# h-walk/PSA

Measured on AMD Instinct MI355X. Metric: SED throughput (k-points*timesteps*atoms/s), higher is better.
Workload: dtype f32 (2xf16 split MFMA, fp32 accumulate)

## Files before the change

include/psa_hip.h:

```cpp
#ifndef PSA_HIP_H
#define PSA_HIP_H

#include <stdint.h>

#ifdef __cplusplus
extern "C" {
#endif

#define PSA_HIP_ABI_VERSION 6

#define PSA_OK          0
#define PSA_EINVAL     -1
#define PSA_EHIP       -2
#define PSA_EFFT       -3
#define PSA_ERCCL      -4
#define PSA_ESTATE     -5
#define PSA_ENOMEM     -6

#define PSA_SLOT_VELOCITIES 0
#define PSA_SLOT_POSITIONS  1
#define PSA_NUM_SLOTS       2

#define PSA_F_DISPLACEMENTS  0x1
#define PSA_F_INTENSITY      0x2

#define PSA_K1_AUTO   0
#define PSA_K1_WAVE   1
#define PSA_K1_MFMA32 2
#define PSA_K1_SPLIT_BF16 3

typedef struct psa_ctx psa_ctx;

int         psa_abi_version(void);
const char* psa_last_error(void);
int         psa_device_count(int* count);
int         psa_host_alloc(size_t bytes, void** out);
int         psa_host_free(void* p);
int         psa_create(int device, psa_ctx** out);
int         psa_destroy(psa_ctx* ctx);
int         psa_synchronize(psa_ctx* ctx);
int         psa_set_k1(psa_ctx* ctx, int selector);
#define PSA_OPT_PLANES         0
#define PSA_OPT_PLANES_BUDGET  1
#define PSA_OPT_PLANES_EAGER   2
#define PSA_OPT_PLANES_MIN_K   3
#define PSA_OPT_FOLD_PAIRS     4
#define PSA_OPT_FFT_PRIME      5
#define PSA_OPT_K1_LOADER_WAVES 6
#define PSA_OPT_K1_WIDE         7
#define PSA_OPT_K1_LOWRANK      8
#define PSA_OPT_K1_LOWRANK_MIN_K 9
#define PSA_OPT_K1_LOWRANK_MIN_LOCAL 10
#define PSA_OPT_VDOS_WORK_BYTES 11
#define PSA_OPT_MODES_WORK_BYTES 12
#define PSA_OPT_DYNAMIC_WORK_BYTES 13
int         psa_set_option(psa_ctx* ctx, int option, int64_t value);
int         psa_device_info(psa_ctx* ctx, char* name, int name_len,
                            int* compute_units, int64_t* hbm_bytes);

int psa_data_upload(psa_ctx* ctx, int slot, const float* host, int64_t T, int64_t N);
int psa_data_alloc(psa_ctx* ctx, int slot, int64_t T, int64_t N);
int psa_data_download(psa_ctx* ctx, int slot, float* host, int64_t t0, int64_t nt);
int psa_data_release(psa_ctx* ctx, int slot);
int psa_data_shape(psa_ctx* ctx, int slot, int64_t* T, int64_t* N);

int psa_data_fill_synthetic(psa_ctx* ctx, int slot, uint64_t seed, int64_t t_offset, int n_modes,
                            const float* amp, const int32_t* mode_comp,
                            const float* ct, const float* st,
                            const float* ca, const float* sa);

int psa_mean_positions(psa_ctx* ctx, int slot, float* mean_host );

int psa_host_mean_frames(const float* x , int64_t T, int64_t cols, float* mean_out, int threads);

int psa_set_atom_weights(psa_ctx* ctx, const float* w , int64_t N);

int psa_set_segments(psa_ctx* ctx, int64_t L, int64_t hop, const float* window );

int psa_sed_project(psa_ctx* ctx, int slot,
                    const float* mean_pos_all,
                    const float* k_vectors, int64_t K_local,
                    int64_t K_total, int64_t k_offset,
                    const int32_t* group_idx, const int64_t* group_off, int32_t G,
                    int32_t flags);

int psa_sed_project_upload(psa_ctx* ctx, int slot, const float* host, int64_t T, int64_t N,
                           const float* mean_pos_all, const float* k_vectors, int64_t K,
                           const int32_t* group_idx, const int64_t* group_off, int32_t G,
                           int32_t flags);

int psa_sed_finalize(psa_ctx* ctx, void* out_host, size_t out_bytes,
                     float* out_intensity, size_t out_intensity_bytes);

int psa_sed_calculate(psa_ctx* ctx, int slot, const float* mean_pos_all,
                      const float* k_vectors, int64_t K,
                      const int32_t* group_idx, const int64_t* group_off, int32_t G,
                      int32_t flags, void* out_host, size_t out_bytes,
                      float* out_intensity, size_t out_intensity_bytes);

int psa_vdos(psa_ctx* ctx, int slot, const float* mean_pos_all ,
             const int32_t* group_idx, const int64_t* group_off, int32_t G,
             int32_t flags , float* out_host , size_t out_bytes);

int psa_sed_modes(psa_ctx* ctx, int slot, const float* mean_pos_all, const float* k_vectors, int64_t K,
                  const int32_t* group_idx, const int64_t* group_off, int32_t B,
                  const void* eig , int64_t M, int32_t flags ,
                  float* out_host , size_t out_bytes);

int psa_sed_covariance(psa_ctx* ctx, int slot, const float* mean_pos_all, const float* k_vectors, int64_t K,
                       const int32_t* group_idx, const int64_t* group_off, int32_t B,
                       const float* freq_weights , int32_t n_w, int32_t flags ,
                       double* out_host , size_t out_bytes);

typedef struct {
    float   window_hwhm;
    int32_t half_window_bins;
    int32_t max_iter;
} psa_peak_opts;
int psa_fit_peaks(psa_ctx* ctx, const float* spec_host, int64_t F, int64_t C, double df, const int32_t* bands, int32_t lo,
                  int32_t hi, const psa_peak_opts* opts, float* fit , int32_t* info );
int psa_sed_modes_fit(psa_ctx* ctx, int slot, const float* mean_pos_all, const float* k_vectors, int64_t K,
                      const int32_t* group_idx, const int64_t* group_off, int32_t B, const void* eig, int64_t M,
                      int32_t flags, double df, const int32_t* bands, int32_t lo, int32_t hi, const psa_peak_opts* opts,
                      float* fit , int32_t* info , float* out_host, size_t out_bytes);

int psa_sed_modes_welch(psa_ctx* ctx, int slot, const float* mean_pos_all, const float* k_vectors, int64_t K,
                        const int32_t* group_idx, const int64_t* group_off, int32_t B,
                        const void* eig , int64_t M, int32_t flags ,
                        float* out_host , size_t out_bytes);
int psa_sed_modes_welch_fit(psa_ctx* ctx, int slot, const float* mean_pos_all, const float* k_vectors, int64_t K,
                            const int32_t* group_idx, const int64_t* group_off, int32_t B, const void* eig, int64_t M,
                            int32_t flags, double df, const int32_t* bands, int32_t lo, int32_t hi, const psa_peak_opts* opts,
                            float* fit , int32_t* info , float* out_host, size_t out_bytes);

int psa_dynamic_spectra(psa_ctx* ctx, const float* k_vectors, int64_t K, const int32_t* idx, int64_t n_g,
                        int32_t currents , float* out_host ,
                        size_t out_bytes);

int psa_lattice_spectra(psa_ctx* ctx, const double* box_inverse , const int32_t* indices , int64_t K,
                        const int32_t* bin_of , int64_t n_bins, const int32_t* idx, int64_t n_g,
                        int32_t currents , float* out_host ,
                        size_t out_bytes);

int psa_self_spectra(psa_ctx* ctx, const double* box_inverse , const int32_t* indices , int64_t K,
                     const int32_t* bin_of , int64_t n_bins, const int32_t* idx, int64_t n_g,
                     float* out_host , size_t out_bytes);

int psa_partial_spectra(psa_ctx* ctx, const double* box_inverse , const int32_t* indices , int64_t K,
                        const int32_t* bin_of , int64_t n_bins, const int32_t* idx, const int64_t* species_start ,
                        int32_t n_species, int32_t currents ,
                        float* out_host , size_t out_bytes);

int psa_lattice_correlations(psa_ctx* ctx, const double* box_inverse , const int32_t* indices , int64_t K,
                             const int32_t* bin_of , int64_t n_bins, const int32_t* idx, int64_t n_g,
                             int32_t currents , int64_t n_lags,
                             float* out_host , size_t out_bytes);

int psa_self_correlations(psa_ctx* ctx, const double* box_inverse , const int32_t* indices , int64_t K,
                          const int32_t* bin_of , int64_t n_bins, const int32_t* idx, int64_t n_g, int64_t n_lags,
                          float* out_host , size_t out_bytes);

int psa_displacement_moments(psa_ctx* ctx, const double* box , const double* box_inverse , const int32_t* idx,
                             const int64_t* group_start , int32_t n_groups, int64_t n_lags, int64_t origin_step,
                             int32_t unwrap, double* out_host , size_t out_bytes);

int psa_van_hove_self(psa_ctx* ctx, const double* box , const double* box_inverse , const int32_t* idx,
                      const int64_t* group_start , int32_t n_groups, const int64_t* lags , int64_t n_vh,
                      int64_t origin_step, int32_t unwrap, double dr, int32_t n_r, uint64_t* out_host ,
                      size_t out_bytes);

int psa_pair_histogram(psa_ctx* ctx, const double* box , const double* box_inverse , const int32_t* idx,
                       const int64_t* group_start , int32_t n_groups, const int64_t* lags , int64_t n_lags,
                       int64_t origin_step, double dr, int32_t n_r, uint64_t* out_host ,
                       size_t out_bytes);

#define PSA_KMAP_MIRROR 0x80000000u
int psa_k_pairs(const float* k_vectors, int64_t K, int32_t* kmap ,
                int32_t* unique_idx , int64_t* n_unique);
int psa_sed_set_kmap(psa_ctx* ctx, const int32_t* kmap, int64_t K_out);

int psa_lowrank_plan(const float* k_vectors, int64_t K, const float* mean_pos_all, int64_t N, const int32_t* idx,
                     int64_t n_g, int32_t* ok, double* geo, double* kappa, float* C, float* L, float* phi);

int psa_sed_single_bin(psa_ctx* ctx, int slot, const float* mean_pos_all, const float* k_vector,
                       const int32_t* idx, int64_t n_g, int32_t flags, int64_t i_w,
                       float* out_c64x3 );

int psa_slab_read(psa_ctx* ctx, int64_t row0, int64_t nrows, void* host);
int psa_slab_write(psa_ctx* ctx, int64_t row0, int64_t nrows, const void* host);

int psa_result_intensity(psa_ctx* ctx, float* out_host , size_t out_bytes);
int psa_result_chiral_phase(psa_ctx* ctx, int c1, int c2, float* out_host, size_t out_bytes);

int psa_last_timings(psa_ctx* ctx, double* ms );
int psa_k1_stats(psa_ctx* ctx, int64_t* launches, double* total_ms);
int psa_k1_lowrank_launches(psa_ctx* ctx, int64_t* launches);
int psa_oneoff_stats(psa_ctx* ctx, double* ms );

int psa_debug_phase_table(psa_ctx* ctx, const float* mean_pos_all,
                          const float* k_vectors, int64_t K,
                          const int32_t* idx, int64_t n_g, int64_t N,
                          void* out_host);
int psa_debug_project_only(psa_ctx* ctx, int slot, const float* mean_pos_all,
                           const float* k_vectors, int64_t K,
                           const int32_t* idx, int64_t n_g, int32_t flags,
                           void* out_host);
int psa_debug_project_route(psa_ctx* ctx, int slot, const float* mean_pos_all,
                            const float* k_vectors, int64_t K,
                            const int32_t* idx, int64_t n_g, int32_t flags,
                            void* out_host);
int psa_debug_project_frames(psa_ctx* ctx, int slot, const float* mean_pos_all,
                             const float* k_vectors, int64_t K,
                             const int32_t* idx, int64_t n_g, int32_t flags,
                             int64_t t_begin, int64_t t_count, void* out_host);
int psa_debug_mode_power(psa_ctx* ctx, const void* S_host, const void* eig, int32_t B, int64_t K, int64_t M, int64_t T,
                         float* out_host);
int psa_debug_covariance(psa_ctx* ctx, const void* S_host , int32_t B, int64_t K,
                         int64_t T, const float* freq_weights, int32_t n_w, double scale, double* out_host);
int psa_debug_mode_power_welch(psa_ctx* ctx, const void* S_host, const void* eig, int32_t B, int64_t K, int64_t M, int64_t L,
                               int64_t ns, int64_t seg_block, float scale, float* out_host);
int psa_debug_dynamic_project(psa_ctx* ctx, const float* k_vectors, int64_t K, const int32_t* idx, int64_t n_g,
                              int32_t currents, void* out_host);
int psa_debug_dynamic_sincos(psa_ctx* ctx, const float* turns, int64_t n, float* out_host);
int psa_debug_lattice_project(psa_ctx* ctx, const double* box_inverse, const int32_t* indices, int64_t K, const int32_t* idx,
                              int64_t n_g, int32_t currents, void* out_host);
int psa_debug_self_series(psa_ctx* ctx, const double* box_inverse, const int32_t* indices, int64_t K, const int32_t* idx,
                          int64_t n_g, void* out_host);
int psa_debug_dynamic_power(psa_ctx* ctx, const void* seg_host, const float* k_vectors , int64_t K, int32_t currents,
                            int64_t n_seg, int64_t L, int64_t k_block, int64_t seg_block, float scale, float* out_host);
int psa_debug_lattice_shell(psa_ctx* ctx, const void* seg_host, const float* khat , const int32_t* bin_of ,
                            int64_t K, int64_t n_bins, int32_t currents, int64_t n_seg, int64_t L, int64_t k_block,
                            int64_t seg_block, double norm, float* out_host);
int psa_debug_self_power(psa_ctx* ctx, const void* work_host, int64_t na, int64_t nv, int64_t n_seg, int64_t L,
                         const int32_t* groups, int64_t n_groups, int64_t cols, const double* scale, int32_t mirror,
                         int64_t n_chunks, int64_t atom_block, int64_t vec_block, int64_t seg_block, float* out_host);
int psa_debug_partial_project(psa_ctx* ctx, const double* box_inverse, const int32_t* indices, int64_t K, const int32_t* idx,
                              const int64_t* species_start, int32_t n_species, int32_t currents, void* out_host);
int psa_debug_partial_power(psa_ctx* ctx, const void* seg_host, const float* khat , const int32_t* bin_of ,
                            int64_t K, int64_t n_bins, int32_t n_species, int32_t currents, int64_t n_seg, int64_t L,
                            int64_t k_block, int64_t seg_block, double norm, float* out_host);
int psa_debug_plane_cache(psa_ctx* ctx, int64_t* n_sets, int64_t* bytes);

#define PSA_UNIQUE_ID_BYTES 128
int psa_comm_unique_id(void* out );
int psa_comm_init(psa_ctx* ctx, const void* unique_id, int rank, int nranks);
int psa_comm_destroy(psa_ctx* ctx);
int psa_comm_selftest(psa_ctx* ctx);
int psa_sed_gather(psa_ctx* ctx, int root, const int64_t* k_offsets, const int64_t* k_counts);
int psa_comm_barrier(psa_ctx* ctx);

int psa_sed_fs_project(psa_ctx* ctx, int slot, const float* mean_pos_all,
                       const float* k_vectors, int64_t K_total,
                       const int32_t* idx, int64_t n_g, int32_t flags,
                       int64_t T_total, int64_t k_offset, int64_t k_count);
int psa_sed_fs_exchange(psa_ctx* ctx, const int64_t* t_offsets, const int64_t* t_counts,
                        const int64_t* k_offsets, const int64_t* k_counts);
int psa_sed_fs_read(psa_ctx* ctx, int64_t k0, int64_t nk, void* host);
int psa_sed_fs_write(psa_ctx* ctx, int64_t t0, int64_t nt, const void* host);
int psa_sed_fs_finish(psa_ctx* ctx, int32_t first_group);

int psa_debug_correlation_transform(psa_ctx* ctx, const double* X_host, int64_t fields, int64_t P, int64_t cols, int64_t L,
                                    int64_t n_seg, int64_t n_lags, int32_t as_float32, float* out_host);

int psa_debug_unwrap(psa_ctx* ctx, const double* box , const double* box_inverse , const int32_t* idx, int64_t n_g,
                     int32_t unwrap, double* out_u , int32_t* out_images );

int psa_debug_pair_fractions(psa_ctx* ctx, const double* box_inverse , const int32_t* idx, int64_t n_g,
                             float* out );

int psa_debug_pair_plan(const int64_t* sizes , int32_t n_groups, int32_t sym, int64_t n_origins, int64_t* out );

#ifdef __cplusplus
}
#endif
#endif
```

psa_amd/_hip.py:

```python
from __future__ import annotations

import ctypes as C
import os
import threading
import weakref
from pathlib import Path
from typing import Optional, Sequence

import numpy as np

LIB_PATH = Path(__file__).resolve().parent / "csrc" / "libpsa_hip.so"

SLOT_VELOCITIES, SLOT_POSITIONS = 0, 1
F_DISPLACEMENTS, F_INTENSITY = 0x1, 0x2
K1_AUTO, K1_WAVE, K1_MFMA32, K1_SPLIT_BF16 = 0, 1, 2, 3
OPT_PLANES, OPT_PLANES_BUDGET, OPT_PLANES_EAGER, OPT_PLANES_MIN_K, OPT_FOLD_PAIRS, OPT_FFT_PRIME = 0, 1, 2, 3, 4, 5
OPT_K1_LOADER_WAVES = 6
OPT_K1_WIDE = 7
OPT_K1_LOWRANK = 8
OPT_K1_LOWRANK_MIN_K = 9
OPT_K1_LOWRANK_MIN_LOCAL = 10
OPT_VDOS_WORK_BYTES = 11
OPT_MODES_WORK_BYTES = 12
OPT_DYNAMIC_WORK_BYTES = 13
KMAP_MIRROR = 0x80000000
ABI_VERSION = 6
COV_CHAIN = 128
COV_FOLDS = 32
COV_TILE = 64
COV_CHUNK = COV_CHAIN * COV_FOLDS
COV_MAX_ROWS = 96
DYN_THREADS = 256
DYN_ATOMS = 512
DYN_CHAIN = 128
DYN_FRAMES = 4
DYN_SINCOS_ERR = 2.6e-7
LAT_THREADS = 256
LAT_KS = 512
LAT_ATOMS = 128
LAT_TABLE = 3584
LAT_CHAIN = 128
LAT_FRAMES = 4
LAT_MAX_INDEX = 64
LAT_MAX_ENTRIES = 3 * (2 * LAT_MAX_INDEX + 1)
PARTIAL_MAX_SPECIES = 8
SELF_THREADS = 256
SELF_ATOMS = 4
SELF_FRAMES = 64
SELF_ENTRIES = 24
SELF_KS = 64
MSD_LAGS = 256
MSD_ORIGINS = 1024
MSD_WINDOW = 1280
MSD_MAX_GROUPS = 8
MSD_MAX_BINS = 1024
MSD_MAX_VH_LAGS = 64
MSD_UNWRAP_FRAMES = 64
MSD_UNWRAP_ATOMS = 16
PAIR_TILE = 256
PAIR_MAX_BINS = 1024
PAIR_MAX_LAGS = 64
PAIR_MAX_SPECIES = 8
UNIQUE_ID_BYTES = 128
TIMING_NAMES = ("h2d", "phase", "project", "fft", "epilogue", "gather", "transpose", "d2h")

_f32p = C.POINTER(C.c_float)
_i32p = C.POINTER(C.c_int32)
_i64p = C.POINTER(C.c_int64)
_ctx = C.c_void_p

SIGNATURES = {
    "psa_abi_version": (C.c_int, []),
    "psa_last_error": (C.c_char_p, []),
    "psa_device_count": (C.c_int, [C.POINTER(C.c_int)]),
    "psa_host_alloc": (C.c_int, [C.c_size_t, C.POINTER(C.c_void_p)]),
    "psa_host_free": (C.c_int, [C.c_void_p]),
    "psa_create": (C.c_int, [C.c_int, C.POINTER(_ctx)]),
    "psa_destroy": (C.c_int, [_ctx]),
    "psa_synchronize": (C.c_int, [_ctx]),
    "psa_set_k1": (C.c_int, [_ctx, C.c_int]),
    "psa_set_option": (C.c_int, [_ctx, C.c_int, C.c_int64]),
    "psa_device_info": (C.c_int, [_ctx, C.c_char_p, C.c_int, C.POINTER(C.c_int), _i64p]),
    "psa_data_upload": (C.c_int, [_ctx, C.c_int, _f32p, C.c_int64, C.c_int64]),
    "psa_data_alloc": (C.c_int, [_ctx, C.c_int, C.c_int64, C.c_int64]),
    "psa_data_download": (C.c_int, [_ctx, C.c_int, _f32p, C.c_int64, C.c_int64]),
    "psa_data_release": (C.c_int, [_ctx, C.c_int]),
    "psa_data_shape": (C.c_int, [_ctx, C.c_int, _i64p, _i64p]),
    "psa_data_fill_synthetic": (C.c_int, [_ctx, C.c_int, C.c_uint64, C.c_int64, C.c_int, _f32p, _i32p,
                                          _f32p, _f32p, _f32p, _f32p]),
    "psa_mean_positions": (C.c_int, [_ctx, C.c_int, _f32p]),
    "psa_host_mean_frames": (C.c_int, [_f32p, C.c_int64, C.c_int64, _f32p, C.c_int]),
    "psa_set_atom_weights": (C.c_int, [_ctx, _f32p, C.c_int64]),
    "psa_set_segments": (C.c_int, [_ctx, C.c_int64, C.c_int64, _f32p]),
    "psa_sed_project": (C.c_int, [_ctx, C.c_int, _f32p, _f32p, C.c_int64, C.c_int64, C.c_int64,
                                  _i32p, _i64p, C.c_int32, C.c_int32]),
    "psa_sed_project_upload": (C.c_int, [_ctx, C.c_int, _f32p, C.c_int64, C.c_int64, _f32p, _f32p, C.c_int64,
                                         _i32p, _i64p, C.c_int32, C.c_int32]),
    "psa_sed_finalize": (C.c_int, [_ctx, C.c_void_p, C.c_size_t, _f32p, C.c_size_t]),
    "psa_sed_calculate": (C.c_int, [_ctx, C.c_int, _f32p, _f32p, C.c_int64, _i32p, _i64p,
                                    C.c_int32, C.c_int32, C.c_void_p, C.c_size_t, _f32p, C.c_size_t]),
    "psa_vdos": (C.c_int, [_ctx, C.c_int, _f32p, _i32p, _i64p, C.c_int32, C.c_int32, _f32p, C.c_size_t]),
    "psa_sed_modes": (C.c_int, [_ctx, C.c_int, _f32p, _f32p, C.c_int64, _i32p, _i64p, C.c_int32, C.c_void_p, C.c_int64,
                                C.c_int32, _f32p, C.c_size_t]),
    "psa_fit_peaks": (C.c_int, [_ctx, _f32p, C.c_int64, C.c_int64, C.c_double, _i32p, C.c_int32, C.c_int32, C.c_void_p,
                                _f32p, _i32p]),
    "psa_sed_modes_fit": (C.c_int, [_ctx, C.c_int, _f32p, _f32p, C.c_int64, _i32p, _i64p, C.c_int32, C.c_void_p, C.c_int64,
                                    C.c_int32, C.c_double, _i32p, C.c_int32, C.c_int32, C.c_void_p, _f32p, _i32p, _f32p,
                                    C.c_size_t]),
    "psa_sed_modes_welch": (C.c_int, [_ctx, C.c_int, _f32p, _f32p, C.c_int64, _i32p, _i64p, C.c_int32, C.c_void_p, C.c_int64,
                                      C.c_int32, _f32p, C.c_size_t]),
    "psa_sed_modes_welch_fit": (C.c_int, [_ctx, C.c_int, _f32p, _f32p, C.c_int64, _i32p, _i64p, C.c_int32, C.c_void_p,
                                          C.c_int64, C.c_int32, C.c_double, _i32p, C.c_int32, C.c_int32, C.c_void_p, _f32p,
                                          _i32p, _f32p, C.c_size_t]),
    "psa_dynamic_spectra": (C.c_int, [_ctx, _f32p, C.c_int64, _i32p, C.c_int64, C.c_int32, _f32p, C.c_size_t]),
    "psa_debug_dynamic_project": (C.c_int, [_ctx, _f32p, C.c_int64, _i32p, C.c_int64, C.c_int32, C.c_void_p]),
    "psa_debug_dynamic_sincos": (C.c_int, [_ctx, _f32p, C.c_int64, _f32p]),
    "psa_lattice_spectra": (C.c_int, [_ctx, C.POINTER(C.c_double), _i32p, C.c_int64, _i32p, C.c_int64, _i32p, C.c_int64, C.c_int32,
                                      _f32p, C.c_size_t]),
    "psa_debug_lattice_project": (C.c_int, [_ctx, C.POINTER(C.c_double), _i32p, C.c_int64, _i32p, C.c_int64, C.c_int32, C.c_void_p]),
    "psa_self_spectra": (C.c_int, [_ctx, C.POINTER(C.c_double), _i32p, C.c_int64, _i32p, C.c_int64, _i32p, C.c_int64, _f32p,
                                   C.c_size_t]),
    "psa_debug_self_series": (C.c_int, [_ctx, C.POINTER(C.c_double), _i32p, C.c_int64, _i32p, C.c_int64, C.c_void_p]),
    "psa_debug_dynamic_power": (C.c_int, [_ctx, C.c_void_p, _f32p, C.c_int64, C.c_int32, C.c_int64, C.c_int64, C.c_int64, C.c_int64,
                                          C.c_float, _f32p]),
    "psa_debug_lattice_shell": (C.c_int, [_ctx, C.c_void_p, _f32p, _i32p, C.c_int64, C.c_int64, C.c_int32, C.c_int64, C.c_int64,
                                          C.c_int64, C.c_int64, C.c_double, _f32p]),
    "psa_debug_self_power": (C.c_int, [_ctx, C.c_void_p, C.c_int64, C.c_int64, C.c_int64, C.c_int64, _i32p, C.c_int64, C.c_int64,
                                       C.POINTER(C.c_double), C.c_int32, C.c_int64, C.c_int64, C.c_int64, C.c_int64, _f32p]),
    "psa_partial_spectra": (C.c_int, [_ctx, C.POINTER(C.c_double), _i32p, C.c_int64, _i32p, C.c_int64, _i32p, _i64p, C.c_int32,
                                      C.c_int32, _f32p, C.c_size_t]),
    "psa_debug_partial_project": (C.c_int, [_ctx, C.POINTER(C.c_double), _i32p, C.c_int64, _i32p, _i64p, C.c_int32, C.c_int32,
                                            C.c_void_p]),
    "psa_debug_partial_power": (C.c_int, [_ctx, C.c_void_p, _f32p, _i32p, C.c_int64, C.c_int64, C.c_int32, C.c_int32, C.c_int64,
                                          C.c_int64, C.c_int64, C.c_int64, C.c_double, _f32p]),
    "psa_lattice_correlations": (C.c_int, [_ctx, C.POINTER(C.c_double), _i32p, C.c_int64, _i32p, C.c_int64, _i32p, C.c_int64,
                                           C.c_int32, C.c_int64, _f32p, C.c_size_t]),
    "psa_self_correlations": (C.c_int, [_ctx, C.POINTER(C.c_double), _i32p, C.c_int64, _i32p, C.c_int64, _i32p, C.c_int64,
                                        C.c_int64, _f32p, C.c_size_t]),
    "psa_debug_correlation_transform": (C.c_int, [_ctx, C.POINTER(C.c_double), C.c_int64, C.c_int64, C.c_int64, C.c_int64,
                                                  C.c_int64, C.c_int64, C.c_int32, _f32p]),
    "psa_displacement_moments": (C.c_int, [_ctx, C.POINTER(C.c_double), C.POINTER(C.c_double), _i32p, _i64p, C.c_int32, C.c_int64,
                                           C.c_int64, C.c_int32, C.POINTER(C.c_double), C.c_size_t]),
    "psa_van_hove_self": (C.c_int, [_ctx, C.POINTER(C.c_double), C.POINTER(C.c_double), _i32p, _i64p, C.c_int32, _i64p, C.c_int64,
                                    C.c_int64, C.c_int32, C.c_double, C.c_int32, C.POINTER(C.c_uint64), C.c_size_t]),
    "psa_debug_unwrap": (C.c_int, [_ctx, C.POINTER(C.c_double), C.POINTER(C.c_double), _i32p, C.c_int64, C.c_int32,
                                   C.POINTER(C.c_double), _i32p]),
    "psa_pair_histogram": (C.c_int, [_ctx, C.POINTER(C.c_double), C.POINTER(C.c_double), _i32p, _i64p, C.c_int32, _i64p, C.c_int64,
                                     C.c_int64, C.c_double, C.c_int32, C.POINTER(C.c_uint64), C.c_size_t]),
    "psa_debug_pair_fractions": (C.c_int, [_ctx, C.POINTER(C.c_double), _i32p, C.c_int64, _f32p]),
    "psa_debug_pair_plan": (C.c_int, [_i64p, C.c_int32, C.c_int32, C.c_int64, _i64p]),
    "psa_k_pairs": (C.c_int, [_f32p, C.c_int64, _i32p, _i32p, _i64p]),
    "psa_lowrank_plan": (C.c_int, [_f32p, C.c_int64, _f32p, C.c_int64, _i32p, C.c_int64, _i32p, C.POINTER(C.c_double),
                                   C.POINTER(C.c_double), _f32p, _f32p, _f32p]),
    "psa_sed_set_kmap": (C.c_int, [_ctx, _i32p, C.c_int64]),
    "psa_sed_single_bin": (C.c_int, [_ctx, C.c_int, _f32p, _f32p, _i32p, C.c_int64, C.c_int32, C.c_int64, _f32p]),
    "psa_slab_read": (C.c_int, [_ctx, C.c_int64, C.c_int64, C.c_void_p]),
    "psa_slab_write": (C.c_int, [_ctx, C.c_int64, C.c_int64, C.c_void_p]),
    "psa_result_intensity": (C.c_int, [_ctx, _f32p, C.c_size_t]),
    "psa_result_chiral_phase": (C.c_int, [_ctx, C.c_int, C.c_int, _f32p, C.c_size_t]),
    "psa_last_timings": (C.c_int, [_ctx, C.POINTER(C.c_double)]),
    "psa_k1_stats": (C.c_int, [_ctx, _i64p, C.POINTER(C.c_double)]),
    "psa_k1_lowrank_launches": (C.c_int, [_ctx, _i64p]),
    "psa_oneoff_stats": (C.c_int, [_ctx, C.POINTER(C.c_double)]),
    "psa_debug_phase_table": (C.c_int, [_ctx, _f32p, _f32p, C.c_int64, _i32p, C.c_int64,
                                        C.c_int64, C.c_void_p]),
    "psa_debug_project_only": (C.c_int, [_ctx, C.c_int, _f32p, _f32p, C.c_int64, _i32p,
                                         C.c_int64, C.c_int32, C.c_void_p]),
    "psa_debug_project_route": (C.c_int, [_ctx, C.c_int, _f32p, _f32p, C.c_int64, _i32p,
                                          C.c_int64, C.c_int32, C.c_void_p]),
    "psa_debug_project_frames": (C.c_int, [_ctx, C.c_int, _f32p, _f32p, C.c_int64, _i32p,
                                           C.c_int64, C.c_int32, C.c_int64, C.c_int64, C.c_void_p]),
    "psa_debug_mode_power": (C.c_int, [_ctx, C.c_void_p, C.c_void_p, C.c_int32, C.c_int64, C.c_int64, C.c_int64, _f32p]),
    "psa_debug_mode_power_welch": (C.c_int, [_ctx, C.c_void_p, C.c_void_p, C.c_int32, C.c_int64, C.c_int64, C.c_int64,
                                             C.c_int64, C.c_int64, C.c_float, _f32p]),
    "psa_sed_covariance": (C.c_int, [_ctx, C.c_int, _f32p, _f32p, C.c_int64, _i32p, _i64p, C.c_int32, _f32p, C.c_int32, C.c_int32,
                                     C.c_void_p, C.c_size_t]),
    "psa_debug_covariance": (C.c_int, [_ctx, C.c_void_p, C.c_int32, C.c_int64, C.c_int64, _f32p, C.c_int32, C.c_double,
                                       C.c_void_p]),
    "psa_debug_plane_cache": (C.c_int, [_ctx, _i64p, _i64p]),
    "psa_comm_unique_id": (C.c_int, [C.c_void_p]),
    "psa_comm_init": (C.c_int, [_ctx, C.c_void_p, C.c_int, C.c_int]),
    "psa_comm_destroy": (C.c_int, [_ctx]),
    "psa_comm_selftest": (C.c_int, [_ctx]),
    "psa_sed_gather": (C.c_int, [_ctx, C.c_int, _i64p, _i64p]),
    "psa_comm_barrier": (C.c_int, [_ctx]),
    "psa_sed_fs_project": (C.c_int, [_ctx, C.c_int, _f32p, _f32p, C.c_int64, _i32p, C.c_int64, C.c_int32,
                                     C.c_int64, C.c_int64, C.c_int64]),
    "psa_sed_fs_exchange": (C.c_int, [_ctx, _i64p, _i64p, _i64p, _i64p]),
    "psa_sed_fs_read": (C.c_int, [_ctx, C.c_int64, C.c_int64, C.c_void_p]),
    "psa_sed_fs_write": (C.c_int, [_ctx, C.c_int64, C.c_int64, C.c_void_p]),
    "psa_sed_fs_finish": (C.c_int, [_ctx, C.c_int32]),
}


class PeakOpts(C.Structure):
    _fields_ = [("window_hwhm", C.c_float), ("half_window_bins", C.c_int32), ("max_iter", C.c_int32)]


class PsaHipError(RuntimeError):
    """A libpsa_hip entry point returned a non-zero code."""


_lib = None
_lib_lock = threading.Lock()


def load_library() -> C.CDLL:
    global _lib
    with _lib_lock:
        if _lib is not None:
            return _lib
        path = Path(os.environ.get("PSA_HIP_LIBRARY", LIB_PATH))
        if not path.exists():
            raise PsaHipError(
                f"{path} not found: build it with `make -C psa_amd/csrc` (needs hipcc, gfx950). "
                "psa_amd has no CPU fallback.")
        os.environ.setdefault("HSA_ENABLE_IPC_MODE_LEGACY", "0")
        lib = C.CDLL(str(path))
        for name, (res, args) in SIGNATURES.items():
            fn = getattr(lib, name)
            fn.restype, fn.argtypes = res, args
        _lib = lib
        return lib


def _check(rc: int, what: str):
    if rc != 0:
        msg = load_library().psa_last_error().decode("utf-8", "replace")
        if rc == -1 and "out of bounds" in msg:
            raise ValueError(msg)
        raise PsaHipError(f"{what} failed (rc={rc}): {msg}")


def _f32(a: np.ndarray):
    return a.ctypes.data_as(_f32p)


def _as_f32(a, shape_tail=None) -> np.ndarray:
    arr = np.ascontiguousarray(a, dtype=np.float32)
    if shape_tail is not None and arr.shape[1:] != shape_tail:
        raise ValueError(f"expected (*,{shape_tail}) array, got {arr.shape}")
    return arr


def device_count() -> int:
    n = C.c_int(0)
    _check(load_library().psa_device_count(C.byref(n)), "psa_device_count")
    return n.value


def k_pairs(k_vectors):
    kv = _as_f32(k_vectors, (3,)) if len(k_vectors) else np.zeros((0, 3), np.float32)
    K = kv.shape[0]
    kmap, uidx, n = np.zeros(K, np.int32), np.zeros(K, np.int32), C.c_int64(0)
    _check(load_library().psa_k_pairs(_f32(kv), K, kmap.ctypes.data_as(_i32p), uidx.ctypes.data_as(_i32p), C.byref(n)),
           "psa_k_pairs")
    return kmap.view(np.uint32), uidx[:n.value].copy()


def lowrank_plan(k_vectors, mean_pos_all, idx=None):
    kv = _as_f32(k_vectors, (3,))
    mean = _as_f32(mean_pos_all, (3,))
    K, N = kv.shape[0], mean.shape[0]
    ix = None if idx is None else np.ascontiguousarray(idx, np.int32)
    n_g = N if ix is None else ix.size
    ok, geo = C.c_int32(0), np.zeros(12, np.float64)
    kappa, cm = np.zeros(64, np.float64), np.zeros((K, 64), np.complex64)
    lw, phi = np.zeros((K, 64), np.float32), np.zeros(K, np.complex64)
    dp = C.POINTER(C.c_double)
    _check(load_library().psa_lowrank_plan(_f32(kv), K, _f32(mean), N, None if ix is None else ix.ctypes.data_as(_i32p), n_g,
                                           C.byref(ok), geo.ctypes.data_as(dp), kappa.ctypes.data_as(dp),
                                           cm.ctypes.data_as(_f32p), _f32(lw), phi.ctypes.data_as(_f32p)), "psa_lowrank_plan")
    if not ok.value:
        return None
    return {"u": geo[0:3].copy(), "k0": geo[3:6].copy(), "x_c": geo[6], "h_x": geo[7], "width": geo[8],
            "interval": int(geo[9]), "d_bound": geo[10], "dscale": geo[11], "kappa": kappa, "C": cm, "L": lw, "phi": phi}


def host_mean_frames(x: np.ndarray, threads: int = 0) -> np.ndarray:
    if x.dtype != np.float32 or not x.flags.c_contiguous or x.ndim < 2 or x.shape[0] < 1 or x.size == 0:
        raise ValueError("host_mean_frames needs a non-empty C-contiguous float32 array")
    out = np.empty(x.shape[1:], np.float32)
    cols = int(np.prod(x.shape[1:], dtype=np.int64))
    _check(load_library().psa_host_mean_frames(_f32(x), x.shape[0], cols, _f32(out), int(threads)), "psa_host_mean_frames")
    return out


def pack_groups(groups: Optional[Sequence[np.ndarray]]):
    if groups is None:
        return None, None, 1
    off = np.zeros(len(groups) + 1, dtype=np.int64)
    off[1:] = np.cumsum([len(g) for g in groups])
    idx = (np.concatenate([np.asarray(g).ravel() for g in groups]) if off[-1] > 0
           else np.zeros(0, dtype=np.int64))
    if idx.size and (idx.min() < 0 or idx.max() >= 2 ** 31):
        raise ValueError("Atom indices in basis out of bounds.")
    return np.ascontiguousarray(idx, dtype=np.int32), off, len(groups)


class _PinnedPool:

    granule = 2 << 20
    min_bytes = 1 << 20
    keep_bytes = 4 << 30
    max_live_bytes = 16 << 30

    def __init__(self):
        self._idle = {}
        self._idle_bytes = 0
        self._live_bytes = 0
        self._lock = threading.Lock()
        self.stats = {"recycled": 0, "allocated": 0, "pageable": 0}

    def _give_back(self, address: int, size: int):
        with self._lock:
            self._live_bytes -= size
            if self._idle_bytes + size <= self.keep_bytes:
                self._idle.setdefault(size, []).append(address)
                self._idle_bytes += size
                return
        load_library().psa_host_free(C.c_void_p(address))

    def empty(self, shape, dtype) -> np.ndarray:
        dtype = np.dtype(dtype)
        nbytes = int(np.prod(shape, dtype=np.int64)) * dtype.itemsize
        if nbytes < self.min_bytes:
            return np.empty(shape, dtype)
        size = -(-nbytes // self.granule) * self.granule
        with self._lock:
            if self._live_bytes + size > self.max_live_bytes:
                self.stats["pageable"] += 1
                return np.empty(shape, dtype)
            self._live_bytes += size
            stack = self._idle.get(size)
            address = stack.pop() if stack else None
            if address is not None:
                self._idle_bytes -= size
        if address is None:
            p = C.c_void_p()
            try:
                _check(load_library().psa_host_alloc(size, C.byref(p)), "psa_host_alloc")
            except PsaHipError:
                with self._lock:
                    self._live_bytes -= size
                    self.stats["pageable"] += 1
                return np.empty(shape, dtype)
            address = p.value
            self.stats["allocated"] += 1
        else:
            self.stats["recycled"] += 1
        block = (C.c_char * size).from_address(address)
        weakref.finalize(block, self._give_back, address, size)
        return np.frombuffer(block, dtype=dtype, count=nbytes // dtype.itemsize).reshape(shape)

    def drain(self):
        with self._lock:
            idle, self._idle, self._idle_bytes = self._idle, {}, 0
        for stack in idle.values():
            for address in stack:
                load_library().psa_host_free(C.c_void_p(address))


_pinned_pool = _PinnedPool()


def pinned_empty(shape, dtype) -> np.ndarray:
    return _pinned_pool.empty(shape, dtype)


_SAMPLE_CACHE = {}


def _sample_positions(shape):
    hit = _SAMPLE_CACHE.get(shape)
    if hit is None:
        size = int(np.prod(shape, dtype=np.int64))
        lin = np.arange(0, size, max(1, size // 1021), dtype=np.int64)[:1021]
        if size > 2048:
            lin = np.concatenate([lin, np.sort(np.random.default_rng(size).integers(0, size, 1021)), [size - 1]])
        if len(_SAMPLE_CACHE) > 64:
            _SAMPLE_CACHE.clear()
        hit = _SAMPLE_CACHE[shape] = (lin, np.unravel_index(lin, shape))
    return hit


class Engine:

    def __init__(self, device: Optional[int] = None):
        self._lib = load_library()
        if device is None:
            device = int(os.environ.get("PSA_HIP_DEVICE", os.environ.get("LOCAL_RANK", "0")))
            n = device_count()
            if n == 0:
                raise PsaHipError("no HIP device visible; psa_amd has no CPU fallback")
            device %= n
        h = _ctx()
        _check(self._lib.psa_create(int(device), C.byref(h)), "psa_create")
        self._h = h
        self.device = int(device)
        self._resident = {}
        self._converted = {}
        self.lock = threading.RLock()
        self.rank, self.nranks = 0, 1
        self.result_serial = 0
        self.segment_length = 0

    def close(self):
        if getattr(self, "_h", None):
            self._lib.psa_destroy(self._h)
            self._h = None

    def __del__(self):
        try:
            self.close()
        except Exception:
            pass

    def synchronize(self):
        _check(self._lib.psa_synchronize(self._h), "psa_synchronize")

    def set_k1(self, selector: int):
        _check(self._lib.psa_set_k1(self._h, selector), "psa_set_k1")

    def device_info(self) -> dict:
        name = C.create_string_buffer(256)
        cu, mem = C.c_int(0), C.c_int64(0)
        _check(self._lib.psa_device_info(self._h, name, 256, C.byref(cu), C.byref(mem)),
               "psa_device_info")
        return {"name": name.value.decode(), "compute_units": cu.value, "hbm_bytes": mem.value}

    @staticmethod
    def _fingerprint(a: np.ndarray) -> int:
        if a.size == 0:
            return 0
        base = a
        while base is not None and not isinstance(base, np.memmap):
            base = getattr(base, "base", None)
        if base is not None and getattr(base, "filename", None):
            try:
                st = os.stat(base.filename)
                return hash((str(base.filename), st.st_size, st.st_mtime_ns, a.shape, a.strides))
            except OSError:
                pass
        lin, idx = _sample_positions(a.shape)
        if a.flags.c_contiguous:
            return hash(a.reshape(-1)[lin].tobytes())
        return hash(a[idx].tobytes())

    def _as_device_layout(self, slot: int, array: np.ndarray) -> np.ndarray:
        if array.ndim != 3 or array.shape[2] != 3:
            raise ValueError("trajectory array must be (frames, atoms, 3)")
        if array.dtype == np.float32 and array.flags.c_contiguous:
            return array
        held = self._converted.get(slot)
        fp = self._fingerprint(array)
        if held is not None and held[0]() is array and held[1] == fp:
            return held[2]
        conv = np.ascontiguousarray(array, dtype=np.float32)
        try:
            self._converted[slot] = (weakref.ref(array), fp, conv)
        except TypeError:
            self._converted.pop(slot, None)
        return conv

    def is_resident(self, slot: int, array: np.ndarray) -> bool:
        held = self._resident.get(slot)
        if held is None or held[0] is None:
            return False
        a = array if held[0]() is array else self._as_device_layout(slot, array)
        return (held[0]() is a and held[1:3] == (a.ctypes.data, a.shape) and held[3] == self._fingerprint(a))

    def _note_resident(self, slot: int, a: np.ndarray):
        try:
            ref = weakref.ref(a)
        except TypeError:
            ref = None
        self._resident[slot] = (ref, a.ctypes.data, a.shape, self._fingerprint(a))

    def ensure_resident(self, slot: int, array: np.ndarray):
        if self.is_resident(slot, array):
            return
        a = self._as_device_layout(slot, array)
        T, N = a.shape[0], a.shape[1]
        _check(self._lib.psa_data_upload(self._h, slot, _f32(a), T, N), "psa_data_upload")
        self._note_resident(slot, a)

    def invalidate(self, slot: Optional[int] = None):
        if slot is None:
            self._resident.clear()
            self._converted.clear()
        else:
            self._resident.pop(slot, None)
            self._converted.pop(slot, None)

    def alloc(self, slot: int, T: int, N: int):
        _check(self._lib.psa_data_alloc(self._h, slot, T, N), "psa_data_alloc")
        self._resident[slot] = (None, None, (T, N, 3), None)

    def fill_synthetic(self, slot: int, seed: int, amp, comp, ct, st, ca, sa, t_offset: int = 0):
        amp = np.ascontiguousarray(amp, np.float32)
        comp = np.ascontiguousarray(comp, np.int32)
        tabs = [np.ascontiguousarray(x, np.float32) for x in (ct, st, ca, sa)]
        _check(self._lib.psa_data_fill_synthetic(
            self._h, slot, C.c_uint64(seed), int(t_offset), len(amp), _f32(amp), comp.ctypes.data_as(_i32p),
            *[_f32(t) for t in tabs]), "psa_data_fill_synthetic")

    def set_option(self, option: int, value: int):
        _check(self._lib.psa_set_option(self._h, option, int(value)), "psa_set_option")

    def plane_cache(self):
        n, b = C.c_int64(0), C.c_int64(0)
        _check(self._lib.psa_debug_plane_cache(self._h, C.byref(n), C.byref(b)), "psa_debug_plane_cache")
        return n.value, b.value

    def download(self, slot: int, t0: int, nt: int) -> np.ndarray:
        T, N = self.shape(slot)
        out = np.empty((nt, N, 3), np.float32)
        _check(self._lib.psa_data_download(self._h, slot, _f32(out), t0, nt), "psa_data_download")
        return out

    def release(self, slot: int):
        _check(self._lib.psa_data_release(self._h, slot), "psa_data_release")
        self._resident.pop(slot, None)

    def shape(self, slot: int):
        T, N = C.c_int64(0), C.c_int64(0)
        _check(self._lib.psa_data_shape(self._h, slot, C.byref(T), C.byref(N)), "psa_data_shape")
        return T.value, N.value

    def mean_positions(self, slot: int) -> np.ndarray:
        _, N = self.shape(slot)
        out = np.empty((N, 3), np.float32)
        _check(self._lib.psa_mean_positions(self._h, slot, _f32(out)), "psa_mean_positions")
        return out

    def set_atom_weights(self, weights: Optional[np.ndarray]):
        if weights is None:
            _check(self._lib.psa_set_atom_weights(self._h, None, 0), "psa_set_atom_weights")
            return
        w = np.ascontiguousarray(weights, np.float32)
        if w.ndim != 1 or w.size == 0:
            raise ValueError(f"atom weights must be a non-empty (N,) array, got shape {w.shape}")
        if not np.all(np.isfinite(w)):
            raise ValueError("atom weights must be finite")
        _check(self._lib.psa_set_atom_weights(self._h, _f32(w), w.shape[0]), "psa_set_atom_weights")

    def set_segments(self, segments):
        if segments is None:
            _check(self._lib.psa_set_segments(self._h, 0, 0, None), "psa_set_segments")
            self.segment_length = 0
            return
        w = np.ascontiguousarray(segments.window_array(), np.float32)
        _check(self._lib.psa_set_segments(self._h, segments.length, segments.hop, _f32(w)), "psa_set_segments")
        self.segment_length = segments.length

    def project(self, slot, mean_pos_all, k_vectors, groups=None, flags=0,
                K_total=None, k_offset=0):
        mean = _as_f32(mean_pos_all, (3,))
        kv = _as_f32(k_vectors, (3,)) if len(k_vectors) else np.zeros((0, 3), np.float32)
        idx, off, G = pack_groups(groups)
        K_local = kv.shape[0]
        self.result_serial += 1
        _check(self._lib.psa_sed_project(
            self._h, slot, _f32(mean), _f32(kv), K_local,
            K_local if K_total is None else K_total, k_offset,
            idx.ctypes.data_as(_i32p) if idx is not None else None,
            off.ctypes.data_as(_i64p) if off is not None else None, G, flags),
            "psa_sed_project")

    def project_upload(self, slot, array, mean_pos_all, k_vectors, groups=None, flags=0):
        a = self._as_device_layout(slot, array)
        mean = _as_f32(mean_pos_all, (3,))
        kv = _as_f32(k_vectors, (3,))
        idx, off, G = pack_groups(groups)
        self._resident.pop(slot, None)
        self.result_serial += 1
        _check(self._lib.psa_sed_project_upload(
            self._h, slot, _f32(a), a.shape[0], a.shape[1], _f32(mean), _f32(kv), kv.shape[0],
            idx.ctypes.data_as(_i32p) if idx is not None else None,
# ... 245 lines not shown
        _check(self._lib.psa_lattice_correlations(self._h, inv.ctypes.data_as(C.POINTER(C.c_double)), n.ctypes.data_as(_i32p), K,
                                                  None if bins is None else bins.ctypes.data_as(_i32p), int(n_bins), ip, n_g,
                                                  1 if currents else 0, int(n_lags), _f32(out), out.nbytes),
               "psa_lattice_correlations")
        return out

    def self_correlations(self, box_inverse, indices, n_lags: int, bin_of=None, n_bins=0, idx=None) -> np.ndarray:
        inv, n, keep, ip, n_g = self._lattice_args(box_inverse, indices, idx)
        K = n.shape[0]
        bins = None if bin_of is None else np.ascontiguousarray(bin_of, np.int32).ravel()
        if bins is not None and bins.size != K:
            raise ValueError(f"bin_of has {bins.size} entries for {K} vectors")
        out = np.empty((max(int(n_lags), 0), K if bins is None else int(n_bins)), np.float32)
        _check(self._lib.psa_self_correlations(self._h, inv.ctypes.data_as(C.POINTER(C.c_double)), n.ctypes.data_as(_i32p), K,
                                               None if bins is None else bins.ctypes.data_as(_i32p), int(n_bins), ip, n_g,
                                               int(n_lags), _f32(out), out.nbytes), "psa_self_correlations")
        return out

    @staticmethod
    def _displacement_args(box, box_inverse, groups):
        H = np.ascontiguousarray(box, np.float64)
        if H.shape != (3, 3):
            raise ValueError(f"box must be (3, 3), got {H.shape}")
        if box_inverse is None:
            try:
                box_inverse = np.linalg.inv(H)
            except np.linalg.LinAlgError as e:
                raise ValueError(f"the box is singular: {e}") from None
        inv = np.ascontiguousarray(box_inverse, np.float64)
        if inv.shape != (3, 3):
            raise ValueError(f"box_inverse must be (3, 3), got {inv.shape}")
        if groups is None:
            return H, inv, None, None, None, None, 1
        lists = [np.asarray(g, np.int32).ravel() for g in groups]
        start = np.zeros(len(lists) + 1, np.int64)
        start[1:] = np.cumsum([g.size for g in lists])
        flat = np.ascontiguousarray(np.concatenate(lists) if lists else np.zeros(0, np.int32), np.int32)
        keep = flat if flat.size else np.zeros(1, np.int32)
        return H, inv, keep, keep.ctypes.data_as(_i32p), start, start.ctypes.data_as(_i64p), len(lists)

    def displacement_moments(self, box, n_lags: int, groups=None, origin_step: int = 1, unwrap: bool = True,
                             box_inverse=None) -> np.ndarray:
        H, inv, keep, ip, start, sp, G = self._displacement_args(box, box_inverse, groups)
        out = np.empty((max(int(n_lags), 0), G, 4), np.float64)
        dp = C.POINTER(C.c_double)
        _check(self._lib.psa_displacement_moments(self._h, H.ctypes.data_as(dp), inv.ctypes.data_as(dp), ip, sp, G, int(n_lags),
                                                  int(origin_step), 1 if unwrap else 0, out.ctypes.data_as(dp), out.nbytes),
               "psa_displacement_moments")
        return out

    def van_hove_self(self, box, lags, dr: float, n_r: int, groups=None, origin_step: int = 1, unwrap: bool = True,
                      box_inverse=None) -> np.ndarray:
        H, inv, keep, ip, start, sp, G = self._displacement_args(box, box_inverse, groups)
        tau = np.ascontiguousarray(lags, np.int64).ravel()
        held = tau if tau.size else np.zeros(1, np.int64)
        out = np.empty((tau.size, G, max(int(n_r), 0) + 1), np.uint64)
        dp = C.POINTER(C.c_double)
        _check(self._lib.psa_van_hove_self(self._h, H.ctypes.data_as(dp), inv.ctypes.data_as(dp), ip, sp, G,
                                           held.ctypes.data_as(_i64p), tau.size, int(origin_step), 1 if unwrap else 0, float(dr),
                                           int(n_r), out.ctypes.data_as(C.POINTER(C.c_uint64)), out.nbytes), "psa_van_hove_self")
        return out

    def debug_unwrap(self, box, idx=None, unwrap: bool = True, images: bool = True, box_inverse=None):
        T, N = self.shape(SLOT_POSITIONS)
        H, inv, keep, ip, _, _, _ = self._displacement_args(box, box_inverse, None if idx is None else [idx])
        n_g = N if idx is None else int(np.asarray(idx).size)
        u = np.empty((T, n_g, 3), np.float64)
        img = np.empty((T, n_g, 3), np.int32) if images else None
        dp = C.POINTER(C.c_double)
        _check(self._lib.psa_debug_unwrap(self._h, H.ctypes.data_as(dp), inv.ctypes.data_as(dp), ip, n_g, 1 if unwrap else 0,
                                          u.ctypes.data_as(dp), None if img is None else img.ctypes.data_as(_i32p)),
               "psa_debug_unwrap")
        return u, img

    def pair_histogram(self, box, lags, dr: float, n_r: int, groups=None, origin_step: int = 1, box_inverse=None) -> np.ndarray:
        H, inv, keep, ip, start, sp, G = self._displacement_args(box, box_inverse, groups)
        tau = np.ascontiguousarray(lags, np.int64).ravel()
        held = tau if tau.size else np.zeros(1, np.int64)
        out = np.empty((tau.size, G, G, max(int(n_r), 0) + 1), np.uint64)
        dp = C.POINTER(C.c_double)
        _check(self._lib.psa_pair_histogram(self._h, H.ctypes.data_as(dp), inv.ctypes.data_as(dp), ip, sp, G,
                                            held.ctypes.data_as(_i64p), tau.size, int(origin_step), float(dr), int(n_r),
                                            out.ctypes.data_as(C.POINTER(C.c_uint64)), out.nbytes), "psa_pair_histogram")
        return out

    def debug_pair_fractions(self, box, idx=None, box_inverse=None) -> np.ndarray:
        T, N = self.shape(SLOT_POSITIONS)
        H, inv, keep, ip, _, _, _ = self._displacement_args(box, box_inverse, None if idx is None else [idx])
        n_g = N if idx is None else int(np.asarray(idx).size)
        out = np.empty((T, n_g, 3), np.float32)
        _check(self._lib.psa_debug_pair_fractions(self._h, inv.ctypes.data_as(C.POINTER(C.c_double)), ip, n_g, _f32(out)),
               "psa_debug_pair_fractions")
        return out

    @staticmethod
    def debug_pair_plan(sizes, sym: bool, n_origins: int) -> dict:
        n = np.ascontiguousarray(sizes, np.int64).ravel()
        out = np.zeros(4, np.int64)
        _check(load_library().psa_debug_pair_plan(n.ctypes.data_as(_i64p), n.size, 1 if sym else 0, int(n_origins),
                                                  out.ctypes.data_as(_i64p)), "psa_debug_pair_plan")
        return dict(run=int(out[0]), slabs=int(out[1]), items=int(out[2]), most_samples=int(out[3]))

    def debug_correlation_transform(self, power, L: int, n_seg: int, n_lags: int, as_float32: bool = False) -> np.ndarray:
        X = np.ascontiguousarray(power, np.float64)
        if X.ndim != 3:
            raise ValueError(f"power {X.shape} does not fit (fields, P, cols)")
        fields, P, cols = X.shape
        out = np.empty((fields, max(int(n_lags), 0), cols), np.float32)
        _check(self._lib.psa_debug_correlation_transform(self._h, X.ctypes.data_as(C.POINTER(C.c_double)), fields, P, cols, int(L),
                                                         int(n_seg), int(n_lags), 1 if as_float32 else 0, _f32(out)),
               "psa_debug_correlation_transform")
        return out

    def _modes_args(self, slot, mean_pos_all, k_vectors, groups, eigenvectors, flags):
        mean = _as_f32(mean_pos_all, (3,))
        kv = _as_f32(k_vectors, (3,))
        idx, off, B = pack_groups(groups)
        eig = np.ascontiguousarray(eigenvectors, np.complex64)
        K = kv.shape[0]
        if eig.ndim != 4 or eig.shape[0] != K or eig.shape[2:] != (B, 3) or eig.shape[1] < 1:
            raise ValueError(f"eigenvectors have shape {eig.shape}, expected (K, M, B, 3) = ({K}, M, {B}, 3)")
        M = eig.shape[1]
        head = (self._h, slot, _f32(mean), _f32(kv), K,
                idx.ctypes.data_as(_i32p) if idx is not None else None,
                off.ctypes.data_as(_i64p) if off is not None else None, B,
                eig.ctypes.data_as(C.c_void_p), M, flags)
        return head, K, M, (mean, kv, idx, off, eig)

    def _sed_modes(self, entry, rows, slot, mean_pos_all, k_vectors, groups, eigenvectors, flags):
        head, K, M, _held = self._modes_args(slot, mean_pos_all, k_vectors, groups, eigenvectors, flags)
        out = pinned_empty((rows, K, M), np.float32)
        _check(getattr(self._lib, entry)(*head, _f32(out), out.nbytes), entry)
        return out

    def sed_modes(self, slot, mean_pos_all, k_vectors, groups, eigenvectors, flags=0) -> np.ndarray:
        return self._sed_modes("psa_sed_modes", self.shape(slot)[0], slot, mean_pos_all, k_vectors, groups, eigenvectors, flags)

    def sed_modes_welch(self, slot, mean_pos_all, k_vectors, groups, eigenvectors, flags=0) -> np.ndarray:
        return self._sed_modes("psa_sed_modes_welch", self.segment_length or self.shape(slot)[0], slot, mean_pos_all, k_vectors,
                               groups, eigenvectors, flags)

    def fit_peaks(self, spectrum, df, *, band=None, centers=None, search=None, window_hwhm=8.0, half_window=None,
                  max_iter=50):
        from . import peaks
        spec, shape = peaks.spectrum_columns(spectrum)
        F, ncol = spec.shape
        peaks.check_fit_options(window_hwhm, max_iter)
        bands = peaks.peak_bands(F, df, ncol, band, centers, search)
        opts = PeakOpts(float(window_hwhm), peaks.half_window_bins(half_window, df), int(max_iter))
        fit, info = np.empty((ncol, 6), np.float32), np.empty((ncol, 4), np.int32)
        _check(self._lib.psa_fit_peaks(self._h, _f32(spec), F, ncol, float(df), bands.ctypes.data_as(_i32p), 0, 0,
                                       C.byref(opts), _f32(fit), info.ctypes.data_as(_i32p)), "psa_fit_peaks")
        return peaks.PeakFit.from_arrays(fit, info, shape)

    def _sed_modes_fit(self, entry, rows, slot, mean_pos_all, k_vectors, groups, eigenvectors, df, flags, return_sed, band,
                       centers, search, window_hwhm, half_window, max_iter):
        from . import peaks
        head, K, M, _held = self._modes_args(slot, mean_pos_all, k_vectors, groups, eigenvectors, flags)
        peaks.check_fit_options(window_hwhm, max_iter)
        bands = peaks.peak_bands(rows, df, K * M, band, centers, search)
        opts = PeakOpts(float(window_hwhm), peaks.half_window_bins(half_window, df), int(max_iter))
        fit, info = np.empty((K * M, 6), np.float32), np.empty((K * M, 4), np.int32)
        out = pinned_empty((rows, K, M), np.float32) if return_sed else None
        _check(getattr(self._lib, entry)(
            *head, float(df), bands.ctypes.data_as(_i32p), 0, 0, C.byref(opts), _f32(fit), info.ctypes.data_as(_i32p),
            _f32(out) if out is not None else None, out.nbytes if out is not None else 0), entry)
        return peaks.PeakFit.from_arrays(fit, info, (K, M)), out

    def sed_modes_fit(self, slot, mean_pos_all, k_vectors, groups, eigenvectors, df, flags=0, *, return_sed=False, band=None,
                      centers=None, search=None, window_hwhm=8.0, half_window=None, max_iter=50):
        return self._sed_modes_fit("psa_sed_modes_fit", self.shape(slot)[0], slot, mean_pos_all, k_vectors, groups, eigenvectors,
                                   df, flags, return_sed, band, centers, search, window_hwhm, half_window, max_iter)

    def sed_modes_welch_fit(self, slot, mean_pos_all, k_vectors, groups, eigenvectors, df, flags=0, *, return_sed=False,
                            band=None, centers=None, search=None, window_hwhm=8.0, half_window=None, max_iter=50):
        return self._sed_modes_fit("psa_sed_modes_welch_fit", self.segment_length or self.shape(slot)[0], slot, mean_pos_all,
                                   k_vectors, groups, eigenvectors, df, flags, return_sed, band, centers, search, window_hwhm,
                                   half_window, max_iter)

    def debug_mode_power(self, spectra: np.ndarray, eigenvectors: np.ndarray) -> np.ndarray:
        S = np.ascontiguousarray(spectra, np.complex64)
        eig = np.ascontiguousarray(eigenvectors, np.complex64)
        B, K, _, T = S.shape
        if S.shape[2] != 3 or eig.ndim != 4 or eig.shape[0] != K or eig.shape[2:] != (B, 3):
            raise ValueError(f"spectra {S.shape} and eigenvectors {eig.shape} do not fit (B,K,3,T) and (K,M,B,3)")
        M = eig.shape[1]
        out = np.empty((T, K, M), np.float32)
        _check(self._lib.psa_debug_mode_power(self._h, S.ctypes.data_as(C.c_void_p), eig.ctypes.data_as(C.c_void_p), B, K, M, T,
                                              _f32(out)), "psa_debug_mode_power")
        return out

    def debug_mode_power_welch(self, segments: np.ndarray, eigenvectors: np.ndarray, scale: float = 1.0, seg_block: int = 0
                               ) -> np.ndarray:
        S = np.ascontiguousarray(segments, np.complex64)
        eig = np.ascontiguousarray(eigenvectors, np.complex64)
        if S.ndim != 5 or S.shape[2] != 3 or eig.ndim != 4 or eig.shape[0] != S.shape[1] or eig.shape[2:] != (S.shape[0], 3):
            raise ValueError(f"segments {S.shape} and eigenvectors {eig.shape} do not fit (B,K,3,ns,L) and (K,M,B,3)")
        if int(seg_block) < 0:
            raise ValueError(f"seg_block = {seg_block} must not be negative")
        B, K, _, ns, L = S.shape
        M = eig.shape[1]
        out = np.empty((L, K, M), np.float32)
        _check(self._lib.psa_debug_mode_power_welch(self._h, S.ctypes.data_as(C.c_void_p), eig.ctypes.data_as(C.c_void_p), B, K, M,
                                                    L, ns, int(seg_block), float(scale), _f32(out)),
               "psa_debug_mode_power_welch")
        return out

    def sed_covariance(self, slot, mean_pos_all, k_vectors, groups, freq_weights, flags=0) -> np.ndarray:
        mean = _as_f32(mean_pos_all, (3,))
        kv = _as_f32(k_vectors, (3,))
        idx, off, B = pack_groups(groups)
        g = np.ascontiguousarray(freq_weights, np.float32)
        T = self.shape(slot)[0]
        if g.ndim != 2 or g.shape[1] != T:
            raise ValueError(f"freq_weights have shape {g.shape}, expected (n_w, T) = (n_w, {T})")
        K, n = kv.shape[0], 3 * B
        out = np.empty((g.shape[0], K, n, n), np.complex128)
        _check(self._lib.psa_sed_covariance(
            self._h, slot, _f32(mean), _f32(kv), K,
            idx.ctypes.data_as(_i32p) if idx is not None else None,
            off.ctypes.data_as(_i64p) if off is not None else None, B, _f32(g), g.shape[0], flags,
            out.ctypes.data_as(C.c_void_p), out.nbytes), "psa_sed_covariance")
        return out

    def debug_covariance(self, spectra: np.ndarray, freq_weights: np.ndarray, scale: float = 1.0) -> np.ndarray:
        S = np.ascontiguousarray(spectra, np.complex64)
        g = np.ascontiguousarray(freq_weights, np.float32)
        if S.ndim != 4 or S.shape[2] != 3 or g.ndim != 2 or g.shape[1] != S.shape[3]:
            raise ValueError(f"spectra {S.shape} and freq_weights {g.shape} do not fit (B,K,3,T) and (n_w,T)")
        B, K, _, T = S.shape
        out = np.empty((g.shape[0], K, 3 * B, 3 * B), np.complex128)
        _check(self._lib.psa_debug_covariance(self._h, S.ctypes.data_as(C.c_void_p), B, K, T, _f32(g), g.shape[0], float(scale),
                                              out.ctypes.data_as(C.c_void_p)), "psa_debug_covariance")
        return out

    def set_kmap(self, kmap: np.ndarray):
        m = np.ascontiguousarray(kmap, np.uint32).view(np.int32)
        _check(self._lib.psa_sed_set_kmap(self._h, m.ctypes.data_as(_i32p), len(m)), "psa_sed_set_kmap")

    def slab_read(self, row0: int, nrows: int, T: int, intensity: bool) -> np.ndarray:
        out = np.empty((nrows, T), np.float32) if intensity else np.empty((nrows, 3, T), np.complex64)
        _check(self._lib.psa_slab_read(self._h, row0, nrows, out.ctypes.data_as(C.c_void_p)), "psa_slab_read")
        return out

    def slab_write(self, row0: int, rows: np.ndarray):
        rows = np.ascontiguousarray(rows)
        self.result_serial += 1
        _check(self._lib.psa_slab_write(self._h, row0, rows.shape[0], rows.ctypes.data_as(C.c_void_p)),
               "psa_slab_write")

    def intensity_source(self, array: np.ndarray):
        serial, ref, stamp = self.result_serial, weakref.ref(array), self._fingerprint(array)
        T, K = array.shape[0], array.shape[1]

        def source(current):
            if current is not ref() or self._h is None:
                return None
            with self.lock:
                if self.result_serial != serial or self._fingerprint(current) != stamp:
                    return None
                try:
                    return self.result_intensity(T, K)
                except PsaHipError:
                    return None
        return source

    def result_intensity(self, T: int, K: int) -> np.ndarray:
        out = pinned_empty((T, K), np.float32)
        _check(self._lib.psa_result_intensity(self._h, _f32(out), out.nbytes), "psa_result_intensity")
        return out

    def result_chiral_phase(self, T: int, K: int, c1: int, c2: int) -> np.ndarray:
        out = pinned_empty((T, K), np.float32)
        _check(self._lib.psa_result_chiral_phase(self._h, c1, c2, _f32(out), out.nbytes),
               "psa_result_chiral_phase")
        return out

    def timings(self) -> dict:
        ms = (C.c_double * 8)()
        _check(self._lib.psa_last_timings(self._h, ms), "psa_last_timings")
        return dict(zip(TIMING_NAMES, list(ms)))

    def oneoff_stats(self) -> dict:
        ms = (C.c_double * 4)()
        _check(self._lib.psa_oneoff_stats(self._h, ms), "psa_oneoff_stats")
        return dict(zip(("rocfft_plan", "absmax", "split_planes", "upload"), list(ms)))

    def adopt(self, slot: int, array: np.ndarray):
        T, N = self.shape(slot)
        if tuple(array.shape) != (T, N, 3) or array.dtype != np.float32 or not array.flags.c_contiguous and array.strides != (0, 0, 0):
            raise ValueError("stand-in must be a float32 (T, N, 3) array of the slot's shape")
        self._note_resident(slot, array)

    def k1_stats(self):
        n, ms = C.c_int64(0), C.c_double(0.0)
        _check(self._lib.psa_k1_stats(self._h, C.byref(n), C.byref(ms)), "psa_k1_stats")
        return n.value, ms.value

    def lowrank_launches(self) -> int:
        n = C.c_int64(0)
        _check(self._lib.psa_k1_lowrank_launches(self._h, C.byref(n)), "psa_k1_lowrank_launches")
        return n.value

    def debug_phase_table(self, mean_pos_all, k_vectors, idx=None) -> np.ndarray:
        mean = _as_f32(mean_pos_all, (3,))
        kv = _as_f32(k_vectors, (3,))
        N = mean.shape[0]
        ii = None if idx is None else np.ascontiguousarray(idx, np.int32)
        n_g = N if ii is None else len(ii)
        out = np.empty((kv.shape[0], n_g), np.complex64)
        _check(self._lib.psa_debug_phase_table(
            self._h, _f32(mean), _f32(kv), kv.shape[0],
            ii.ctypes.data_as(_i32p) if ii is not None else None, n_g, N,
            out.ctypes.data_as(C.c_void_p)), "psa_debug_phase_table")
        return out

    def debug_project_only(self, slot, mean_pos_all, k_vectors, idx=None, flags=0, frames=None, route=False) -> np.ndarray:
        if route and frames is not None:
            raise ValueError("route=True projects all frames")
        T, N = self.shape(slot)
        mean = _as_f32(mean_pos_all, (3,))
        kv = _as_f32(k_vectors, (3,))
        ii = None if idx is None else np.ascontiguousarray(idx, np.int32)
        n_g = N if ii is None else len(ii)
        out = np.empty((kv.shape[0], 3, T), np.complex64)
        ip = ii.ctypes.data_as(_i32p) if ii is not None else None
        if route:
            _check(self._lib.psa_debug_project_route(
                self._h, slot, _f32(mean), _f32(kv), kv.shape[0], ip, n_g, flags,
                out.ctypes.data_as(C.c_void_p)), "psa_debug_project_route")
        elif frames is None:
            _check(self._lib.psa_debug_project_only(
                self._h, slot, _f32(mean), _f32(kv), kv.shape[0], ip, n_g, flags,
                out.ctypes.data_as(C.c_void_p)), "psa_debug_project_only")
        else:
            _check(self._lib.psa_debug_project_frames(
                self._h, slot, _f32(mean), _f32(kv), kv.shape[0], ip, n_g, flags, int(frames[0]), int(frames[1]),
                out.ctypes.data_as(C.c_void_p)), "psa_debug_project_frames")
        return out

    @staticmethod
    def new_unique_id() -> bytes:
        buf = C.create_string_buffer(UNIQUE_ID_BYTES)
        _check(load_library().psa_comm_unique_id(buf), "psa_comm_unique_id")
        return buf.raw

    def comm_init(self, unique_id: bytes, rank: int, nranks: int):
        buf = C.create_string_buffer(bytes(unique_id), UNIQUE_ID_BYTES)
        _check(self._lib.psa_comm_init(self._h, buf, rank, nranks), "psa_comm_init")
        self.rank, self.nranks = rank, nranks

    def comm_selftest(self):
        _check(self._lib.psa_comm_selftest(self._h), "psa_comm_selftest")

    def comm_destroy(self):
        _check(self._lib.psa_comm_destroy(self._h), "psa_comm_destroy")
        self.rank, self.nranks = 0, 1

    def gather(self, root: int, k_offsets, k_counts):
        o = np.ascontiguousarray(k_offsets, np.int64)
        n = np.ascontiguousarray(k_counts, np.int64)
        _check(self._lib.psa_sed_gather(self._h, root, o.ctypes.data_as(_i64p),
                                        n.ctypes.data_as(_i64p)), "psa_sed_gather")

    def barrier(self):
        _check(self._lib.psa_comm_barrier(self._h), "psa_comm_barrier")

    def fs_project(self, slot, mean_pos_all, k_vectors, idx, flags, T_total: int, k_offset: int, k_count: int):
        mean = _as_f32(mean_pos_all, (3,))
        kv = _as_f32(k_vectors, (3,))
        ii = None if idx is None else np.ascontiguousarray(idx, np.int32)
        self.result_serial += 1
        _check(self._lib.psa_sed_fs_project(
            self._h, slot, _f32(mean), _f32(kv), kv.shape[0], ii.ctypes.data_as(_i32p) if ii is not None else None,
            0 if ii is None else len(ii), flags, int(T_total), int(k_offset), int(k_count)), "psa_sed_fs_project")

    def fs_exchange(self, t_offsets, t_counts, k_offsets, k_counts):
        arrs = [np.ascontiguousarray(x, np.int64) for x in (t_offsets, t_counts, k_offsets, k_counts)]
        _check(self._lib.psa_sed_fs_exchange(self._h, *[a.ctypes.data_as(_i64p) for a in arrs]), "psa_sed_fs_exchange")

    def fs_read(self, k0: int, nk: int, T_local: int) -> np.ndarray:
        out = np.empty((nk, 3, T_local), np.complex64)
        _check(self._lib.psa_sed_fs_read(self._h, k0, nk, out.ctypes.data_as(C.c_void_p)), "psa_sed_fs_read")
        return out

    def fs_write(self, t0: int, block: np.ndarray):
        block = np.ascontiguousarray(block, np.complex64)
        _check(self._lib.psa_sed_fs_write(self._h, t0, block.shape[2], block.ctypes.data_as(C.c_void_p)),
               "psa_sed_fs_write")

    def fs_finish(self, first_group: bool):
        _check(self._lib.psa_sed_fs_finish(self._h, 1 if first_group else 0), "psa_sed_fs_finish")
```

psa_amd/csrc/api_core.hip:

```cpp
#include "api_internal.h"

#include <unistd.h>

#include <filesystem>

namespace psa {

thread_local std::string g_error;


void set_error(const char* fmt, ...) {
    char    buf[1024];
    va_list ap;
    va_start(ap, fmt);
    vsnprintf(buf, sizeof(buf), fmt, ap);
    va_end(ap);
    g_error = buf;
}

int DevBuf::reserve(size_t bytes) {
    if (bytes <= cap) return PSA_OK;
    if (ptr) {
        PSA_HIP_CHECK(hipFree(ptr));
        ptr = nullptr;
// ... 8 lines not shown
    cap = bytes;
    return PSA_OK;
}

void DevBuf::release() {
    if (ptr) (void)hipFree(ptr);
    ptr = nullptr;
    cap = 0;
}

int enter(psa_ctx* c) {
    PSA_REQUIRE(c != nullptr, "null context");
    PSA_HIP_CHECK(hipSetDevice(c->device));
    return PSA_OK;
}

TimingState& timing(psa_ctx* c) { return c->timing; }

int get_event(TimingState& ts, hipEvent_t* ev) {
    if (!ts.pool.empty()) {
        *ev = ts.pool.back();
        ts.pool.pop_back();
        return PSA_OK;
    }
    PSA_HIP_CHECK(hipEventCreate(ev));
    return PSA_OK;
}

int collect(psa_ctx* c, TimingState& ts) {
    if (ts.pending.empty()) return PSA_OK;
    PSA_HIP_CHECK(hipStreamSynchronize(c->stream));
    for (auto& p : ts.pending) {
        float ms = 0.f;
        PSA_HIP_CHECK(hipEventElapsedTime(&ms, p.e0, p.e1));
        ts.acc[p.stage] += ms;
        if (p.stage == PSA_T_PROJECT) {
            ts.k1_launches += 1;
            ts.k1_ms += ms;
        }
        ts.pool.push_back(p.e0);
        ts.pool.push_back(p.e1);
    }
    ts.pending.clear();
    return PSA_OK;
}

int upload(psa_ctx* c, DevBuf& b, const void* host, size_t bytes) {
    PSA_TRY(b.reserve(bytes ? bytes : 16));
    if (bytes) PSA_HIP_CHECK(hipMemcpyAsync(b.ptr, host, bytes, hipMemcpyHostToDevice, c->stream));
    return PSA_OK;
}

static int create_plan(psa_ctx* c, int64_t T, int64_t batch, FftPlan* p) {
    size_t len = (size_t)T;
    PSA_FFT_CHECK(rocfft_plan_create(&p->plan, rocfft_placement_inplace, rocfft_transform_type_complex_forward,
                                     rocfft_precision_single, 1, &len, (size_t)batch, nullptr));
    PSA_FFT_CHECK(rocfft_plan_get_work_buffer_size(p->plan, &p->work_bytes));
    PSA_FFT_CHECK(rocfft_execution_info_create(&p->info));
    PSA_FFT_CHECK(rocfft_execution_info_set_stream(p->info, c->stream));
    return PSA_OK;
}

static void join_primer(psa_ctx* c) {
    if (!c->fft_primer.joinable()) return;
    HostTimer ht(&c->oneoff_ms[0]);
    c->fft_primer.join();
    if (c->primed.plan) {
        auto key = std::make_pair(c->primed_T, (int64_t)3);
        if (c->plans.find(key) == c->plans.end()) {
            c->plans.emplace(key, c->primed);
        } else {
            (void)rocfft_execution_info_destroy(c->primed.info);
            (void)rocfft_plan_destroy(c->primed.plan);
        }
        c->primed = FftPlan{};
    }
}

void prime_fft(psa_ctx* c, int64_t T) {
    if (!c->opt_fft_prime || c->fft_primer.joinable() || T < 2 || c->primed_T == T) return;
    for (auto& kv : c->plans)
        if (kv.first.first == T) return;
    c->primed_T = T;
    c->fft_primer = std::thread([c, T] {
        (void)hipSetDevice(c->device);
        FftPlan p;
        if (create_plan(c, T, 3, &p) == PSA_OK) c->primed = p;
    });
}

int get_plan(psa_ctx* c, int64_t T, int64_t batch, FftPlan** out) {
    join_primer(c);
    auto key = std::make_pair(T, batch);
    auto it = c->plans.find(key);
    if (it == c->plans.end()) {
        HostTimer ht(&c->oneoff_ms[0]);
        FftPlan   p;
        PSA_TRY(create_plan(c, T, batch, &p));
        it = c->plans.emplace(key, p).first;
    }
    *out = &it->second;
    return PSA_OK;
}

int run_fft(psa_ctx* c, float2* data, int64_t T, int64_t batch) {
    FftPlan* p = nullptr;
    PSA_TRY(get_plan(c, T, batch, &p));
    if (p->work_bytes) {
        PSA_TRY(c->d_fft_work.reserve(p->work_bytes));
        PSA_FFT_CHECK(rocfft_execution_info_set_work_buffer(p->info, c->d_fft_work.ptr, p->work_bytes));
    }
    void* bufs[1] = {data};
    PSA_FFT_CHECK(rocfft_execute(p->plan, bufs, nullptr, p->info));
    return PSA_OK;
}

int check_slot(psa_ctx* c, int slot) {
    PSA_REQUIRE(slot >= 0 && slot < PSA_NUM_SLOTS, "bad data slot %d", slot);
    PSA_REQUIRE(c->slot[slot].valid, "data slot %d holds no array", slot);
    return PSA_OK;
}

int validate_groups(int64_t N, const int32_t* group_idx, const int64_t* group_off, int32_t G) {
    PSA_REQUIRE(G >= 1, "need at least one atom group");
    if (!group_idx) {
        PSA_REQUIRE(G == 1, "group_idx NULL means one group of all atoms (G must be 1)");
        return PSA_OK;
    }
    PSA_REQUIRE(group_off != nullptr, "group_off is NULL");
    PSA_REQUIRE(group_off[0] == 0, "group_off[0] must be 0");
    for (int g = 0; g < G; ++g)
        PSA_REQUIRE(group_off[g + 1] >= group_off[g], "group_off must be non-decreasing");
    for (int64_t i = 0; i < group_off[G]; ++i)
        PSA_REQUIRE(group_idx[i] >= 0 && group_idx[i] < N, "Atom indices in basis out of bounds.");
    return PSA_OK;
}

}

using namespace psa;

extern "C" {

int psa_abi_version(void) { return PSA_HIP_ABI_VERSION; }

const char* psa_last_error(void) { return g_error.c_str(); }

int psa_device_count(int* count) {
    PSA_REQUIRE(count != nullptr, "null count");
    PSA_HIP_CHECK(hipGetDeviceCount(count));
    return PSA_OK;
}

int psa_host_alloc(size_t bytes, void** out) {
    PSA_REQUIRE(out != nullptr && bytes > 0, "bad argument");
    PSA_HIP_CHECK(hipHostMalloc(out, bytes, hipHostMallocDefault));
    return PSA_OK;
}

int psa_host_free(void* p) {
    if (p) PSA_HIP_CHECK(hipHostFree(p));
    return PSA_OK;
}

int psa_create(int device, psa_ctx** out) {
    PSA_REQUIRE(out != nullptr, "null out");
    int n = 0;
    PSA_HIP_CHECK(hipGetDeviceCount(&n));
    PSA_REQUIRE(device >= 0 && device < n, "device %d out of range (%d visible)", device, n);
    PSA_HIP_CHECK(hipSetDevice(device));
    hipDeviceProp_t prop;
    PSA_HIP_CHECK(hipGetDeviceProperties(&prop, device));
    PSA_REQUIRE(std::strncmp(prop.gcnArchName, "gfx950", 6) == 0,
                "libpsa_hip is built for gfx950 (MI355X) only; device %d is %s", device,
                prop.gcnArchName);
    static std::once_flag fft_once;
    std::call_once(fft_once, [] {
        if (!std::getenv("ROCFFT_RTC_CACHE_PATH")) {
            std::string dir;
            if (const char* e = std::getenv("PSA_CACHE_DIR")) dir = e;
            else if (const char* x = std::getenv("XDG_CACHE_HOME")) dir = std::string(x) + "/psa_amd";
            else if (const char* h = std::getenv("HOME")) dir = std::string(h) + "/.cache/psa_amd";
            if (!dir.empty()) {
                std::error_code ec;
                std::filesystem::create_directories(dir, ec);
                if (!ec && ::access(dir.c_str(), W_OK) == 0)
                    ::setenv("ROCFFT_RTC_CACHE_PATH", (dir + "/rocfft_rtc_cache.db").c_str(), 0);
            }
        }
        (void)rocfft_setup();
    });
    psa_ctx* c = new psa_ctx();
    c->device = device;
    c->compute_units = prop.multiProcessorCount;
    if (const char* v = std::getenv("PSA_K1_LOWRANK")) c->opt_k1_lowrank = std::atoi(v) != 0;
    if (const char* v = std::getenv("PSA_K1_LOWRANK_MIN_K")) c->opt_k1_lowrank_min_k = std::max(1, std::atoi(v));
    hipError_t e = hipStreamCreateWithFlags(&c->stream, hipStreamNonBlocking);
    if (e != hipSuccess) {
        delete c;
        set_error("hipStreamCreate failed: %s", hipGetErrorString(e));
        return PSA_EHIP;
    }
    *out = c;
    return PSA_OK;
}

int psa_destroy(psa_ctx* c) {
    if (!c) return PSA_OK;
    {
        Guard g(c);
        (void)hipSetDevice(c->device);
        (void)hipStreamSynchronize(c->stream);
        if (c->fft_primer.joinable()) c->fft_primer.join();
        if (c->primed.plan) {
            (void)rocfft_execution_info_destroy(c->primed.info);
            (void)rocfft_plan_destroy(c->primed.plan);
        }
        if (c->comm) (void)ncclCommDestroy(c->comm);
        for (auto& kv : c->plans) {
            (void)rocfft_execution_info_destroy(kv.second.info);
            (void)rocfft_plan_destroy(kv.second.plan);
        }
        for (auto& p : c->timing.pending) {
            (void)hipEventDestroy(p.e0);
            (void)hipEventDestroy(p.e1);
        }
        for (auto ev : c->timing.pool) (void)hipEventDestroy(ev);
        for (auto& s : c->slot) s.buf.release();
        for (auto& ps : c->planes) ps->buf.release();
        c->planes.clear();
        stager_release(c);
        if (c->d2h_stream) (void)hipStreamDestroy(c->d2h_stream);
        if (c->d2h_ready) (void)hipEventDestroy(c->d2h_ready);
        for (DevBuf* b : {&c->d_kvec, &c->d_mean_all, &c->d_idx, &c->d_mean_g, &c->d_phase, &c->d_qwork,
                          &c->d_fft_work, &c->d_tables, &c->d_absmax, &c->d_slab, &c->d_out, &c->d_aux, &c->d_sync,
                          &c->d_qrows, &c->d_stage, &c->d_bin, &c->d_upload_max, &c->d_zeros, &c->d_kmap, &c->d_cols, &c->d_inten,
                          &c->d_vdos_work, &c->d_vdos_pairs, &c->d_vdos_off, &c->d_vdos_mean, &c->d_vdos_part, &c->d_vdos_acc,
                          &c->d_vdos_out, &c->d_modes_work, &c->d_modes_coef, &c->d_modes_out, &c->d_cov_slab, &c->d_cov_g, &c->d_cov_out, &c->d_peaks_spec, &c->d_peaks_bands,
                          &c->d_peaks_part, &c->d_peaks_fit, &c->d_peaks_info, &c->d_dyn_q, &c->d_dyn_kappa, &c->d_dyn_khat, &c->d_dyn_idx,
                          &c->d_dyn_out, &c->d_lat_q, &c->d_lat_tiles, &c->d_lat_ent, &c->d_lat_slot, &c->d_lat_dest, &c->d_lat_khat,
                          &c->d_lat_idx, &c->d_lat_bins, &c->d_lat_scale, &c->d_lat_acc, &c->d_lat_out, &c->d_self_work, &c->d_self_tiles,
                          &c->d_self_ent, &c->d_self_slot, &c->d_self_idx, &c->d_self_groups, &c->d_self_scale, &c->d_self_part, &c->d_self_acc,
                          &c->d_self_out, &c->d_par_q, &c->d_par_tiles, &c->d_par_ent, &c->d_par_slot, &c->d_par_dest, &c->d_par_khat,
                          &c->d_par_idx, &c->d_par_bins, &c->d_par_scale, &c->d_par_acc, &c->d_par_out, &c->d_corr_tab, &c->d_corr_factor,
                          &c->d_corr_scale, &c->d_corr_in, &c->d_corr_out, &c->d_msd_u, &c->d_msd_img, &c->d_msd_sums, &c->d_msd_offs,
                          &c->d_msd_idx, &c->d_msd_chunks, &c->d_msd_sizes, &c->d_msd_lags, &c->d_msd_part, &c->d_msd_acc, &c->d_msd_out,
                          &c->d_pair_c, &c->d_pair_idx, &c->d_pair_items, &c->d_pair_part, &c->d_pair_acc})
            b->release();
        (void)hipStreamDestroy(c->stream);
    }
    delete c;
    return PSA_OK;
}

int psa_synchronize(psa_ctx* c) {
    PSA_TRY(enter(c));
    Guard g(c);
    PSA_HIP_CHECK(hipStreamSynchronize(c->stream));
    return PSA_OK;
}

int psa_set_k1(psa_ctx* c, int selector) {
    PSA_TRY(enter(c));
    PSA_REQUIRE(selector == PSA_K1_AUTO || selector == PSA_K1_WAVE || selector == PSA_K1_MFMA32 ||
                    selector == PSA_K1_SPLIT_BF16,
                "unknown K1 selector %d", selector);
    Guard g(c);
    c->k1_selector = selector;
    return PSA_OK;
}

int psa_set_option(psa_ctx* c, int option, int64_t value) {
    PSA_TRY(enter(c));
    Guard g(c);
    switch (option) {
        case PSA_OPT_PLANES:
            c->opt_planes = value != 0;
            if (!c->opt_planes) {
                PSA_HIP_CHECK(hipStreamSynchronize(c->stream));
                for (auto& ps : c->planes) ps->buf.release();
                c->planes.clear();
            }
            return PSA_OK;
        case PSA_OPT_PLANES_BUDGET:
            PSA_REQUIRE(value >= 0, "negative plane budget");
            c->opt_planes_budget = value;
            return PSA_OK;
        case PSA_OPT_PLANES_EAGER: c->opt_planes_eager = value != 0; return PSA_OK;
        case PSA_OPT_PLANES_MIN_K:
            PSA_REQUIRE(value >= 1, "PSA_OPT_PLANES_MIN_K must be >= 1");
            c->opt_planes_min_k = value;
            return PSA_OK;
        case PSA_OPT_FOLD_PAIRS: c->opt_fold_pairs = value != 0; return PSA_OK;
        case PSA_OPT_FFT_PRIME: c->opt_fft_prime = value != 0; return PSA_OK;
        case PSA_OPT_K1_LOADER_WAVES: c->opt_k1_loader_waves = value != 0; return PSA_OK;
        case PSA_OPT_K1_WIDE: c->opt_k1_wide = value != 0; return PSA_OK;
        case PSA_OPT_K1_LOWRANK:
            c->opt_k1_lowrank = value != 0;
            if (!c->opt_k1_lowrank) {
                PSA_HIP_CHECK(hipStreamSynchronize(c->stream));
                for (psa::DevBuf* b : {&c->d_lr_diff, &c->d_lr_qn, &c->d_lr_L, &c->d_lr_phi, &c->d_lr_f64}) b->release();
            }
            return PSA_OK;
        case PSA_OPT_K1_LOWRANK_MIN_LOCAL:
            PSA_REQUIRE(value >= 1, "PSA_OPT_K1_LOWRANK_MIN_LOCAL must be >= 1");
            c->opt_k1_lowrank_min_local = value;
            return PSA_OK;
        case PSA_OPT_K1_LOWRANK_MIN_K:
            PSA_REQUIRE(value >= 1, "PSA_OPT_K1_LOWRANK_MIN_K must be >= 1");
            c->opt_k1_lowrank_min_k = value;
            return PSA_OK;
        case PSA_OPT_VDOS_WORK_BYTES:
            PSA_REQUIRE(value >= 1, "PSA_OPT_VDOS_WORK_BYTES must be >= 1");
            c->opt_vdos_work_bytes = value;
            return PSA_OK;
        case PSA_OPT_MODES_WORK_BYTES:
            PSA_REQUIRE(value >= 1, "PSA_OPT_MODES_WORK_BYTES must be >= 1");
            c->opt_modes_work_bytes = value;
            return PSA_OK;
        case PSA_OPT_DYNAMIC_WORK_BYTES:
            PSA_REQUIRE(value >= 1, "PSA_OPT_DYNAMIC_WORK_BYTES must be >= 1");
            c->opt_dynamic_work_bytes = value;
            return PSA_OK;
    }
    set_error("unknown option %d", option);
    return PSA_EINVAL;
}

int psa_device_info(psa_ctx* c, char* name, int name_len, int* compute_units, int64_t* hbm_bytes) {
    PSA_TRY(enter(c));
    hipDeviceProp_t prop;
    PSA_HIP_CHECK(hipGetDeviceProperties(&prop, c->device));
    if (name && name_len > 0) {
        std::snprintf(name, (size_t)name_len, "%s (%s)", prop.name[0] ? prop.name : "AMD GPU",
                      prop.gcnArchName);
    }
    if (compute_units) *compute_units = prop.multiProcessorCount;
    if (hbm_bytes) *hbm_bytes = (int64_t)prop.totalGlobalMem;
    return PSA_OK;
}

int psa_last_timings(psa_ctx* c, double* ms) {
    PSA_TRY(enter(c));
    PSA_REQUIRE(ms != nullptr, "null output");
    Guard guard(c);
    TimingState& ts = timing(c);
    PSA_TRY(collect(c, ts));
    for (int i = 0; i < PSA_T_COUNT; ++i) {
        ms[i] = ts.acc[i];
        ts.acc[i] = 0.0;
    }
    return PSA_OK;
}

int psa_oneoff_stats(psa_ctx* c, double* ms) {
    PSA_TRY(enter(c));
    PSA_REQUIRE(ms != nullptr, "null output");
    Guard guard(c);
    for (int i = 0; i < 4; ++i) {
        ms[i] = c->oneoff_ms[i];
        c->oneoff_ms[i] = 0.0;
    }
    return PSA_OK;
}

int psa_k1_lowrank_launches(psa_ctx* c, int64_t* launches) {
    PSA_TRY(enter(c));
    PSA_REQUIRE(launches != nullptr, "null argument");
    *launches = c->lowrank_launches;
    return PSA_OK;
}

int psa_k1_stats(psa_ctx* c, int64_t* launches, double* total_ms) {
    PSA_TRY(enter(c));
    Guard guard(c);
    TimingState& ts = timing(c);
    PSA_TRY(collect(c, ts));
    if (launches) *launches = ts.k1_launches;
    if (total_ms) *total_ms = ts.k1_ms;
    ts.k1_launches = 0;
    ts.k1_ms = 0.0;
    return PSA_OK;
}

}
```

psa_amd/csrc/api_lowrank.hip:

```cpp
#include "api_internal.h"

namespace psa {

namespace {
constexpr double LR_OMEGA = 30.0;
constexpr double LR_D_MAX = 1.0 / 8192.0;
}

int plan_lowrank(const float* k, int64_t K, const float* mean_all, int64_t N, const int32_t* h_idx, int64_t n_g, LowRankPlan* p,
                 float* C) {
    *p = LowRankPlan{};
    auto fail = [&](const char* why) {
        p->why = why;
        return PSA_OK;
    };
    if (K < 2) return fail("fewer than two k-vectors");
    if (n_g < 1) return fail("empty group");
    for (int64_t i = 0; i < 3 * K; ++i)
        if (!std::isfinite(k[i])) return fail("k-vector not finite");
    double  p0[3] = {k[0], k[1], k[2]}, far = 0.0;
    int64_t jf = 0;
    for (int64_t j = 1; j < K; ++j) {
        double d2 = 0.0;
        for (int i = 0; i < 3; ++i) d2 += ((double)k[3 * j + i] - p0[i]) * ((double)k[3 * j + i] - p0[i]);
        if (d2 > far) {
            far = d2;
            jf = j;
        }
    }
    if (!(far > 0.0)) return fail("all k-vectors equal");
    double u[3], nu = std::sqrt(far);
    for (int i = 0; i < 3; ++i) u[i] = ((double)k[3 * jf + i] - p0[i]) / nu;
    {
        int im = 0;
        for (int i = 1; i < 3; ++i)
            if (std::fabs(u[i]) > std::fabs(u[im])) im = i;
        if (u[im] < 0)
            for (double& v : u) v = -v;
    }
    bool snapped = false;
    for (int n = 1; n <= 12 && !snapped; ++n) {
        double m[3], mn = 0.0, dev = 0.0;
        const double s = n / std::max({std::fabs(u[0]), std::fabs(u[1]), std::fabs(u[2])});
        for (int i = 0; i < 3; ++i) {
            m[i] = std::nearbyint(u[i] * s);
            mn += m[i] * m[i];
        }
        mn = std::sqrt(mn);
        for (int i = 0; i < 3; ++i) dev = std::max(dev, std::fabs(m[i] / mn - u[i]));
        if (dev < 1e-6) {
            for (int i = 0; i < 3; ++i) u[i] = m[i] / mn + 0.0;
            snapped = true;
        }
    }
    if (!snapped) return fail("direction not a lattice direction");
    {
        double kmax2 = 0.0, off2 = 0.0;
        for (int64_t j = 0; j < K; ++j) {
            double kj[3], d = 0.0, n2 = 0.0;
            for (int i = 0; i < 3; ++i) {
                kj[i] = k[3 * j + i];
                d += kj[i] * u[i];
                n2 += kj[i] * kj[i];
            }
            double o2 = 0.0;
            for (int i = 0; i < 3; ++i) o2 += (kj[i] - d * u[i]) * (kj[i] - d * u[i]);
            kmax2 = std::max(kmax2, n2);
            off2 = std::max(off2, o2);
        }
        if (!(std::sqrt(off2) <= 1e-5 * std::sqrt(kmax2))) return fail("line does not pass through Gamma");
    }
    for (int i = 0; i < 3; ++i) p->u[i] = u[i];
    double xmin = INFINITY, xmax = -INFINITY, rmax = 0.0, rabs[3] = {0, 0, 0};
    for (int64_t a = 0; a < n_g; ++a) {
        const int64_t src = h_idx ? h_idx[a] : a;
        if (src < 0 || src >= N) return fail("index outside the trajectory");
        const float* r = mean_all + 3 * src;
        if (!std::isfinite(r[0]) || !std::isfinite(r[1]) || !std::isfinite(r[2])) return fail("mean position not finite");
        const double x = u[0] * r[0] + u[1] * r[1] + u[2] * r[2];
        xmin = std::min(xmin, x);
        xmax = std::max(xmax, x);
        rmax = std::max(rmax, std::sqrt((double)r[0] * r[0] + (double)r[1] * r[1] + (double)r[2] * r[2]));
        for (int i = 0; i < 3; ++i) rabs[i] = std::max(rabs[i], (double)std::fabs(r[i]));
    }
    p->x_c = 0.5 * (xmin + xmax);
    p->h_x = std::max(0.5 * (xmax - xmin), 1e-12);
    p->width = 2.0 * LR_OMEGA / p->h_x;
    p->kline.resize((size_t)3 * K);
    std::vector<double> kap((size_t)K);
    double              off = 0.0, kabs[3] = {0, 0, 0};
    for (int64_t j = 0; j < K; ++j) {
        double kj[3], kk = 0.0;
        for (int i = 0; i < 3; ++i) {
            kj[i] = k[3 * j + i];
            kk += (kj[i] - p->k0[i]) * u[i];
            kabs[i] = std::max(kabs[i], std::fabs(kj[i]));
        }
        kap[(size_t)j] = kk;
        double e2 = 0.0;
        for (int i = 0; i < 3; ++i) {
            p->kline[3 * j + i] = p->k0[i] + kk * u[i];
            e2 += (kj[i] - p->kline[3 * j + i]) * (kj[i] - p->kline[3 * j + i]);
        }
        off = std::max(off, std::sqrt(e2));
    }
    p->d_bound = 0x1p-22 * (kabs[0] * rabs[0] + kabs[1] * rabs[1] + kabs[2] * rabs[2]) + off * rmax + 0x1p-20;
    if (!(p->d_bound <= LR_D_MAX)) return fail("k-vectors not on one line (or phases too large)");
    bool pos = true, neg = true;
    for (int64_t j = 0; j < K; ++j) {
        pos = pos && kap[(size_t)j] >= 0.0;
        neg = neg && kap[(size_t)j] <= 0.0;
    }
    if (!pos && !neg) return fail("k-list crosses Gamma");
    const bool   side = pos;
    const double n0 = std::floor(std::fabs(kap[0]) / p->width);
    for (int64_t j = 0; j < K; ++j)
        if (std::floor(std::fabs(kap[(size_t)j]) / p->width) != n0) return fail("k-path longer than one node interval");
    p->interval = side ? (int64_t)n0 : -(int64_t)n0 - 1;
    const double mid = (p->interval + 0.5) * p->width, half = 0.5 * p->width;
    double       bw[LOWRANK_NODES];
    for (int l = 0; l < LOWRANK_NODES; ++l) {
        const double th = M_PI * (2 * l + 1) / (2.0 * LOWRANK_NODES);
        p->kappa[l] = mid + half * std::cos(th);
        bw[l] = ((l & 1) ? -1.0 : 1.0) * std::sin(th);
    }
    p->L.assign((size_t)K * LOWRANK_NODES, 0.f);
    p->phi.assign((size_t)K * 2, 0.f);
    for (int64_t j = 0; j < K; ++j) {
        const double kj = kap[(size_t)j];
        double       L[LOWRANK_NODES], den = 0.0;
        int          hit = -1;
        for (int l = 0; l < LOWRANK_NODES; ++l)
            if (kj == p->kappa[l]) hit = l;
        if (hit >= 0) {
            for (int l = 0; l < LOWRANK_NODES; ++l) L[l] = l == hit;
        } else {
            for (int l = 0; l < LOWRANK_NODES; ++l) {
                L[l] = bw[l] / (kj - p->kappa[l]);
                den += L[l];
            }
            for (double& v : L) v /= den;
        }
        const double cr = std::cos(kj * p->x_c), ci = std::sin(kj * p->x_c);
        p->phi[(size_t)j * 2 + 0] = (float)cr;
        p->phi[(size_t)j * 2 + 1] = (float)ci;
        for (int l = 0; l < LOWRANK_NODES; ++l) {
            p->L[(size_t)j * LOWRANK_NODES + l] = (float)L[l];
            if (C) {
                C[((size_t)j * LOWRANK_NODES + l) * 2 + 0] = (float)(cr * L[l]);
                C[((size_t)j * LOWRANK_NODES + l) * 2 + 1] = (float)(ci * L[l]);
            }
        }
    }
    p->dscale = std::ldexp(1.0f, 14 - (int)std::ceil(std::log2(p->d_bound)));
    p->ok = true;
    return PSA_OK;
}

int prepare_lowrank(psa_ctx* c, const GroupView& v, const ProjectArgs& list, int64_t k_first, int64_t nk, ProjGeom* g) {
    g->lowrank = false;
    if (!c->opt_k1_lowrank || g->split != K1Family::f16_planes || !v.ps || list.K_total < c->opt_k1_lowrank_min_k ||
        nk < c->opt_k1_lowrank_min_local)
        return PSA_OK;
    LowRankPlan p;
    PSA_TRY(plan_lowrank(list.k_vectors + 3 * k_first, nk, list.mean_pos_all, c->slot[v.slot].N, v.h_idx, g->n_g, &p));
    if (!p.ok) return PSA_OK;
    std::vector<double> f64((size_t)7 + LOWRANK_NODES + 3 * (size_t)nk);
    std::memcpy(f64.data(), p.k0, 3 * sizeof(double));
    std::memcpy(f64.data() + 3, p.u, 3 * sizeof(double));
    f64[6] = p.x_c;
    std::memcpy(f64.data() + 7, p.kappa, sizeof(p.kappa));
    std::memcpy(f64.data() + 7 + LOWRANK_NODES, p.kline.data(), p.kline.size() * sizeof(double));
    PSA_TRY(upload(c, c->d_lr_f64, f64.data(), f64.size() * sizeof(double)));
    PSA_TRY(upload(c, c->d_lr_L, p.L.data(), p.L.size() * sizeof(float)));
    PSA_TRY(upload(c, c->d_lr_phi, p.phi.data(), p.phi.size() * sizeof(float)));
    PSA_TRY(c->d_lr_qn.reserve((size_t)LOWRANK_NODES * 3 * (size_t)c->slot[v.slot].T * sizeof(float2)));
    g->lowrank = true;
    g->dscale = p.dscale;
    g->M_pad_d = (int)((2 * nk + 511) / 512 * 512);
    return PSA_OK;
}

}

using namespace psa;

extern "C" {

int psa_lowrank_plan(const float* k_vectors, int64_t K, const float* mean_pos_all, int64_t N, const int32_t* idx, int64_t n_g,
                     int32_t* ok, double* geo, double* kappa, float* C, float* L, float* phi) {
    PSA_REQUIRE(K >= 0 && K < (1ll << 29) && N >= 1 && n_g >= 0 && n_g <= (idx ? (int64_t)1 << 30 : N) && ok && geo &&
                    (K == 0 || k_vectors) && mean_pos_all,
                "bad argument");
    LowRankPlan p;
    PSA_TRY(plan_lowrank(k_vectors, K, mean_pos_all, N, idx, n_g, &p, C));
    *ok = p.ok;
    const double g[12] = {p.u[0], p.u[1], p.u[2], p.k0[0], p.k0[1], p.k0[2], p.x_c, p.h_x, p.width, (double)p.interval, p.d_bound, p.dscale};
    std::memcpy(geo, g, sizeof(g));
    if (p.ok && kappa) std::memcpy(kappa, p.kappa, sizeof(p.kappa));
    if (p.ok && L) std::memcpy(L, p.L.data(), p.L.size() * sizeof(float));
    if (p.ok && phi) std::memcpy(phi, p.phi.data(), p.phi.size() * sizeof(float));
    return PSA_OK;
}

}
```

psa_amd/csrc/api_project.hip:

```cpp
#include "api_internal.h"

namespace psa {

uint64_t hash_idx(const int32_t* p, int64_t n) {
    uint64_t h = 1469598103934665603ull ^ (uint64_t)n;
    for (int64_t i = 0; i < n; ++i) h = (h ^ (uint32_t)p[i]) * 1099511628211ull;
    return h;
}

void fold_pairs(const float* k, int64_t K, std::vector<int32_t>* kmap, std::vector<int32_t>* unique_idx) {
    struct Key {
        uint32_t x, y, z;
        bool operator==(const Key& o) const { return x == o.x && y == o.y && z == o.z; }
    };
    struct KeyHash {
        size_t operator()(const Key& a) const {
            uint64_t h = 1469598103934665603ull;
            for (uint32_t v : {a.x, a.y, a.z}) h = (h ^ v) * 1099511628211ull;
            return (size_t)h;
        }
    };
    auto bits = [](float v, bool negate) {
        if (negate) v = -v;
        if (v == 0.f) v = 0.f;
        uint32_t u;
        std::memcpy(&u, &v, sizeof(u));
        return u;
    };
    std::unordered_map<Key, int32_t, KeyHash> seen;
    seen.reserve((size_t)K * 2);
    kmap->assign((size_t)K, 0);
    unique_idx->clear();
    for (int64_t i = 0; i < K; ++i) {
        const float* v = k + 3 * i;
        const bool   has_nan = v[0] != v[0] || v[1] != v[1] || v[2] != v[2];
        const Key    same{bits(v[0], false), bits(v[1], false), bits(v[2], false)};
        const Key    neg{bits(v[0], true), bits(v[1], true), bits(v[2], true)};
        if (!has_nan) {
            auto it = seen.find(same);
            if (it != seen.end()) {
                (*kmap)[i] = it->second;
                continue;
            }
            it = seen.find(neg);
            if (it != seen.end()) {
                (*kmap)[i] = it->second | KMAP_MIRROR;
                continue;
            }
        }
        const int32_t row = (int32_t)unique_idx->size();
        unique_idx->push_back((int32_t)i);
        (*kmap)[i] = row;
        if (!has_nan) seen.emplace(same, row);
    }
}

static bool fold_k_list(psa_ctx* c, const float* k, int64_t K, std::vector<float>* uniq_k, std::vector<int32_t>* kmap) {
    if (!c->opt_fold_pairs || K < 2 || K >= (1ll << 30)) return false;
    std::vector<int32_t> uidx;
    fold_pairs(k, K, kmap, &uidx);
    if ((int64_t)uidx.size() == K) return false;
    uniq_k->resize(uidx.size() * 3);
    for (size_t u = 0; u < uidx.size(); ++u) std::memcpy(uniq_k->data() + 3 * u, k + 3 * (size_t)uidx[u], 3 * sizeof(float));
    return true;
}

int install_kmap(psa_ctx* c, const std::vector<int32_t>& kmap) {
    c->kmap = kmap;
    c->out_K = (int64_t)kmap.size();
    c->out_valid = false;
    return upload(c, c->d_kmap, c->kmap.data(), c->kmap.size() * sizeof(int32_t));
}

size_t planes_bytes_held(psa_ctx* c) {
    size_t b = 0;
    for (auto& ps : c->planes) b += ps->buf.cap;
    return b;
}

void drop_stale_planes(psa_ctx* c) {
    auto& v = c->planes;
    v.erase(std::remove_if(v.begin(), v.end(),
                           [&](const std::unique_ptr<PlaneSet>& ps) {
                               const DataSlot& s = c->slot[ps->slot];
                               if (s.valid && s.generation == ps->generation) return false;
                               ps->buf.release();
                               return true;
                           }),
            v.end());
}

bool evict_one_plane_set(psa_ctx* c) {
    int victim = -1;
    for (size_t i = 0; i < c->planes.size(); ++i)
        if (c->planes[i]->last_use < c->plane_call_mark &&
            (victim < 0 || c->planes[i]->last_use < c->planes[victim]->last_use))
            victim = (int)i;
    if (victim < 0) return false;
    c->planes[victim]->buf.release();
    c->planes.erase(c->planes.begin() + victim);
    return true;
}

int get_planes(psa_ctx* c, const GroupView& v, int64_t K_local, const float* mean_host, PlaneSet** out) {
    *out = nullptr;
    if (c->k1_selector != PSA_K1_AUTO || !c->opt_planes) return PSA_OK;
    const int      slot = v.slot;
    const int32_t* h_idx = v.h_idx;
    const int64_t  n_g = v.n_g;
    DataSlot&      s = c->slot[slot];
    drop_stale_planes(c);
    const bool     all = h_idx == nullptr, displaced = mean_host != nullptr;
    const uint64_t h = (all ? 0 : hash_idx(h_idx, n_g)) ^ (displaced ? 0x9E3779B97F4A7C15ull : 0);
    const size_t   n_mean = (size_t)s.N * 3;
    for (auto& ps : c->planes)
        if (ps->slot == slot && ps->all_atoms == all && ps->n_g == n_g && ps->displaced == displaced &&
            (all || (ps->idx_hash == h && std::memcmp(ps->idx.data(), h_idx, (size_t)n_g * sizeof(int32_t)) == 0)) &&
            (!displaced || (ps->mean.size() == n_mean && std::memcmp(ps->mean.data(), mean_host, n_mean * sizeof(float)) == 0))) {
            ps->last_use = ++c->plane_tick;
            *out = ps.get();
            return PSA_OK;
        }
    if (K_local < c->opt_planes_min_k) return PSA_OK;
    if (!all && !c->opt_planes_eager) {
        auto& seen = c->seen_groups;
        if (std::find(seen.begin(), seen.end(), h) == seen.end()) {
            seen.push_back(h);
            if (seen.size() > 256) seen.erase(seen.begin());
            return PSA_OK;
        }
    }
    unsigned bits = 0;
    if (displaced) {
        PSA_TRY(displaced_absmax(c, slot, mean_host, h_idx, n_g, &bits));
    } else if (all) {
        PSA_TRY(slot_absmax(c, slot));
        bits = s.absmax_bits;
    } else {
        PSA_TRY(group_absmax(c, slot, h_idx, n_g, &bits));
    }
    const float vscale = k1_f16_vscale(bits);
    if (!(vscale > 0.f)) return PSA_OK;
    const int     A_pad = k1_pair_atom_pad(n_g);
    const int64_t n_fg = (s.T + 15) / 16;
    const size_t  bytes = plane_bytes(n_fg, A_pad / K1_BA);
    size_t        free_b = 0, total_b = 0;
    PSA_HIP_CHECK(hipMemGetInfo(&free_b, &total_b));
    const size_t budget = c->opt_planes_budget > 0 ? (size_t)c->opt_planes_budget : (size_t)(0.45 * (double)total_b);
    if (bytes > budget) return PSA_OK;
    while (planes_bytes_held(c) + bytes > budget)
        if (!evict_one_plane_set(c)) return PSA_OK;
    const size_t reserve = (size_t)2 << 30;
    while (free_b < bytes + reserve) {
        if (!evict_one_plane_set(c)) return PSA_OK;
        PSA_HIP_CHECK(hipMemGetInfo(&free_b, &total_b));
    }
    auto ps = std::make_unique<PlaneSet>();
    if (ps->buf.reserve(bytes) != PSA_OK) {
        (void)hipGetLastError();
        return PSA_OK;
    }
    {
        HostTimer ht(&c->oneoff_ms[2]);
        PSA_HIP_CHECK(hipStreamSynchronize(c->stream));
        PSA_TRY(launch_split_planes(c, s.buf.as<float>(), displaced ? c->d_mean_all.as<float>() : nullptr, v.d_idx, ps->buf.ptr,
                                    s.T, s.N, (int)n_g, A_pad, vscale));
        PSA_HIP_CHECK(hipStreamSynchronize(c->stream));
    }
    ps->slot = slot;
    ps->generation = s.generation;
    ps->all_atoms = all;
    if (!all) ps->idx.assign(h_idx, h_idx + n_g);
    ps->idx_hash = h;
    ps->displaced = displaced;
    if (displaced) ps->mean.assign(mean_host, mean_host + n_mean);
    ps->T = s.T;
    ps->n_fg = n_fg;
    ps->n_g = (int)n_g;
    ps->A_pad = A_pad;
    ps->vscale = vscale;
    ps->last_use = ++c->plane_tick;
    *out = ps.get();
    c->planes.push_back(std::move(ps));
    return PSA_OK;
}

int check_weights(psa_ctx* c, int64_t N) {
    PSA_REQUIRE(c->weights_N == 0 || c->weights_N == N, "atom weights were set for %lld atoms, the trajectory has %lld",
                (long long)c->weights_N, (long long)N);
    return PSA_OK;
}

void set_geom_weights(const psa_ctx* c, ProjGeom* g) {
    g->weights = c->weights_N ? c->d_weights.as<float>() : nullptr;
    g->wscale = c->weights_N ? c->weights_scale : 1.f;
}

int make_geom(psa_ctx* c, const GroupView& v, int64_t K_local, GeomRule rule, ProjGeom* g) {
    const int     slot = v.slot;
    const int64_t n_g = v.n_g;
    set_geom_weights(c, g);
    g->T = c->slot[slot].T;
    g->q_stride = g->T;
    g->N_tot = c->slot[slot].N;
    PSA_REQUIRE(n_g < (1ll << 30) && K_local < (1ll << 29), "group or k-list too large");
    g->n_g = (int)n_g;
    g->A_pad = (int)((n_g + 31) / 32 * 32);
    g->K = (int)K_local;
    g->split = K1Family::f32;
    const bool autosel = c->k1_selector == PSA_K1_AUTO;
    if (v.ps && rule == GeomRule::product) {
        g->split = K1Family::f16_planes;
        g->vscale = v.ps->vscale;
        g->m_blk = k1_planes_block_rows((int)K_local, c->opt_k1_wide != 0);
        g->A_pad = v.ps->A_pad;
        g->M_pad = (int)((2 * K_local + g->m_blk - 1) / g->m_blk * g->m_blk);
        return PSA_OK;
    }
    if (rule == GeomRule::product && autosel && k1_pair_eligible(v.d_idx, g->N_tot, n_g, K_local, v.disp)) {
        unsigned bits = 0;
        if (v.h_idx) {
            PSA_TRY(group_absmax(c, slot, v.h_idx, n_g, &bits));
        } else {
            PSA_TRY(slot_absmax(c, slot));
            bits = c->slot[slot].absmax_bits;
        }
        g->vscale = k1_f16_vscale(bits);
        if (g->vscale > 0.f) g->split = K1Family::f16_fly;
    }
    if (g->split == K1Family::f32 && rule != GeomRule::f32_only && (autosel || c->k1_selector == PSA_K1_SPLIT_BF16) &&
        k1_split_eligible(v.d_idx, g->N_tot, n_g, v.disp))
        g->split = K1Family::bf16;
    if (g->split == K1Family::f16_fly) {
        g->m_blk = k1_pair_block_rows((int)K_local);
        g->A_pad = k1_pair_atom_pad(n_g);
    } else {
        g->m_blk = g->split == K1Family::bf16 ? k1_split_block_rows((int)K_local) : k1_mfma_block_rows((int)K_local);
    }
    g->M_pad = (int)((2 * K_local + g->m_blk - 1) / g->m_blk * g->m_blk);
    return PSA_OK;
}

int prepare_phase(psa_ctx* c, const GroupView& v, const ProjGeom& g, int64_t k_first) {
    const int*   d_idx = v.d_idx;
    const float* d_kvec = c->d_kvec.as<float>() + 3 * k_first;
    const bool   f16 = g.split == K1Family::f16_fly || g.split == K1Family::f16_planes, bf16 = g.split == K1Family::bf16;
    if (g.lowrank) {
        PSA_TRY(c->d_lr_diff.reserve(pd16_table_bytes(g.M_pad_d, g.A_pad)));
        PSA_TRY(c->d_phase.reserve(pf16_table_bytes(128, g.A_pad)));
        StageTimer    st(c, PSA_T_PHASE);
        const double* f64 = c->d_lr_f64.as<double>();
        return launch_lowrank_tables(c, d_kvec, f64 + 7 + LOWRANK_NODES, f64, f64 + 7, c->d_mean_all.as<float>(), d_idx,
                                     c->d_lr_diff.ptr, c->d_phase.ptr, g, g.M_pad_d, g.dscale);
    }
    PSA_TRY(c->d_phase.reserve(f16    ? pf16_table_bytes(g.M_pad, g.A_pad)
                               : bf16 ? pb_table_bytes(g.M_pad, g.A_pad)
                                      : p_table_floats(g.M_pad, g.A_pad) * sizeof(float)));
    StageTimer st(c, PSA_T_PHASE);
    if (f16)
        PSA_TRY(launch_phase_table_f16(c, d_kvec, c->d_mean_all.as<float>(), d_idx, c->d_phase.ptr, g));
    else if (bf16)
        PSA_TRY(launch_phase_table_split(c, d_kvec, c->d_mean_all.as<float>(), d_idx, c->d_phase.ptr, g));
    else
        PSA_TRY(launch_phase_table(c, d_kvec, c->d_mean_all.as<float>(), d_idx, c->d_phase.as<float>(), g));
    if (v.disp) {
        PSA_TRY(c->d_mean_g.reserve((size_t)g.A_pad * 3 * sizeof(float)));
        PSA_TRY(launch_gather_mean(c, c->d_mean_all.as<float>(), d_idx, c->d_mean_g.as<float>(), g));
    }
    return PSA_OK;
}

static int launch_projection_once(psa_ctx* c, const GroupView& v, ProjGeom g, float2* d_q, int64_t q_stride, int64_t t_begin,
                                  int64_t t_count);

int launch_projection(psa_ctx* c, const GroupView& v, ProjGeom g, float2* d_q, int64_t q_stride, int64_t t_begin,
                      int64_t t_count) {
    static const int reps = [] {
        const char* e = std::getenv("PSA_DEBUG_REPEAT_K1");
        return e ? std::max(1, std::atoi(e)) : 1;
    }();
    for (int r = 0; r < reps; ++r) PSA_TRY(launch_projection_once(c, v, g, d_q, q_stride, t_begin, t_count));
    return PSA_OK;
}

static int launch_projection_once(psa_ctx* c, const GroupView& v, ProjGeom g, float2* d_q, int64_t q_stride, int64_t t_begin,
                                  int64_t t_count) {
    const DataSlot& s = c->slot[v.slot];
    const PlaneSet* ps = v.ps;
    PSA_REQUIRE(t_begin >= 0 && t_count > 0 && t_begin + t_count <= s.T && q_stride >= t_begin + t_count,
                "frame range [%lld,%lld) outside the slot", (long long)t_begin, (long long)(t_begin + t_count));
    g.T = t_count;
    g.q_stride = q_stride;
    StageTimer   st(c, PSA_T_PROJECT);
    const float* d_v = s.buf.as<float>() + (size_t)t_begin * 3 * (size_t)s.N;
    d_q += t_begin;
    if (g.split == K1Family::f16_planes) {
        PSA_REQUIRE(ps != nullptr && t_begin % 16 == 0, "planes are cut in groups of 16 frames");
        const int64_t fg0 = t_begin / 16, n_fg = ps->n_fg - fg0;
        const _Float16* pl = ps->buf.as<_Float16>() + (size_t)fg0 * (size_t)(ps->A_pad / K1_BA) * PL_STAGE_ELEMS;
        if (g.lowrank) {
            ProjGeom gn = g;
            gn.K = LOWRANK_NODES;
            gn.m_blk = gn.M_pad = 2 * LOWRANK_NODES;
            gn.q_stride = t_count;
            PSA_REQUIRE(c->d_lr_qn.cap >= (size_t)LOWRANK_NODES * 3 * t_count * sizeof(float2), "node projections not reserved");
            PSA_TRY(launch_k1_planes_lw(c, pl, c->d_phase.ptr, c->d_lr_qn.as<float2>(), gn, n_fg));
            ProjGeom gd = g;
            gd.M_pad = g.M_pad_d;
            PSA_TRY(launch_k1_planes_diff(c, pl, c->d_lr_diff.ptr, d_q, gd, n_fg, g.dscale));
            PSA_TRY(launch_lowrank_combine_r(c, c->d_lr_qn.as<float2>(), c->d_lr_L.as<float>(), c->d_lr_phi.as<float2>(), d_q, g,
                                             t_count));
            ++c->lowrank_launches;
            return PSA_OK;
        }
        if (g.m_blk == 256) return launch_k1_planes_wide(c, pl, c->d_phase.ptr, d_q, g, n_fg);
        if (g.m_blk == 128 && c->opt_k1_loader_waves) return launch_k1_planes_lw(c, pl, c->d_phase.ptr, d_q, g, n_fg);
        return launch_k1_planes(c, pl, c->d_phase.ptr, d_q, g, n_fg);
    }
    if (g.split == K1Family::f16_fly) return launch_k1_pair(c, d_v, c->d_phase.ptr, v.d_idx, d_q, g);
    if (g.split == K1Family::bf16) return launch_k1_split(c, d_v, c->d_phase.ptr, v.d_idx, d_q, g);
    if (c->k1_selector == PSA_K1_WAVE)
        return launch_k1_wave(c, d_v, c->d_phase.as<float>(), v.d_idx, c->d_mean_g.as<float>(), d_q, g, v.disp);
    return launch_k1_mfma(c, d_v, c->d_phase.as<float>(), v.d_idx, c->d_mean_g.as<float>(), d_q, g, v.disp);
}

int prepare_block(psa_ctx* c, const GroupView& v, GeomRule rule, const ProjectArgs* lowrank, int64_t k_first, int64_t nk,
                  ProjGeom* g) {
    PSA_TRY(make_geom(c, v, nk, rule, g));
    if (lowrank) PSA_TRY(prepare_lowrank(c, v, *lowrank, k_first, nk, g));
    return prepare_phase(c, v, *g, k_first);
}

int project_block(psa_ctx* c, const GroupView& v, const ProjectArgs* lowrank, int64_t k_first, int64_t nk, float2* d_q) {
    const int64_t T = c->slot[v.slot].T;
    ProjGeom      g;
    PSA_TRY(prepare_block(c, v, GeomRule::product, lowrank, k_first, nk, &g));
    return launch_projection(c, v, g, d_q, T, 0, T);
}

int group_source(psa_ctx* c, GroupView* v, const float* mean_host, int64_t K) {
    PSA_TRY(get_planes(c, *v, K, v->disp ? mean_host : nullptr, &v->ps));
    if (v->ps) {
        v->disp = false;
        return PSA_OK;
    }
    return materialise_displacements(c, v, mean_host);
}

int check_group_indices(const GroupView& v, int64_t N) {
    for (int64_t i = 0; v.h_idx && i < v.n_g; ++i)
        PSA_REQUIRE(v.h_idx[i] >= 0 && v.h_idx[i] < N, "Atom indices in basis out of bounds.");
    return PSA_OK;
}

int upload_single_group(psa_ctx* c, GroupView* v, int64_t N, const float* k_vectors, int64_t K, const float* mean_pos_all) {
    if (v->n_g == 0) return PSA_OK;
    PSA_TRY(upload(c, c->d_kvec, k_vectors, (size_t)K * 3 * sizeof(float)));
    PSA_TRY(upload(c, c->d_mean_all, mean_pos_all, (size_t)N * 3 * sizeof(float)));
    if (v->h_idx) PSA_TRY(upload(c, c->d_idx, v->h_idx, (size_t)v->n_g * sizeof(int32_t)));
    v->d_idx = v->h_idx ? c->d_idx.as<int>() : nullptr;
    return PSA_OK;
}

int check_project_args(psa_ctx* c, const ProjectArgs& a, int64_t N) {
    PSA_REQUIRE(a.mean_pos_all != nullptr, "null mean_pos_all");
    PSA_REQUIRE(a.K_local >= 0 && a.K_total >= 1 && a.k_offset >= 0 && a.k_offset + a.K_local <= a.K_total,
                "k range [%lld,%lld) outside [0,%lld)", (long long)a.k_offset, (long long)(a.k_offset + a.K_local),
                (long long)a.K_total);
    PSA_REQUIRE(a.K_local == 0 || a.k_vectors != nullptr, "null k_vectors");
    PSA_TRY(validate_groups(N, a.group_idx, a.group_off, a.G));
    PSA_REQUIRE((a.flags & PSA_F_INTENSITY) || a.G == 1, "complex output needs exactly one atom group (got %d)", a.G);
    (void)c;
    return PSA_OK;
}

int begin_result(psa_ctx* c, int64_t T, int64_t K_total, int64_t k_offset, bool intensity, char** rows) {
    PSA_TRY(c->d_slab.reserve(row_bytes(T, intensity) * (size_t)K_total));
    c->res_T = T;
    c->res_K = K_total;
    c->res_intensity = intensity;
    c->slab_valid = true;
    c->out_valid = false;
    c->inten_valid = false;
    c->kmap.clear();
    c->out_K = K_total;
    c->plane_call_mark = c->plane_tick + 1;
    *rows = (char*)c->d_slab.ptr + row_bytes(T, intensity) * (size_t)k_offset;
    return PSA_OK;
}

int upload_project_inputs(psa_ctx* c, const ProjectArgs& a, int64_t N) {
    StageTimer st(c, PSA_T_H2D);
    PSA_TRY(upload(c, c->d_kvec, a.k_vectors, (size_t)a.K_local * 3 * sizeof(float)));
    PSA_TRY(upload(c, c->d_mean_all, a.mean_pos_all, (size_t)N * 3 * sizeof(float)));
    if (a.group_idx) PSA_TRY(upload(c, c->d_idx, a.group_idx, (size_t)a.group_off[a.G] * sizeof(int32_t)));
    return PSA_OK;
}

int check_segments(psa_ctx* c, int64_t T, int32_t flags) {
    if (c->seg_L == 0) return PSA_OK;
    PSA_REQUIRE(flags & PSA_F_INTENSITY, "segment-averaged spectra are intensities: PSA_F_INTENSITY is required while segments are set");
    PSA_REQUIRE(c->seg_L <= T, "segment length %lld exceeds the trajectory's %lld frames", (long long)c->seg_L, (long long)T);
    return PSA_OK;
}

static int64_t result_frames(const psa_ctx* c, int64_t T) { return c->seg_L ? c->seg_L : T; }

static void segment_blocks(const psa_ctx* c, int64_t T, int64_t K_local, int64_t* nk, int64_t* ns) {
    const int64_t n_seg = 1 + (T - c->seg_L) / c->seg_hop;
    const int64_t units = std::max<int64_t>(1, K_local * T / c->seg_L);
    if (units >= n_seg) {
        *ns = n_seg;
        *nk = std::max<int64_t>(1, std::min(K_local, units / n_seg));
    } else {
        *ns = units;
        *nk = 1;
    }
}

static int segment_stage(psa_ctx* c, const float2* d_q, int64_t T, int64_t K_local, float* rows, bool first) {
    const int64_t L = c->seg_L, H = c->seg_hop, n_seg = 1 + (T - L) / H;
    int64_t       nk = 0, ns = 0;
    segment_blocks(c, T, K_local, &nk, &ns);
    const float inv_norm = (float)(1.0 / ((double)n_seg * c->seg_U));
    PSA_TRY(c->d_seg.reserve((size_t)nk * 3 * (size_t)ns * (size_t)L * sizeof(float2)));
    float2* d_seg = c->d_seg.as<float2>();
    for (int64_t k0 = 0; k0 < K_local; k0 += nk) {
        const int64_t bk = std::min(nk, K_local - k0);
        for (int64_t s0 = 0; s0 < n_seg; s0 += ns) {
            const int64_t bs = std::min(ns, n_seg - s0);
            {
                StageTimer st(c, PSA_T_EPILOGUE);
                PSA_TRY(launch_segment_window(c, d_q + (size_t)k0 * 3 * (size_t)T, c->d_seg_window.as<float>(), d_seg, T, L, H, s0,
                                              bs, bk));
            }
            {
                StageTimer st(c, PSA_T_FFT);
                PSA_TRY(run_fft(c, d_seg, L, 3 * bk * bs));
            }
            StageTimer st(c, PSA_T_EPILOGUE);
            PSA_TRY(launch_segment_power(c, d_seg, rows + (size_t)k0 * (size_t)L, L, bs, bk, inv_norm, first && s0 == 0));
        }
    }
    return PSA_OK;
}

static int spectrum_stage(psa_ctx* c, float2* d_q, int64_t T, int64_t K_local, bool intensity, float* rows, bool first) {
    if (c->seg_L) return segment_stage(c, d_q, T, K_local, rows, first);
    {
        StageTimer st(c, PSA_T_FFT);
        PSA_TRY(run_fft(c, d_q, T, 3 * K_local));
    }
    if (intensity) {
        StageTimer st(c, PSA_T_EPILOGUE);
        PSA_TRY(launch_intensity_accumulate(c, d_q, rows, T, K_local, first));
    }
    return PSA_OK;
}

static int project_groups(psa_ctx* c, const ProjectArgs& a, int g_first, bool* first, char* rows, float2* d_q) {
    const int64_t T = c->slot[a.slot].T, N = c->slot[a.slot].N;
    for (int gi = g_first; gi < a.G; ++gi) {
        GroupView v{a.slot, (a.flags & PSA_F_DISPLACEMENTS) != 0};
        set_group(c, a.group_idx, a.group_off, gi, N, &v);
        if (v.n_g == 0) continue;
        PSA_TRY(group_source(c, &v, a.mean_pos_all, a.K_local));
        const int64_t per_k = 8 * ((v.n_g + 63) / 64 * 64);
        int64_t       table = (int64_t)2 << 30;
        if (const char* e = std::getenv("PSA_PHASE_TABLE_MIB")) table = (int64_t)std::max(1, std::atoi(e)) << 20;
        int64_t kb = std::max<int64_t>(64, (table / per_k) / 64 * 64);
        if (a.K_local <= kb + 64) kb = a.K_local;
        for (int64_t k0 = 0; k0 < a.K_local; k0 += kb)
            PSA_TRY(project_block(c, v, &a, k0, std::min(kb, a.K_local - k0), d_q + (size_t)k0 * 3 * (size_t)T));
        PSA_TRY(spectrum_stage(c, d_q, T, a.K_local, (a.flags & PSA_F_INTENSITY) != 0, (float*)rows, *first));
        *first = false;
    }
    return PSA_OK;
}

static int begin_list(psa_ctx* c, ProjectArgs* a, std::vector<float>* uniq_k, std::vector<int32_t>* kmap, char** rows,
                      float2** d_q) {
    const int64_t T = c->slot[a->slot].T, N = c->slot[a->slot].N;
    const bool    intensity = (a->flags & PSA_F_INTENSITY) != 0;
    const bool folded = a->K_local == a->K_total && a->k_offset == 0 && fold_k_list(c, a->k_vectors, a->K_local, uniq_k, kmap);
    if (folded) {
        a->k_vectors = uniq_k->data();
        a->K_local = a->K_total = (int64_t)uniq_k->size() / 3;
    }
    PSA_TRY(begin_result(c, result_frames(c, T), a->K_total, a->k_offset, intensity, rows));
    if (folded) PSA_TRY(install_kmap(c, *kmap));
    if (a->K_local == 0) return PSA_OK;
    PSA_TRY(upload_project_inputs(c, *a, N));
    *d_q = (float2*)*rows;
    if (intensity) {
        PSA_TRY(c->d_qwork.reserve((size_t)a->K_local * 3 * T * sizeof(float2)));
        *d_q = c->d_qwork.as<float2>();
    }
    return PSA_OK;
}

}

using namespace psa;

extern "C" {

int psa_set_atom_weights(psa_ctx* c, const float* w, int64_t N) {
    PSA_TRY(enter(c));
    Guard guard(c);
    if (w == nullptr) {
        c->weights_N = 0;
        c->weights_scale = 1.f;
        return PSA_OK;
    }
    PSA_REQUIRE(N >= 1 && N < (1ll << 31), "bad atom count %lld", (long long)N);
    float wmax = 0.f;
    for (int64_t a = 0; a < N; ++a) {
        PSA_REQUIRE(std::isfinite(w[a]), "atom weight %lld is not finite", (long long)a);
        wmax = std::max(wmax, std::fabs(w[a]));
    }
    int e = 0;
    if (wmax > 0.f) {
        const float m = std::frexp(wmax, &e);
        if (m == 0.5f) --e;
        e = std::min(127, std::max(-126, e));
    }
    c->weights_N = 0;
    PSA_TRY(upload(c, c->d_weights, w, (size_t)N * sizeof(float)));
    PSA_HIP_CHECK(hipStreamSynchronize(c->stream));
    c->weights_N = N;
    c->weights_scale = std::ldexp(1.f, e);
    return PSA_OK;
}

int psa_set_segments(psa_ctx* c, int64_t L, int64_t hop, const float* window) {
    PSA_TRY(enter(c));
    Guard guard(c);
    if (L == 0) {
        c->seg_L = c->seg_hop = 0;
        c->seg_U = 0.0;
        return PSA_OK;
    }
    PSA_REQUIRE(L >= 2 && L < (1ll << 31), "bad segment length %lld", (long long)L);
    PSA_REQUIRE(hop >= 1, "segment hop %lld < 1", (long long)hop);
    PSA_REQUIRE(window != nullptr, "null window");
    double u = 0.0;
    bool   boxcar = true;
    for (int64_t t = 0; t < L; ++t) {
        PSA_REQUIRE(std::isfinite(window[t]), "window value %lld is not finite", (long long)t);
        u += (double)window[t] * (double)window[t];
        boxcar = boxcar && window[t] == 1.0f;
    }
    u /= (double)L;
    PSA_REQUIRE(u > 0.0, "the window is zero everywhere (U = 0)");
    c->seg_L = 0;
    PSA_TRY(upload(c, c->d_seg_window, window, (size_t)L * sizeof(float)));
    PSA_HIP_CHECK(hipStreamSynchronize(c->stream));
    c->seg_L = L;
    c->seg_hop = hop;
    c->seg_U = u;
    c->seg_boxcar = boxcar;
    return PSA_OK;
}

int psa_sed_project(psa_ctx* c, int slot, const float* mean_pos_all, const float* k_vectors,
                    int64_t K_local, int64_t K_total, int64_t k_offset, const int32_t* group_idx,
                    const int64_t* group_off, int32_t G, int32_t flags) {
    PSA_TRY(enter(c));
    Guard guard(c);
    PSA_TRY(check_slot(c, slot));
    ProjectArgs   a{slot, mean_pos_all, k_vectors, K_local, K_total, k_offset, group_idx, group_off, G, flags};
    const int64_t T = c->slot[slot].T, N = c->slot[slot].N;
    PSA_TRY(check_project_args(c, a, N));
    PSA_TRY(check_weights(c, N));
    PSA_TRY(check_segments(c, T, flags));
    std::vector<float>   uniq_k;
    std::vector<int32_t> kmap;
    char*                rows = nullptr;
    float2*              d_q = nullptr;
    PSA_TRY(begin_list(c, &a, &uniq_k, &kmap, &rows, &d_q));
    if (a.K_local == 0) return PSA_OK;
    bool first = true;
    PSA_TRY(project_groups(c, a, 0, &first, rows, d_q));
    if (first)
        PSA_HIP_CHECK(hipMemsetAsync(rows, 0, row_bytes(c->res_T, c->res_intensity) * (size_t)a.K_local, c->stream));
    return PSA_OK;
}

int psa_sed_project_upload(psa_ctx* c, int slot, const float* host, int64_t T, int64_t N, const float* mean_pos_all,
                           const float* k_vectors, int64_t K, const int32_t* group_idx, const int64_t* group_off,
                           int32_t G, int32_t flags) {
    PSA_TRY(enter(c));
    PSA_REQUIRE(host != nullptr, "null host array");
    PSA_REQUIRE(K >= 1, "need at least one k-vector");
    Guard       guard(c);
    ProjectArgs a{slot, mean_pos_all, k_vectors, K, K, 0, group_idx, group_off, G, flags};
    PSA_REQUIRE(slot >= 0 && slot < PSA_NUM_SLOTS, "bad data slot %d", slot);
    PSA_REQUIRE(T > 0 && N > 0, "empty trajectory (T=%lld, N=%lld)", (long long)T, (long long)N);
    PSA_TRY(check_project_args(c, a, N));
    PSA_TRY(check_weights(c, N));
    PSA_TRY(check_segments(c, T, flags));
    PSA_TRY(data_alloc_locked(c, slot, T, N));
    c->slot[slot].valid = false;
    const bool         intensity = (flags & PSA_F_INTENSITY) != 0;
    const bool         disp = (flags & PSA_F_DISPLACEMENTS) != 0;
    std::vector<float>   uniq_k;
    std::vector<int32_t> kmap;
    char*                rows = nullptr;
    float2*              d_q = nullptr;
    PSA_TRY(begin_list(c, &a, &uniq_k, &kmap, &rows, &d_q));
    K = a.K_local;
    int64_t fft_len = T, fft_batch = 3 * K;
// ... 335 lines not shown
```

psa_amd/csrc/k1_planes_diff.hip:

```cpp
#include <utility>

#include "k1_f16.h"

namespace psa {

namespace {
constexpr int D_M_BLK = 512, D_T_BLK = 64, D_MT = 16, D_PERIOD = 40;
constexpr int D_STAGE_UNITS = 44, D_RING_UNITS = 160, D_EARLY = D_RING_UNITS - 3 * D_STAGE_UNITS;
constexpr int D_STAGE_BYTES = D_M_BLK * K1_BA * 2;
static_assert(D_EARLY == 28 && D_RING_UNITS % 4 == 0 && D_STAGE_UNITS % 4 == 0, "ring arithmetic");
constexpr auto d_unit_off = unit_off<D_STAGE_UNITS, D_RING_UNITS, D_PERIOD>;
}

__host__ __device__ inline size_t pd16_index(int m, int a, int n_stage) {
    const int row = m % D_M_BLK, rt = row >> 4, v = 2 * (rt & 15) + (rt >> 4), r = row & 15, al = a % K1_BA;
    return (((size_t)(m / D_M_BLK) * n_stage + a / K1_BA) * 32 + v) * (16 * K1_BA) + (size_t)r * K1_BA +
           (size_t)((((al >> 3) ^ pl_swizzle(r)) << 3) + (al & 7));
}
size_t pd16_table_bytes(int M_pad, int A_pad) { return ((size_t)M_pad * A_pad + 4 * (size_t)D_M_BLK * K1_BA) * 2; }

template <bool NT_V>
__global__ void __launch_bounds__(512, 2)
k1_planes_diff_kernel(const _Float16* __restrict__ planes, const _Float16* __restrict__ Db, float2* __restrict__ Q, int64_t T,
                      int64_t q_stride, int n_fg, int n_stage, int K, int n_mblk, int n_tblk, float qscale) {
    using PR = F16x2;
    using E8 = PR::v8;
    __shared__ __attribute__((aligned(16))) unsigned char smem[D_RING_UNITS * 1024];
    const unsigned lds0 = (unsigned)(size_t)(lds_u8*)smem;

    int mb, tb;
    if (!k1_block_map(n_mblk, n_tblk, mb, tb)) return;

    const int tid = threadIdx.x, lane = tid & 63;
    const int w = __builtin_amdgcn_readfirstlane(tid >> 6);
    const int wh = w >> 2, wf = w & 3;
    const int r16 = lane & 15, q = lane >> 4;

    const unsigned char* src[11];
    {
        int fg = tb * 4 + (w & 3);
        if (fg >= n_fg) fg = n_fg - 1;
        const unsigned char* pl0 = reinterpret_cast<const unsigned char*>(planes) + (size_t)fg * n_stage * PL_STAGE_BYTES;
#pragma unroll
        for (int i = 0; i < 3; ++i) src[i] = pl0 + 1024 * (2 * i);
        const unsigned char* d0 = reinterpret_cast<const unsigned char*>(Db) + (size_t)mb * n_stage * D_STAGE_BYTES;
#pragma unroll
        for (int i = 3; i < 11; ++i) src[i] = d0 + 1024 * ((w & 3) + 4 * (i - 3));
    }
    const unsigned dma_voff = 16 * lane;
    const unsigned wbase = lds0 + 1024 * (w & 3);
    using std::integral_constant;
    auto dma = [&](auto s40_c, auto i_c) __attribute__((always_inline)) {
        constexpr int      S40 = decltype(s40_c)::value, I = decltype(i_c)::value;
        constexpr unsigned OFF = d_unit_off(S40, 4 * I);
        if constexpr (I < 3) {
            lds_dma16_at<OFF, NT_V>(src[I], dma_voff, wbase);
            src[I] += PL_STAGE_BYTES;
        } else {
            lds_dma16_at<OFF, false>(src[I], dma_voff, wbase);
            src[I] += D_STAGE_BYTES;
        }
    };
    auto dma_range = [&]<int S40, int... Is>(integral_constant<int, S40>, std::integer_sequence<int, Is...>) __attribute__((always_inline)) {
        (dma(integral_constant<int, S40>{}, integral_constant<int, Is>{}), ...);
    };
    auto dma_late = [&](auto s40_c) __attribute__((always_inline)) {
        dma_range(s40_c, std::integer_sequence<int, 7, 8, 9, 10>{});
    };
    auto dma_early = [&](auto s40_c) __attribute__((always_inline)) {
        dma_range(s40_c, std::make_integer_sequence<int, 7>{});
    };

    const unsigned lane_off = lds0 + r16 * (K1_BA * 2) + ((q ^ pl_swizzle(r16)) << 4);
    unsigned       lane_a[3], lane_b[3];
    unit_ring_windows(lane_off + 1024 * wh, lane_off + 1024 * wf, lane_a, lane_b);
    E8    a[4];
    E8    bf[3];
    f32x4 acc[D_MT][3];
    auto  read_a = [&](auto s40_c, auto mt_c) __attribute__((always_inline)) {
        constexpr int S40 = decltype(s40_c)::value, MTI = decltype(mt_c)::value;
        a[MTI & 3] = lds_frag(lane_a, d_unit_off(S40, 12 + 2 * MTI));
    };
    auto read_b = [&](auto s40_c, auto c_c) __attribute__((always_inline)) {
        constexpr int S40 = decltype(s40_c)::value, CC = decltype(c_c)::value;
        bf[CC] = lds_frag(lane_b, d_unit_off(S40, 4 * CC));
    };
#pragma unroll
    for (int mt = 0; mt < D_MT; ++mt)
#pragma unroll
        for (int c = 0; c < 3; ++c) acc[mt][c] = f32x4{0.f, 0.f, 0.f, 0.f};

    using I0 = integral_constant<int, 0>;
    using I1 = integral_constant<int, 1>;
    using I2 = integral_constant<int, 2>;
    if (wh == 0) {
        dma_early(I0{});
        dma_late(I0{});
        dma_early(I1{});
        dma_late(I1{});
        dma_early(I2{});
    }
    asm volatile("s_waitcnt vmcnt(7)\n\ts_barrier" ::: "memory");
    read_b(I0{}, I0{});
    read_b(I0{}, I1{});
    read_b(I0{}, I2{});
    read_a(I0{}, I0{});
    read_a(I0{}, I1{});

    int  left = n_stage;
    auto stage = [&](auto s40_c) __attribute__((always_inline)) {
        constexpr int S40 = decltype(s40_c)::value;
        if (left <= S40) return;
        using SN = integral_constant<int, (S40 + 1) % D_PERIOD>;
        using SNN = integral_constant<int, (S40 + 2) % D_PERIOD>;
        using S3 = integral_constant<int, (S40 + 3) % D_PERIOD>;
        if (wh == 0) {
            dma_late(SNN{});
            dma_early(S3{});
        }
        auto tile = [&](auto mt_c) __attribute__((always_inline)) {
            constexpr int MTI = decltype(mt_c)::value;
            if constexpr (MTI + 2 < D_MT)
                read_a(s40_c, integral_constant<int, MTI + 2>{});
            else
                read_a(SN{}, integral_constant<int, MTI + 2 - D_MT>{});
            auto comp = [&](auto c_c) __attribute__((always_inline)) {
                constexpr int CC = decltype(c_c)::value;
                acc[MTI][CC] = PR::mma(a[MTI & 3], bf[CC], acc[MTI][CC]);
                if constexpr (MTI == D_MT - 1) read_b(SN{}, c_c);
            };
            comp(I0{});
            comp(I1{});
            comp(I2{});
            __builtin_amdgcn_sched_barrier(0);
        };
        [&]<int... Ms>(std::integer_sequence<int, Ms...>) __attribute__((always_inline)) { (tile(integral_constant<int, Ms>{}), ...); }(
            std::make_integer_sequence<int, D_MT>{});
        asm volatile("s_waitcnt vmcnt(7)\n\ts_barrier" ::: "memory");
    };
    for (; left > 0; left -= D_PERIOD)
        [&]<int... Ss>(std::integer_sequence<int, Ss...>) __attribute__((always_inline)) { (stage(integral_constant<int, Ss>{}), ...); }(
            std::make_integer_sequence<int, D_PERIOD>{});
    asm volatile("s_waitcnt vmcnt(0)" ::: "memory");

    const int lane_e = __builtin_amdgcn_mbcnt_hi(~0u, __builtin_amdgcn_mbcnt_lo(~0u, 0u));
    const int r16_e = lane_e & 15, q_e = lane_e >> 4;
    k1_store_q(Q, acc, wh * (D_M_BLK / 2) + mb * D_M_BLK, q_e, (int64_t)tb * D_T_BLK + wf * 16 + r16_e, T, K, q_stride, qscale);
}

int launch_k1_planes_diff(psa_ctx* c, const void* d_planes, const void* d_diff, float2* d_q, const ProjGeom& g, int64_t n_fg, float dscale) {
    PSA_REQUIRE(g.M_pad % D_M_BLK == 0 && g.M_pad >= 2 * g.K && g.M_pad > 0, "D pass: 512-row M blocks only");
    PSA_REQUIRE(dscale > 0.f, "planes do not cover the launch");
    return launch_planes_family(c, k1_planes_diff_kernel<true>, k1_planes_diff_kernel<false>, D_M_BLK, 512, "D pass", K1_BA, dscale,
                                d_planes, d_diff, d_q, g, n_fg);
}

__global__ void __launch_bounds__(256)
diff_table_kernel(const float* __restrict__ kvec, const double* __restrict__ kline, const float* __restrict__ mean_all,
                  const int* __restrict__ idx, const float* __restrict__ w, float wnorm, _Float16* __restrict__ Db, int K,
                  int n_g, int A_pad, float dscale) {
    const int a = blockIdx.y * 256 + threadIdx.x;
    const int k = blockIdx.x;
    if (a >= A_pad) return;
    float d[2] = {0.f, 0.f};
    if (k < K && a < n_g) {
        const int   src = idx ? idx[a] : a;
        const float rx = mean_all[3 * (size_t)src + 0], ry = mean_all[3 * (size_t)src + 1], rz = mean_all[3 * (size_t)src + 2];
        const float kx = kvec[3 * k + 0], ky = kvec[3 * k + 1], kz = kvec[3 * k + 2];
        const float arg = __fmaf_rn(kz, rz, __fmaf_rn(ky, ry, __fmul_rn(kx, rx)));
        float       cs[2];
        sincosf(arg, &cs[1], &cs[0]);
        const double th = kline[3 * k + 0] * (double)rx + kline[3 * k + 1] * (double)ry + kline[3 * k + 2] * (double)rz;
        double       se, ce;
        sincos(th, &se, &ce);
        const double wa = w ? (double)(w[src] * wnorm) : 1.0;
        d[0] = (float)(((double)cs[0] - ce) * (double)dscale * wa);
        d[1] = (float)(((double)cs[1] - se) * (double)dscale * wa);
    }
    const int n_stage = A_pad / K1_BA;
    Db[pd16_index(2 * k, a, n_stage)] = (_Float16)d[0];
    Db[pd16_index(2 * k + 1, a, n_stage)] = (_Float16)d[1];
}

__global__ void __launch_bounds__(256)
node_table_kernel(const double* __restrict__ geo, const double* __restrict__ kappa, const float* __restrict__ mean_all,
                  const int* __restrict__ idx, const float* __restrict__ w, float wnorm, _Float16* __restrict__ Pb, int n_g,
                  int A_pad) {
    const int a = blockIdx.y * 256 + threadIdx.x;
    const int l = blockIdx.x;
    if (a >= A_pad) return;
    double cs[2] = {0.0, 0.0};
    if (a < n_g) {
        const int    src = idx ? idx[a] : a;
        const double rx = mean_all[3 * (size_t)src + 0], ry = mean_all[3 * (size_t)src + 1], rz = mean_all[3 * (size_t)src + 2];
        const double th = (geo[0] * rx + geo[1] * ry + geo[2] * rz) + kappa[l] * ((geo[3] * rx + geo[4] * ry + geo[5] * rz) - geo[6]);
        sincos(th, &cs[1], &cs[0]);
        if (w) {
            const double wa = (double)(w[src] * wnorm);
            cs[0] *= wa;
            cs[1] *= wa;
        }
    }
    const int n_stage = A_pad / K1_BA;
#pragma unroll
    for (int ri = 0; ri < 2; ++ri) {
        const double   x = cs[ri] * (double)F16x2::P_SCALE;
        const _Float16 lead = (_Float16)(float)x;
        Pb[pf16_tile_index(0, 2 * l + ri, a, 128, n_stage)] = lead;
        Pb[pf16_tile_index(1, 2 * l + ri, a, 128, n_stage)] = (_Float16)(float)(x - (double)lead);
    }
}

int launch_lowrank_tables(psa_ctx* c, const float* d_kvec, const double* d_kline, const double* d_geo, const double* d_kappa,
                          const float* d_mean_all, const int* d_idx, void* d_diff, void* d_nodes, const ProjGeom& g, int M_pad_d,
                          float dscale) {
    PSA_REQUIRE(M_pad_d % D_M_BLK == 0 && M_pad_d >= 2 * g.K && g.A_pad % K1_BA == 0, "bad low-rank table geometry");
    hipLaunchKernelGGL(diff_table_kernel, dim3(M_pad_d / 2, (g.A_pad + 255) / 256), dim3(256), 0, c->stream, d_kvec, d_kline, d_mean_all,
                       d_idx, g.weights, 1.f / g.wscale, (_Float16*)d_diff, g.K, g.n_g, g.A_pad, dscale);
    PSA_HIP_CHECK(hipGetLastError());
    PSA_HIP_CHECK(hipMemsetAsync((char*)d_diff + (size_t)M_pad_d * g.A_pad * 2, 0, pd16_table_bytes(M_pad_d, g.A_pad) - (size_t)M_pad_d * g.A_pad * 2,
                                 c->stream));
    hipLaunchKernelGGL(node_table_kernel, dim3(LOWRANK_NODES, (g.A_pad + 255) / 256), dim3(256), 0, c->stream, d_geo, d_kappa, d_mean_all,
                       d_idx, g.weights, 1.f / g.wscale, (_Float16*)d_nodes, g.n_g, g.A_pad);
    PSA_HIP_CHECK(hipGetLastError());
    return PSA_OK;
}

}
```

psa_amd/csrc/psa_ctx.h:

```cpp
#pragma once
#include <hip/hip_runtime.h>
#include <rocfft/rocfft.h>
#include <rccl/rccl.h>

#include <cstdarg>
#include <cstdint>
#include <cstdio>
#include <map>
#include <memory>
#include <mutex>
#include <string>
#include <thread>
#include <utility>
#include <vector>

#include "psa_hip.h"

namespace psa {

void set_error(const char* fmt, ...);

#define PSA_HIP_CHECK(expr)                                                              \
    do {                                                                                 \
        hipError_t e_ = (expr);                                                          \
        if (e_ != hipSuccess) {                                                          \
            psa::set_error("%s:%d: %s -> %s", __FILE__, __LINE__, #expr,                 \
                           hipGetErrorString(e_));                                       \
            return PSA_EHIP;                                                             \
        }                                                                                \
    } while (0)

#define PSA_FFT_CHECK(expr)                                                              \
    do {                                                                                 \
        rocfft_status s_ = (expr);                                                       \
        if (s_ != rocfft_status_success) {                                               \
            psa::set_error("%s:%d: %s -> rocfft_status %d", __FILE__, __LINE__, #expr,   \
                           (int)s_);                                                     \
            return PSA_EFFT;                                                             \
        }                                                                                \
    } while (0)

#define PSA_NCCL_CHECK(expr)                                                             \
    do {                                                                                 \
        ncclResult_t r_ = (expr);                                                        \
        if (r_ != ncclSuccess) {                                                         \
            psa::set_error("%s:%d: %s -> %s", __FILE__, __LINE__, #expr,                 \
                           ncclGetErrorString(r_));                                      \
            return PSA_ERCCL;                                                            \
        }                                                                                \
    } while (0)

#define PSA_REQUIRE(cond, ...)                                                           \
    do {                                                                                 \
        if (!(cond)) {                                                                   \
            psa::set_error(__VA_ARGS__);                                                 \
            return PSA_EINVAL;                                                           \
        }                                                                                \
    } while (0)

#define PSA_TRY(expr)                                                                    \
    do {                                                                                 \
        int rc_ = (expr);                                                                \
        if (rc_ != PSA_OK) return rc_;                                                   \
    } while (0)

struct DevBuf {
    void*  ptr = nullptr;
    size_t cap = 0;
    int reserve(size_t bytes);
    void release();
    template <class T> T* as() const { return static_cast<T*>(ptr); }
};

struct FftPlan {
    rocfft_plan           plan = nullptr;
    rocfft_execution_info info = nullptr;
    size_t                work_bytes = 0;
};

struct DataSlot {
    DevBuf  buf;
    int64_t T = 0, N = 0;
    bool    valid = false;
    uint64_t generation = 0;
    bool     absmax_known = false;
    unsigned absmax_bits = 0;
    bool                  blocks_known = false;
    std::vector<unsigned> block_absmax;
};

struct Timed {
    int        stage;
    hipEvent_t e0, e1;
};
struct TimingState {
    std::vector<hipEvent_t> pool;
    std::vector<Timed>      pending;
    double                  acc[8] = {};
    int64_t                 k1_launches = 0;
    double                  k1_ms = 0.0;
};

constexpr int K1_BA   = 32;
constexpr int LOWRANK_NODES = 64;
constexpr int K1_VROW = 96;
constexpr int K1_PROW = 36;

__host__ __device__ inline size_t p_tile_index(int m, int a, int m_blk, int n_stage) {
    return ((size_t)(m / m_blk) * n_stage + (a / K1_BA)) * ((size_t)m_blk * K1_PROW) +
           (size_t)(m % m_blk) * K1_PROW + (a % K1_BA);
}
inline size_t p_table_floats(int M_pad, int A_pad) { return (size_t)M_pad * (A_pad / K1_BA) * K1_PROW; }

enum class K1Family : int {
    f32 = 0,
    f16_fly = 2,
    bf16 = 3,
    f16_planes = 4,
};

struct ProjGeom {
    int64_t T = 0;
    int64_t q_stride = 0;
    int64_t N_tot = 0;
    int     n_g = 0;
    int     A_pad = 0;
    int     K = 0;
    int     M_pad = 0;
    int     m_blk = 0;
    K1Family split = K1Family::f32;
    float   vscale = 0.f;
    bool    lowrank = false;
    int     M_pad_d = 0;
    float   dscale = 0.f;
    const float* weights = nullptr;
    float        wscale = 1.f;
};

struct PlaneSet {
    DevBuf               buf;
    int                  slot = 0;
    uint64_t             generation = 0;
    bool                 all_atoms = true;
    std::vector<int32_t> idx;
    uint64_t             idx_hash = 0;
    bool                 displaced = false;
    std::vector<float>   mean;
    int64_t              T = 0, n_fg = 0;
    int                  n_g = 0, A_pad = 0;
    float                vscale = 0.f;
    uint64_t             last_use = 0;
};

constexpr int KMAP_MIRROR = (int)0x80000000u;

struct Stager {
    void*       pin[2] = {nullptr, nullptr};
    size_t      cap = 0;
    hipEvent_t  freed[2] = {nullptr, nullptr};
    hipStream_t copy_stream = nullptr;
};

}

enum { PSA_T_H2D = 0, PSA_T_PHASE, PSA_T_PROJECT, PSA_T_FFT, PSA_T_EPILOGUE, PSA_T_GATHER,
       PSA_T_TRANSPOSE, PSA_T_D2H, PSA_T_COUNT };

struct psa_ctx {
    int         device = 0;
    hipStream_t stream = nullptr;
    std::mutex  mu;
    int         k1_selector = PSA_K1_AUTO;
    int         compute_units = 0;

    psa::DataSlot slot[PSA_NUM_SLOTS + 1];
    std::vector<float> disp_mean;
    uint64_t           disp_source = 0;
    std::vector<unsigned> disp_block_absmax;
    std::vector<float>    disp_abs_mean;
    uint64_t              disp_abs_source = ~0ull;

    psa::DevBuf d_kvec, d_mean_all, d_idx, d_mean_g, d_phase, d_qwork, d_fft_work, d_tables, d_absmax;
    psa::DevBuf d_upload_max;
    psa::DevBuf d_zeros;
    psa::DevBuf d_qrows, d_stage, d_bin;

    std::vector<std::unique_ptr<psa::PlaneSet>> planes;
    std::vector<uint64_t> seen_groups;
    uint64_t plane_tick = 0, plane_call_mark = 0;
    int64_t  opt_planes = 1, opt_planes_budget = 0, opt_planes_eager = 0, opt_planes_min_k = 17;
    psa::Stager stager;
    hipStream_t d2h_stream = nullptr;
    hipEvent_t  d2h_ready = nullptr;

    int64_t fs_T_total = 0, fs_T_local = 0, fs_K_total = 0, fs_rows_k0 = 0, fs_rows_nk = 0;
    bool    fs_intensity = false;
    psa::DevBuf d_slab;
    psa::DevBuf d_out;
    psa::DevBuf d_aux;
    int64_t res_T = 0, res_K = 0;
    bool    res_intensity = false;
    int64_t              out_K = 0;
    std::vector<int32_t> kmap;
    psa::DevBuf          d_kmap, d_cols;
    int64_t              opt_fold_pairs = 1;
    psa::DevBuf          d_inten;
    bool                 inten_valid = false;
    bool    slab_valid = false, out_valid = false;

    std::map<std::pair<int64_t, int64_t>, psa::FftPlan> plans;
    std::thread  fft_primer;
    psa::FftPlan primed;
    int64_t      primed_T = 0;
    int64_t      opt_fft_prime = 1;
    int64_t      opt_k1_wide = 1;
    int64_t      opt_k1_loader_waves = 1;
    int64_t      opt_k1_lowrank = 1;
    int64_t      opt_k1_lowrank_min_k = 256;
    int64_t      opt_k1_lowrank_min_local = 128;
    int64_t      lowrank_launches = 0;
    psa::DevBuf  d_lr_diff, d_lr_qn, d_lr_L, d_lr_phi, d_lr_f64;

    psa::DevBuf  d_weights;
    int64_t      weights_N = 0;
    float        weights_scale = 1.f;

    psa::DevBuf  d_seg_window, d_seg;
    int64_t      seg_L = 0, seg_hop = 0;
    double       seg_U = 0.0;
    bool         seg_boxcar = false;

    psa::DevBuf  d_vdos_work, d_vdos_pairs, d_vdos_off, d_vdos_mean, d_vdos_part, d_vdos_acc, d_vdos_out;
    int64_t      opt_vdos_work_bytes = (int64_t)1 << 30;

    psa::DevBuf  d_modes_work, d_modes_coef, d_modes_out;
    int64_t      opt_modes_work_bytes = (int64_t)4 << 30;

    psa::DevBuf  d_cov_slab, d_cov_g, d_cov_out;

    psa::DevBuf  d_peaks_spec, d_peaks_bands, d_peaks_part, d_peaks_fit, d_peaks_info;

    psa::DevBuf  d_dyn_q, d_dyn_kappa, d_dyn_khat, d_dyn_idx, d_dyn_out;
    int64_t      opt_dynamic_work_bytes = (int64_t)4 << 30;

    psa::DevBuf  d_lat_q, d_lat_tiles, d_lat_ent, d_lat_slot, d_lat_dest, d_lat_khat, d_lat_idx, d_lat_bins, d_lat_scale,
                 d_lat_acc, d_lat_out;

    psa::DevBuf  d_self_work, d_self_tiles, d_self_ent, d_self_slot, d_self_idx, d_self_groups, d_self_scale, d_self_part,
                 d_self_acc, d_self_out;

    psa::DevBuf  d_par_q, d_par_tiles, d_par_ent, d_par_slot, d_par_dest, d_par_khat, d_par_idx, d_par_bins, d_par_scale,
                 d_par_acc, d_par_out;

    psa::DevBuf  d_corr_tab, d_corr_factor, d_corr_scale, d_corr_in, d_corr_out;

    psa::DevBuf  d_msd_u, d_msd_img, d_msd_sums, d_msd_offs, d_msd_idx, d_msd_chunks, d_msd_sizes, d_msd_lags, d_msd_part,
                 d_msd_acc, d_msd_out;

    psa::DevBuf  d_pair_c, d_pair_idx, d_pair_items, d_pair_part, d_pair_acc;

    psa::TimingState timing;
    double oneoff_ms[4] = {0, 0, 0, 0};
    psa::DevBuf      d_sync;

    ncclComm_t comm = nullptr;
    int        rank = 0, nranks = 1;
};

namespace psa {

int launch_phase_table(psa_ctx* c, const float* d_kvec, const float* d_mean_all, const int* d_idx,
                       float* d_phase, const ProjGeom& g);
int launch_gather_mean(psa_ctx* c, const float* d_mean_all, const int* d_idx, float* d_mean_g,
                       const ProjGeom& g);
int launch_fill_synthetic(psa_ctx* c, float* d_v, int64_t T, int64_t N, uint64_t seed, int64_t t_offset, int n_modes,
                          const float* d_amp, const int* d_comp, const float* d_ct,
                          const float* d_st, const float* d_ca, const float* d_sa);
int launch_mean_over_frames(psa_ctx* c, const float* d_x, int64_t T, int64_t N, float* d_mean);
int launch_subtract_mean(psa_ctx* c, const float* d_x, const float* d_mean, float* d_out, int64_t T, int64_t N);
int launch_absmax_bits(psa_ctx* c, const float* d_x, int64_t n, unsigned* d_out, bool reset = true);
int launch_absmax_blocks(psa_ctx* c, const float* d_x, const float* d_mean, int64_t T, int64_t N, unsigned* d_out);

int  k1_mfma_block_rows(int K);
int  launch_k1_mfma(psa_ctx* c, const float* d_v, const float* d_phase, const int* d_idx,
                    const float* d_mean_g, float2* d_q, const ProjGeom& g, bool displacements);
int  launch_k1_wave(psa_ctx* c, const float* d_v, const float* d_phase, const int* d_idx,
                    const float* d_mean_g, float2* d_q, const ProjGeom& g, bool displacements);

bool   k1_split_eligible(const int* d_idx, int64_t N_tot, int64_t n_g, bool displacements);
int    k1_split_block_rows(int K);
size_t pb_table_bytes(int M_pad, int A_pad);
int    launch_phase_table_split(psa_ctx* c, const float* d_kvec, const float* d_mean_all, const int* d_idx,
                                void* d_phase, const ProjGeom& g);
int    launch_k1_split(psa_ctx* c, const float* d_v, const void* d_phase, const int* d_idx, float2* d_q,
                       const ProjGeom& g);

bool   k1_pair_eligible(const int* d_idx, int64_t N_tot, int64_t n_g, int64_t K, bool displacements);
int    k1_pair_atom_pad(int64_t n_g);
int    k1_pair_block_rows(int K);
float  k1_f16_vscale(unsigned absmax_bits);
size_t pf16_table_bytes(int M_pad, int A_pad);
int    launch_phase_table_f16(psa_ctx* c, const float* d_kvec, const float* d_mean_all, const int* d_idx,
                              void* d_phase, const ProjGeom& g);
int    launch_k1_pair(psa_ctx* c, const float* d_v, const void* d_phase, const int* d_idx, float2* d_q,
                      const ProjGeom& g);

int    k1_planes_block_rows(int K, bool wide);
int    launch_split_planes(psa_ctx* c, const float* d_x, const float* d_mean, const int* d_idx, void* d_planes, int64_t T,
                           int64_t N_tot, int n_g, int A_pad, float vscale);
int    launch_k1_planes(psa_ctx* c, const void* d_planes, const void* d_phase, float2* d_q, const ProjGeom& g,
                        int64_t n_fg);
int    launch_k1_planes_lw(psa_ctx* c, const void* d_planes, const void* d_phase, float2* d_q, const ProjGeom& g,
                           int64_t n_fg);

int    launch_k1_planes_wide(psa_ctx* c, const void* d_planes, const void* d_phase, float2* d_q, const ProjGeom& g,
                             int64_t n_fg);

size_t pd16_table_bytes(int M_pad, int A_pad);
int    launch_lowrank_tables(psa_ctx* c, const float* d_kvec, const double* d_kline, const double* d_geo, const double* d_kappa,
                             const float* d_mean_all, const int* d_idx, void* d_diff, void* d_nodes, const ProjGeom& g, int M_pad_d,
                             float dscale);
int    launch_k1_planes_diff(psa_ctx* c, const void* d_planes, const void* d_diff, float2* d_q, const ProjGeom& g, int64_t n_fg,
                             float dscale);

int    launch_lowrank_combine_r(psa_ctx* c, const float2* d_qn, const float* d_L, const float2* d_phi, float2* d_q, const ProjGeom& g,
                                int64_t qn_stride);

int launch_dft_bin(psa_ctx* c, const float2* d_q, int64_t T, int64_t bin, float2* d_out3);
int launch_scale_transpose_c64(psa_ctx* c, const float2* d_slab, float2* d_out, float* d_inten, int64_t T, int64_t n,
                               int64_t K_pitch, int64_t col_first, int64_t src_first, const int32_t* d_cols,
                               const int32_t* d_srcs);
int launch_intensity_accumulate(psa_ctx* c, const float2* d_q, float* d_slab_rows, int64_t T,
                                int64_t K_local, bool first_group);
int launch_transpose_f32(psa_ctx* c, const float* d_slab, float* d_out, int64_t T, int64_t K, const int32_t* d_srcs);
int launch_segment_window(psa_ctx* c, const float2* d_q, const float* d_w, float2* d_seg, int64_t T, int64_t L, int64_t H,
                          int64_t s0, int64_t ns, int64_t nk);
int launch_segment_window_rows(psa_ctx* c, const float2* d_q, const float* d_w, float2* d_seg, int64_t T, int64_t L, int64_t H,
                               int64_t s0, int64_t ns, int64_t n_series);
int launch_segment_power(psa_ctx* c, const float2* d_seg, float* d_rows, int64_t L, int64_t ns, int64_t nk, float inv_norm,
                         bool first);
constexpr int VDOS_TILE_PAIRS = 32;
int launch_vdos_gather(psa_ctx* c, const float* d_data, const float* d_mean, const float* d_weights, const float* d_win,
                       const int* d_pair_atoms, float2* d_work, int64_t T, int64_t N, int64_t L, int64_t H, int64_t s0,
                       int64_t ns, int64_t n_pairs);
int launch_vdos_power(psa_ctx* c, const float2* d_work, const int64_t* d_pair_off, double* d_part, double* d_acc, int64_t L,
                      int64_t ns, int64_t n_pairs, int64_t p0, int64_t g_first, int64_t n_groups, int64_t n_chunks);
int launch_vdos_finish(psa_ctx* c, const double* d_acc, float* d_out, int64_t L, int64_t rows, double scale);
int modes_tile(int64_t M);
int launch_mode_power(psa_ctx* c, const float2* d_S, const float2* d_coef, float* d_out, int64_t L, int64_t ns, int64_t nk,
                      int64_t B, int64_t M, int MT, int64_t K_pitch, int64_t k_col0, float scale, bool first);
int64_t covariance_chunks(int64_t T);
int64_t covariance_slab_floats(int64_t T, int64_t n, int n_w);
int launch_covariance(psa_ctx* c, const float2* d_S, const float* d_g, float* d_slab, double2* d_out, int64_t T, int64_t nk, int64_t B,
                      int n_w, int64_t K_pitch, int64_t k_col0, double scale);
int peaks_slices(int64_t C, int64_t rows);
int launch_peak_find(psa_ctx* c, const float* d_spec, int64_t C, const int32_t* d_bands, int lo, int hi, int row0, int row_end,
                     int n_slices, float* d_pmax, int* d_pidx, int* d_pflag);
int launch_peak_fit(psa_ctx* c, const float* d_spec, int64_t C, const int32_t* d_bands, int lo, int hi, const float* d_pmax,
                    const int* d_pidx, const int* d_pflag, int n_slices, double df, float window_hwhm, int half_window_bins,
                    int max_iter, float* d_fit, int32_t* d_info);
constexpr int DYN_THREADS = 256;
constexpr int DYN_ATOMS = 512;
constexpr int DYN_CHAIN = 128;
constexpr int DYN_FRAMES = 4;
int dynamic_slices(int64_t K);
int launch_dynamic_project(psa_ctx* c, const float* d_pos, const float* d_vel, const float* d_weights, const int* d_idx,
                           const float* d_kappa, float2* d_q, int64_t T, int64_t N, int64_t n_g, int64_t nk, bool currents,
                           int slices);
int launch_dynamic_power(psa_ctx* c, const float2* d_seg, const float* d_khat, float* d_out, int64_t L, int64_t ns, int64_t nk,
                         bool currents, int64_t K_pitch, int64_t k_col0, float scale, bool first);
int launch_dynamic_sincos(psa_ctx* c, const float* d_turns, float2* d_out, int64_t n);
constexpr int LAT_THREADS = 256;
constexpr int LAT_KS = 512;
constexpr int LAT_ATOMS = 128;
constexpr int LAT_TABLE = 3584;
constexpr int LAT_CHAIN = 128;
constexpr int LAT_FRAMES = 4;
constexpr int LAT_MAX_INDEX = 64;
constexpr int LAT_MAX_ENTRIES = 3 * (2 * LAT_MAX_INDEX + 1);
int launch_lattice_project(psa_ctx* c, const float* d_pos, const float* d_vel, const float* d_weights, const int* d_idx,
                           const float* box_hi, const float* box_lo, const int* d_tile_off, const unsigned short* d_ent,
                           const unsigned* d_slot, const int* d_dest, float2* d_q, int64_t T, int64_t N, int64_t n_g, int64_t tile0,
                           int64_t n_tiles, bool currents);
int launch_lattice_shell(psa_ctx* c, const float2* d_seg, const float* d_khat, const int* d_bin_start, double* d_acc, int64_t L,
                         int64_t ns, int64_t g0, int64_t nb, int64_t n_bins, bool currents);
int launch_lattice_finish(psa_ctx* c, const double* d_acc, const double* d_scale, float* d_out, int64_t n, int64_t n_bins);
constexpr int PARTIAL_MAX_SPECIES = 8;
constexpr int PARTIAL_MAX_PAIRS = PARTIAL_MAX_SPECIES * (PARTIAL_MAX_SPECIES + 1) / 2;
int launch_partial_power(psa_ctx* c, const float2* d_seg, const float* d_khat, float* d_out, int64_t L, int64_t ns, int64_t nk,
                         int n_species, bool currents, int64_t K_pitch, int64_t k_col0, float scale, bool first);
int launch_partial_shell(psa_ctx* c, const float2* d_seg, const float* d_khat, const int* d_bin_start, double* d_acc, int64_t L,
                         int64_t ns, int64_t g0, int64_t nb, int64_t n_bins, int n_species, bool currents);
constexpr int SELF_THREADS = 256;
constexpr int SELF_ATOMS = 4;
constexpr int SELF_FRAMES = 64;
constexpr int SELF_ENTRIES = 24;
constexpr int SELF_KS = 64;
int launch_self_series(psa_ctx* c, const float* d_pos, const float* d_weights, const int* d_idx, int64_t a0, const float* box_hi,
                       const float* box_lo, const int* d_tile, const unsigned short* d_ent, const unsigned* d_slot, const float* d_win,
                       float2* d_work, int64_t T, int64_t N, int64_t na, int64_t tile0, int64_t n_tiles, int64_t v0, int64_t nv,
                       int64_t L, int64_t H, int64_t s0, int64_t ns, int64_t pitch);
int launch_self_power(psa_ctx* c, const float2* d_work, const int* d_groups, double* d_part, double* d_acc, int64_t L, int64_t ns,
                      int64_t na, int64_t v0, int64_t nv, int64_t g_first, int64_t ng, int64_t cols, int64_t n_chunks, bool mirror);
constexpr int CORR_LAGS = 8;
constexpr int CORR_COLS_MIN = 64;
int launch_correlation_pad(psa_ctx* c, const float2* d_q, float2* d_seg, int64_t T, int64_t L, int64_t P, int64_t H, int64_t s0,
                           int64_t ns, int64_t n_rows);
int launch_correlation_transform(psa_ctx* c, const double* d_X, const double* d_tab, const double* d_factor, const double* d_scale,
                                 float* d_out, int64_t fields, int64_t P, int64_t cols, int64_t n_lags);
int launch_correlation_transform(psa_ctx* c, const float* d_X, const double* d_tab, const double* d_factor, const double* d_scale,
                                 float* d_out, int64_t fields, int64_t P, int64_t cols, int64_t n_lags);
constexpr int MSD_LAGS = 256;
constexpr int MSD_ORIGINS = 1024;
constexpr int MSD_WINDOW = 1280;
constexpr int MSD_MAX_GROUPS = 8;
constexpr int MSD_MAX_BINS = 1024;
constexpr int MSD_MAX_VH_LAGS = 64;
constexpr int MSD_UNWRAP_FRAMES = 64;
constexpr int MSD_UNWRAP_ATOMS = 16;
int msd_origins(int64_t step);
int launch_msd_unwrap(psa_ctx* c, const float* d_pos, const int* d_idx, int64_t a0, int64_t na, const double* box,
                      const double* box_inverse, bool unwrap, int* d_sums, int* d_offs, double* d_u, int* d_img, int64_t T, int64_t N);
int launch_msd_moments(psa_ctx* c, const double* d_u, const void* d_chunks, int64_t n_chunks, double* d_part, int64_t T, int64_t n_lags,
                       int64_t step, int64_t n_os);
int launch_msd_moments_reduce(psa_ctx* c, const double* d_part, const int32_t* group_first, double* d_acc, int64_t n_lags, int64_t n_os,
                              int32_t G);
int launch_msd_moments_finish(psa_ctx* c, const double* d_acc, const int64_t* d_group_size, double* d_out, int64_t T, int64_t n_lags,
                              int32_t G, int64_t step);
int launch_msd_hist(psa_ctx* c, const double* d_u, const void* d_chunks, int64_t n_chunks, const int64_t* d_lags, int64_t n_vh,
                    unsigned* d_part, int64_t T, int64_t step, int64_t n_os, float inv_dr, int32_t n_r);
int launch_msd_hist_reduce(psa_ctx* c, const unsigned* d_part, const int32_t* group_first, unsigned long long* d_acc, int64_t n_vh,
                           int64_t n_os, int32_t n_r, int32_t G);
constexpr int PAIR_TILE = 256;
constexpr int PAIR_MAX_BINS = 1024;
constexpr int PAIR_MAX_LAGS = 64;
constexpr int PAIR_MAX_SPECIES = 8;
struct PairItem {
    int a_lo, a_n, b_lo, b_hi, slab, n_os, diag, pair;
};
int launch_pair_frac(psa_ctx* c, const float* d_pos, const int* d_idx, int64_t n_a, const double* box_inverse, float* d_out, int64_t f0,
                     int64_t df, int64_t n_frames, int64_t T, int64_t N);
int launch_pair_hist(psa_ctx* c, const float* d_cA, const float* d_cB, const void* d_items, int64_t n_items, unsigned* d_part,
                     const double* box, int64_t n_a, int64_t n_ob, float inv_dr, int32_t n_r);
int launch_pair_hist_reduce(psa_ctx* c, const unsigned* d_part, const int32_t* pair_first, unsigned long long* d_acc, int32_t S,
                            int32_t n_r, bool sym);
int launch_result_intensity(psa_ctx* c, const float2* d_out, float* d_int, int64_t n_tk);
int launch_result_chiral_c(psa_ctx* c, const float2* d_out, float* d_phase, int64_t n_tk, int c1, int c2);

}
```

Baseline: 53930 billion.

## Fuse low-rank node and diff projections into one paired-role MFMA kernel

Adds a kernel in which one 512-row block computes the low-rank node projections (two-f16 split, hi/lo) together with the first 64 diff rows, while a second block computes the remaining 448 diff rows. Both roles are balanced to issue the same number of MFMAs per stage and stream from a shared LDS ring. A new pair-specific diff-table layout matches the two roles. The aim is to replace two separate launches with one and overlap the small node GEMM with the diff GEMM, avoiding the underutilised node-only launch and a second pass over the planes. The path is used only when the diff table is exactly one 512-row block, it adds complex hand-scheduled code, and the new layout risks indexing errors.

```diff
diff --git a/include/psa_hip.h b/include/psa_hip.h
--- a/include/psa_hip.h
+++ b/include/psa_hip.h
@@ -54,6 +54,7 @@
 #define PSA_OPT_VDOS_WORK_BYTES 11
 #define PSA_OPT_MODES_WORK_BYTES 12
 #define PSA_OPT_DYNAMIC_WORK_BYTES 13
+#define PSA_OPT_K1_LOWRANK_PAIR 15
 int         psa_set_option(psa_ctx* ctx, int option, int64_t value);
 int         psa_device_info(psa_ctx* ctx, char* name, int name_len,
                             int* compute_units, int64_t* hbm_bytes);
@@ -195,6 +196,8 @@
 int psa_last_timings(psa_ctx* ctx, double* ms );
 int psa_k1_stats(psa_ctx* ctx, int64_t* launches, double* total_ms);
 int psa_k1_lowrank_launches(psa_ctx* ctx, int64_t* launches);
+int psa_k1_lowrank_pair_launches(psa_ctx* ctx, int64_t* launches);
+int psa_lowrank_pair_image(int32_t n_stage, int64_t* index, int64_t* bytes);
 int psa_oneoff_stats(psa_ctx* ctx, double* ms );
 
 int psa_debug_phase_table(psa_ctx* ctx, const float* mean_pos_all,
diff --git a/psa_amd/_hip.py b/psa_amd/_hip.py
--- a/psa_amd/_hip.py
+++ b/psa_amd/_hip.py
@@ -23,6 +23,7 @@
 OPT_VDOS_WORK_BYTES = 11
 OPT_MODES_WORK_BYTES = 12
 OPT_DYNAMIC_WORK_BYTES = 13
+OPT_K1_LOWRANK_PAIR = 15
 KMAP_MIRROR = 0x80000000
 ABI_VERSION = 6
 COV_CHAIN = 128
@@ -161,6 +162,8 @@
     "psa_last_timings": (C.c_int, [_ctx, C.POINTER(C.c_double)]),
     "psa_k1_stats": (C.c_int, [_ctx, _i64p, C.POINTER(C.c_double)]),
     "psa_k1_lowrank_launches": (C.c_int, [_ctx, _i64p]),
+    "psa_k1_lowrank_pair_launches": (C.c_int, [_ctx, _i64p]),
+    "psa_lowrank_pair_image": (C.c_int, [C.c_int32, _i64p, _i64p]),
     "psa_oneoff_stats": (C.c_int, [_ctx, C.POINTER(C.c_double)]),
     "psa_debug_phase_table": (C.c_int, [_ctx, _f32p, _f32p, C.c_int64, _i32p, C.c_int64,
                                         C.c_int64, C.c_void_p]),
@@ -275,6 +278,12 @@
         return None
     return {"u": geo[0:3].copy(), "k0": geo[3:6].copy(), "x_c": geo[6], "h_x": geo[7], "width": geo[8],
             "interval": int(geo[9]), "d_bound": geo[10], "dscale": geo[11], "kappa": kappa, "C": cm, "L": lw, "phi": phi}
+
+
+def lowrank_pair_image(n_stage: int):
+    index, nbytes = np.zeros((512, 32 * int(n_stage)), np.int64), C.c_int64(0)
+    _check(load_library().psa_lowrank_pair_image(int(n_stage), index.ctypes.data_as(_i64p), C.byref(nbytes)), "psa_lowrank_pair_image")
+    return index, nbytes.value
 
 
 def host_mean_frames(x: np.ndarray, threads: int = 0) -> np.ndarray:
@@ -1126,6 +1135,11 @@
         _check(self._lib.psa_k1_lowrank_launches(self._h, C.byref(n)), "psa_k1_lowrank_launches")
         return n.value
 
+    def lowrank_pair_launches(self) -> int:
+        n = C.c_int64(0)
+        _check(self._lib.psa_k1_lowrank_pair_launches(self._h, C.byref(n)), "psa_k1_lowrank_pair_launches")
+        return n.value
+
     def debug_phase_table(self, mean_pos_all, k_vectors, idx=None) -> np.ndarray:
         mean = _as_f32(mean_pos_all, (3,))
         kv = _as_f32(k_vectors, (3,))
diff --git a/psa_amd/csrc/api_core.hip b/psa_amd/csrc/api_core.hip
--- a/psa_amd/csrc/api_core.hip
+++ b/psa_amd/csrc/api_core.hip
@@ -334,6 +334,7 @@
                 for (psa::DevBuf* b : {&c->d_lr_diff, &c->d_lr_qn, &c->d_lr_L, &c->d_lr_phi, &c->d_lr_f64}) b->release();
             }
             return PSA_OK;
+        case PSA_OPT_K1_LOWRANK_PAIR: c->opt_k1_lowrank_pair = value != 0; return PSA_OK;
         case PSA_OPT_K1_LOWRANK_MIN_LOCAL:
             PSA_REQUIRE(value >= 1, "PSA_OPT_K1_LOWRANK_MIN_LOCAL must be >= 1");
             c->opt_k1_lowrank_min_local = value;
@@ -403,6 +404,13 @@
     return PSA_OK;
 }
 
+int psa_k1_lowrank_pair_launches(psa_ctx* c, int64_t* launches) {
+    PSA_TRY(enter(c));
+    PSA_REQUIRE(launches != nullptr, "null argument");
+    *launches = c->lowrank_pair_launches;
+    return PSA_OK;
+}
+
 int psa_k1_stats(psa_ctx* c, int64_t* launches, double* total_ms) {
     PSA_TRY(enter(c));
     Guard guard(c);
diff --git a/psa_amd/csrc/api_lowrank.hip b/psa_amd/csrc/api_lowrank.hip
--- a/psa_amd/csrc/api_lowrank.hip
+++ b/psa_amd/csrc/api_lowrank.hip
@@ -1,4 +1,5 @@
 #include "api_internal.h"
+#include "k1_lowrank_pair.h"
 
 namespace psa {
 
@@ -178,6 +179,7 @@
     g->lowrank = true;
     g->dscale = p.dscale;
     g->M_pad_d = (int)((2 * nk + 511) / 512 * 512);
+    g->lr_pair = c->opt_k1_lowrank_pair && g->M_pad_d == LRP_ROWS;
     return PSA_OK;
 }
 
@@ -203,4 +205,13 @@
     return PSA_OK;
 }
 
-}
+int psa_lowrank_pair_image(int32_t n_stage, int64_t* index, int64_t* bytes) {
+    PSA_REQUIRE(n_stage >= 1 && n_stage < (1 << 20) && bytes, "bad argument");
+    *bytes = (int64_t)pd16_pair_table_bytes(n_stage);
+    if (index)
+        for (int m = 0; m < LRP_ROWS; ++m)
+            for (int a = 0; a < n_stage * K1_BA; ++a) index[(size_t)m * n_stage * K1_BA + a] = (int64_t)pd16_pair_index(m, a, n_stage);
+    return PSA_OK;
+}
+
+}
diff --git a/psa_amd/csrc/api_project.hip b/psa_amd/csrc/api_project.hip
--- a/psa_amd/csrc/api_project.hip
+++ b/psa_amd/csrc/api_project.hip
@@ -251,7 +251,7 @@
         StageTimer    st(c, PSA_T_PHASE);
         const double* f64 = c->d_lr_f64.as<double>();
         return launch_lowrank_tables(c, d_kvec, f64 + 7 + LOWRANK_NODES, f64, f64 + 7, c->d_mean_all.as<float>(), d_idx,
-                                     c->d_lr_diff.ptr, c->d_phase.ptr, g, g.M_pad_d, g.dscale);
+                                     c->d_lr_diff.ptr, c->d_phase.ptr, g, g.M_pad_d, g.dscale, g.lr_pair);
     }
     PSA_TRY(c->d_phase.reserve(f16    ? pf16_table_bytes(g.M_pad, g.A_pad)
                                : bf16 ? pb_table_bytes(g.M_pad, g.A_pad)
@@ -304,10 +304,15 @@
             gn.m_blk = gn.M_pad = 2 * LOWRANK_NODES;
             gn.q_stride = t_count;
             PSA_REQUIRE(c->d_lr_qn.cap >= (size_t)LOWRANK_NODES * 3 * t_count * sizeof(float2), "node projections not reserved");
-            PSA_TRY(launch_k1_planes_lw(c, pl, c->d_phase.ptr, c->d_lr_qn.as<float2>(), gn, n_fg));
-            ProjGeom gd = g;
-            gd.M_pad = g.M_pad_d;
-            PSA_TRY(launch_k1_planes_diff(c, pl, c->d_lr_diff.ptr, d_q, gd, n_fg, g.dscale));
+            if (g.lr_pair) {
+                PSA_TRY(launch_k1_lowrank_pair(c, pl, c->d_phase.ptr, c->d_lr_diff.ptr, c->d_lr_qn.as<float2>(), d_q, g, n_fg, g.dscale));
+                ++c->lowrank_pair_launches;
+            } else {
+                PSA_TRY(launch_k1_planes_lw(c, pl, c->d_phase.ptr, c->d_lr_qn.as<float2>(), gn, n_fg));
+                ProjGeom gd = g;
+                gd.M_pad = g.M_pad_d;
+                PSA_TRY(launch_k1_planes_diff(c, pl, c->d_lr_diff.ptr, d_q, gd, n_fg, g.dscale));
+            }
             PSA_TRY(launch_lowrank_combine_r(c, c->d_lr_qn.as<float2>(), c->d_lr_L.as<float>(), c->d_lr_phi.as<float2>(), d_q, g,
                                              t_count));
             ++c->lowrank_launches;
diff --git a/psa_amd/csrc/k1_lowrank_pair.h b/psa_amd/csrc/k1_lowrank_pair.h
--- /dev/null
+++ b/psa_amd/csrc/k1_lowrank_pair.h
@@ -0,0 +1,28 @@
+#pragma once
+#include "k1_tile.h"
+
+namespace psa {
+
+constexpr int LRP_ROWS = 512;
+constexpr int LRP_A_ROWS = 64, LRP_A_UNITS = 4;
+constexpr int LRP_B_MT = 14, LRP_B_UNITS = 2 * LRP_B_MT;
+constexpr int LRP_PAD_STAGES = 4;
+static_assert(LRP_A_ROWS + 16 * LRP_B_UNITS == LRP_ROWS, "the two roles share the block's rows");
+
+__host__ __device__ inline size_t lrp_b_first_unit(int n_stage) { return (size_t)(n_stage + LRP_PAD_STAGES) * LRP_A_UNITS; }
+__host__ __device__ inline size_t pd16_pair_index(int m, int a, int n_stage) {
+    const int rt = m >> 4, r = m & 15, al = a % K1_BA, st = a / K1_BA;
+    size_t    unit;
+    if (rt < LRP_A_UNITS) {
+        unit = (size_t)st * LRP_A_UNITS + (size_t)(2 * (rt & 1) + (rt >> 1));
+    } else {
+        const int rb = rt - LRP_A_UNITS, h = rb / LRP_B_MT, mt = rb % LRP_B_MT;
+        unit = lrp_b_first_unit(n_stage) + (size_t)st * LRP_B_UNITS + (size_t)(2 * mt + h);
+    }
+    return unit * (16 * K1_BA) + (size_t)r * K1_BA + (size_t)((((al >> 3) ^ pl_swizzle(r)) << 3) + (al & 7));
+}
+__host__ __device__ inline size_t pd16_pair_table_bytes(int n_stage) {
+    return (size_t)(n_stage + LRP_PAD_STAGES) * (LRP_A_UNITS + LRP_B_UNITS) * 1024;
+}
+
+}
diff --git a/psa_amd/csrc/k1_lowrank_pair.hip b/psa_amd/csrc/k1_lowrank_pair.hip
--- /dev/null
+++ b/psa_amd/csrc/k1_lowrank_pair.hip
@@ -0,0 +1,304 @@
+#include <utility>
+
+#include "k1_f16.h"
+#include "k1_lowrank_pair.h"
+
+namespace psa {
+
+namespace {
+constexpr int LP_T_BLK = 64, LP_RING_UNITS = 160;
+constexpr int LPA_STAGE_UNITS = 44, LPA_PERIOD = 40, LPA_FOLD = 8, LPA_MT = 4, LPA_DT = LRP_A_UNITS / 2;
+constexpr int LPA_NODE_U0 = 24, LPA_D_U0 = 40;
+constexpr int LPA_EARLY = LP_RING_UNITS - 3 * LPA_STAGE_UNITS;
+constexpr int LPB_STAGE_UNITS = 12 + LRP_B_UNITS, LPB_PERIOD = LP_RING_UNITS / LPB_STAGE_UNITS, LPB_D_U0 = 12;
+constexpr int LP_NODE_STAGE_BYTES = pf16_stage_bytes(2 * LOWRANK_NODES);
+static_assert(LPA_EARLY == 28 && LPA_PERIOD % LPA_FOLD == 0 && LPA_D_U0 + LRP_A_UNITS == LPA_STAGE_UNITS, "role A's ring");
+static_assert(LPB_STAGE_UNITS == 40 && LPB_PERIOD == 4, "role B's ring is four whole stages");
+static_assert(3 * 3 * LPA_MT + 3 * LPA_DT == 3 * LRP_B_MT, "both roles multiply the same per stage: 42 MFMAs per wavefront");
+constexpr auto a_unit_off = unit_off<LPA_STAGE_UNITS, LP_RING_UNITS, LPA_PERIOD>;
+constexpr auto b_unit_off = unit_off<LPB_STAGE_UNITS, LP_RING_UNITS, LPB_PERIOD>;
+}
+
+__global__ void __launch_bounds__(512, 2)
+k1_lowrank_pair_kernel(const _Float16* __restrict__ planes, const _Float16* __restrict__ Pn, const _Float16* __restrict__ Dp,
+                       float2* __restrict__ Qn, float2* __restrict__ Q, int64_t T, int64_t q_stride, int n_fg, int n_stage, int K,
+                       int n_tblk, float qscale_n, float qscale_d) {
+    using PR = F16x2;
+    using E8 = PR::v8;
+    using std::integral_constant;
+    __shared__ __attribute__((aligned(16))) unsigned char smem[LP_RING_UNITS * 1024];
+    const unsigned lds0 = (unsigned)(size_t)(lds_u8*)smem;
+
+    int mb, tb;
+    if (!k1_block_map(2, n_tblk, mb, tb)) return;
+
+    const int tid = threadIdx.x, lane = tid & 63;
+    const int w = __builtin_amdgcn_readfirstlane(tid >> 6);
+    const int wh = w >> 2, wf = w & 3;
+    const int r16 = lane & 15, q = lane >> 4;
+
+    int fg = tb * 4 + wf;
+    if (fg >= n_fg) fg = n_fg - 1;
+    const unsigned char* pl0 = reinterpret_cast<const unsigned char*>(planes) + (size_t)fg * n_stage * PL_STAGE_BYTES;
+    const unsigned dma_voff = 16 * lane;
+    const unsigned wbase = lds0 + 1024 * wf;
+    const unsigned lane_off = lds0 + r16 * (K1_BA * 2) + ((q ^ pl_swizzle(r16)) << 4);
+    unsigned       lane_a[3], lane_b[3];
+    unit_ring_windows(lane_off + 1024 * wh, lane_off + 1024 * wf, lane_a, lane_b);
+    using I0 = integral_constant<int, 0>;
+    using I1 = integral_constant<int, 1>;
+    using I2 = integral_constant<int, 2>;
+
+    if (mb == 0) {
+        const unsigned char* src[11];
+#pragma unroll
+        for (int i = 0; i < 6; ++i) src[i] = pl0 + 1024 * i;
+#pragma unroll
+        for (int j = 0; j < 4; ++j) {
+            const int x = 4 * j + wf;
+            src[6 + j] = reinterpret_cast<const unsigned char*>(Pn) + 1024 * (8 * (x >> 3) + 4 * (x & 1) + ((x >> 1) & 3));
+        }
+        src[10] = reinterpret_cast<const unsigned char*>(Dp) + 1024 * wf;
+        auto dma = [&](auto s40_c, auto i_c) __attribute__((always_inline)) {
+            constexpr int      S40 = decltype(s40_c)::value, I = decltype(i_c)::value;
+            constexpr unsigned OFF = a_unit_off(S40, 4 * I);
+            if constexpr (I < 6) {
+                lds_dma16_at<OFF, (I & 1) != 0>(src[I], dma_voff, wbase);
+                src[I] += PL_STAGE_BYTES;
+            } else if constexpr (I < 10) {
+                lds_dma16_at<OFF, false>(src[I], dma_voff, wbase);
+                src[I] += LP_NODE_STAGE_BYTES;
+            } else {
+                lds_dma16_at<OFF, false>(src[I], dma_voff, wbase);
+                src[I] += LRP_A_UNITS * 1024;
+            }
+        };
+        auto dma_range = [&]<int S40, int... Is>(integral_constant<int, S40>, std::integer_sequence<int, Is...>) __attribute__((always_inline)) {
+            (dma(integral_constant<int, S40>{}, integral_constant<int, Is>{}), ...);
+        };
+        auto dma_late = [&](auto s40_c) __attribute__((always_inline)) { dma_range(s40_c, std::integer_sequence<int, 7, 8, 9, 10>{}); };
+        auto dma_early = [&](auto s40_c) __attribute__((always_inline)) { dma_range(s40_c, std::make_integer_sequence<int, 7>{}); };
+
+        E8    a[2][2][LPA_MT];
+        E8    ad[2][LPA_DT];
+        E8    bb[3][2];
+        f32x4 hi[LPA_MT][3], lo[LPA_MT][3], accd[LPA_DT][3];
+        auto  read_a = [&](auto s40_c, auto p_c, auto mt_c) __attribute__((always_inline)) {
+            constexpr int S40 = decltype(s40_c)::value, P = decltype(p_c)::value, MTI = decltype(mt_c)::value;
+            a[S40 & 1][P][MTI] = lds_frag(lane_a, a_unit_off(S40, LPA_NODE_U0 + 8 * P + 2 * MTI));
+        };
+        auto read_ad = [&](auto s40_c, auto mt_c) __attribute__((always_inline)) {
+            constexpr int S40 = decltype(s40_c)::value, MTI = decltype(mt_c)::value;
+            ad[S40 & 1][MTI] = lds_frag(lane_a, a_unit_off(S40, LPA_D_U0 + 2 * MTI));
+        };
+        auto read_b = [&](auto s40_c, auto c_c, auto p_c) __attribute__((always_inline)) {
+            constexpr int S40 = decltype(s40_c)::value, CC = decltype(c_c)::value, P = decltype(p_c)::value;
+            bb[CC][P] = lds_frag(lane_b, a_unit_off(S40, 4 * (2 * CC + P)));
+        };
+        auto each_mt = [&](auto&& f) __attribute__((always_inline)) {
+            f(I0{});
+            f(I1{});
+            f(I2{});
+            f(integral_constant<int, 3>{});
+        };
+        static_assert(LPA_PERIOD % 2 == 0, "the fragment sets alternate with the stage");
+#pragma unroll
+        for (int mt = 0; mt < LPA_MT; ++mt)
+#pragma unroll
+            for (int c = 0; c < 3; ++c) {
+                hi[mt][c] = f32x4{0.f, 0.f, 0.f, 0.f};
+                lo[mt][c] = f32x4{0.f, 0.f, 0.f, 0.f};
+            }
+#pragma unroll
+        for (int mt = 0; mt < LPA_DT; ++mt)
+#pragma unroll
+            for (int c = 0; c < 3; ++c) accd[mt][c] = f32x4{0.f, 0.f, 0.f, 0.f};
+
+        if (wh == 0) {
+            dma_early(I0{});
+            dma_late(I0{});
+            dma_early(I1{});
+            dma_late(I1{});
+            dma_early(I2{});
+        }
+        asm volatile("s_waitcnt vmcnt(7)\n\ts_barrier" ::: "memory");
+        each_mt([&](auto mt_c) __attribute__((always_inline)) {
+            read_a(I0{}, I1{}, mt_c);
+            read_a(I0{}, I0{}, mt_c);
+        });
+        read_b(I0{}, I0{}, I0{});
+        read_b(I0{}, I0{}, I1{});
+        read_ad(I0{}, I0{});
+        read_ad(I0{}, I1{});
+        read_b(I0{}, I1{}, I0{});
+        read_b(I0{}, I1{}, I1{});
+        read_b(I0{}, I2{}, I0{});
+        read_b(I0{}, I2{}, I1{});
+
+        int  left = n_stage;
+        auto stage = [&](auto s40_c) __attribute__((always_inline)) {
+            constexpr int S40 = decltype(s40_c)::value, PAR = S40 & 1;
+            if (left <= S40) return;
+            constexpr bool restart = S40 % LPA_FOLD == 0;
+            using SN = integral_constant<int, (S40 + 1) % LPA_PERIOD>;
+            using SNN = integral_constant<int, (S40 + 2) % LPA_PERIOD>;
+            using S3 = integral_constant<int, (S40 + 3) % LPA_PERIOD>;
+            if (wh == 0) {
+                dma_late(SNN{});
+                dma_early(S3{});
+            }
+            auto comp = [&](auto c_c) __attribute__((always_inline)) {
+                constexpr int CC = decltype(c_c)::value;
+                f32x4         ch[LPA_MT];
+                each_mt([&](auto mt_c) __attribute__((always_inline)) {
+                    constexpr int MTI = decltype(mt_c)::value;
+                    ch[MTI] = PR::mma(a[PAR][1][MTI], bb[CC][0], restart ? f32x4{0.f, 0.f, 0.f, 0.f} : hi[MTI][CC]);
+                });
+                if constexpr (CC == 0) each_mt([&](auto mt_c) __attribute__((always_inline)) { read_a(SN{}, I1{}, mt_c); });
+                if constexpr (CC == 1) {
+                    read_ad(SN{}, I0{});
+                    read_ad(SN{}, I1{});
+                }
+                __builtin_amdgcn_sched_barrier(0);
+                each_mt([&](auto mt_c) __attribute__((always_inline)) {
+                    constexpr int MTI = decltype(mt_c)::value;
+                    ch[MTI] = PR::mma(a[PAR][0][MTI], bb[CC][1], ch[MTI]);
+                });
+                read_b(SN{}, c_c, I1{});
+                if constexpr (CC == 0) each_mt([&](auto mt_c) __attribute__((always_inline)) { read_a(SN{}, I0{}, mt_c); });
+                __builtin_amdgcn_sched_barrier(0);
+                accd[0][CC] = PR::mma(ad[PAR][0], bb[CC][0], accd[0][CC]);
+                accd[1][CC] = PR::mma(ad[PAR][1], bb[CC][0], accd[1][CC]);
+                each_mt([&](auto mt_c) __attribute__((always_inline)) {
+                    constexpr int MTI = decltype(mt_c)::value;
+                    hi[MTI][CC] = PR::mma(a[PAR][0][MTI], bb[CC][0], ch[MTI]);
+                });
+                read_b(SN{}, c_c, I0{});
+                __builtin_amdgcn_sched_barrier(0);
+            };
+            comp(I0{});
+            comp(I1{});
+            comp(I2{});
+            asm volatile("s_waitcnt vmcnt(7)\n\ts_barrier" ::: "memory");
+        };
+        auto chain = [&](auto c_c) __attribute__((always_inline)) {
+            constexpr int C0 = decltype(c_c)::value * LPA_FOLD;
+            if (left <= C0) return;
+            [&]<int... Ss>(std::integer_sequence<int, Ss...>) __attribute__((always_inline)) { (stage(integral_constant<int, C0 + Ss>{}), ...); }(
+                std::make_integer_sequence<int, LPA_FOLD>{});
+            k1_fold(lo, hi);
+        };
+        for (; left > 0; left -= LPA_PERIOD)
+            [&]<int... Cs>(std::integer_sequence<int, Cs...>) __attribute__((always_inline)) { (chain(integral_constant<int, Cs>{}), ...); }(
+                std::make_integer_sequence<int, LPA_PERIOD / LPA_FOLD>{});
+        asm volatile("s_waitcnt vmcnt(0)" ::: "memory");
+
+        const int     lane_e = __builtin_amdgcn_mbcnt_hi(~0u, __builtin_amdgcn_mbcnt_lo(~0u, 0u));
+        const int     r16_e = lane_e & 15, q_e = lane_e >> 4;
+        const int64_t t = (int64_t)tb * LP_T_BLK + wf * 16 + r16_e;
+        k1_store_q(Qn, lo, wh * LOWRANK_NODES, q_e, t, T, LOWRANK_NODES, T, qscale_n);
+        k1_store_q(Q, accd, wh * (LRP_A_ROWS / 2), q_e, t, T, K, q_stride, qscale_d);
+    } else {
+        const unsigned char* src[10];
+#pragma unroll
+        for (int i = 0; i < 3; ++i) src[i] = pl0 + 1024 * (2 * i);
+        const unsigned char* d0 = reinterpret_cast<const unsigned char*>(Dp) + lrp_b_first_unit(n_stage) * 1024;
+#pragma unroll
+        for (int i = 3; i < 10; ++i) src[i] = d0 + 1024 * (wf + 4 * (i - 3));
+        auto dma = [&](auto s4_c, auto i_c) __attribute__((always_inline)) {
+            constexpr int      S4 = decltype(s4_c)::value, I = decltype(i_c)::value;
+            constexpr unsigned OFF = b_unit_off(S4, 4 * I);
+            lds_dma16_at<OFF, false>(src[I], dma_voff, wbase);
+            src[I] += I < 3 ? PL_STAGE_BYTES : LRP_B_UNITS * 1024;
+        };
+        auto dma_stage = [&](auto s4_c) __attribute__((always_inline)) {
+            [&]<int... Is>(std::integer_sequence<int, Is...>) __attribute__((always_inline)) { (dma(s4_c, integral_constant<int, Is>{}), ...); }(
+                std::make_integer_sequence<int, 10>{});
+        };
+
+        E8    a[4];
+        E8    bf[3];
+        f32x4 acc[LRP_B_MT][3];
+        auto read_a = [&](auto s4_c, auto mt_c) __attribute__((always_inline)) {
+            constexpr int S4 = decltype(s4_c)::value, MTI = decltype(mt_c)::value;
+            a[(LRP_B_MT * S4 + MTI) & 3] = lds_frag(lane_a, b_unit_off(S4, LPB_D_U0 + 2 * MTI));
+        };
+        auto read_b = [&](auto s4_c, auto c_c) __attribute__((always_inline)) {
+            constexpr int S4 = decltype(s4_c)::value, CC = decltype(c_c)::value;
+            bf[CC] = lds_frag(lane_b, b_unit_off(S4, 4 * CC));
+        };
+#pragma unroll
+        for (int mt = 0; mt < LRP_B_MT; ++mt)
+#pragma unroll
+            for (int c = 0; c < 3; ++c) acc[mt][c] = f32x4{0.f, 0.f, 0.f, 0.f};
+
+        if (wh == 0) {
+            dma_stage(I0{});
+            dma_stage(I1{});
+            dma_stage(I2{});
+        }
+        asm volatile("s_waitcnt vmcnt(10)\n\ts_barrier" ::: "memory");
+        read_b(I0{}, I0{});
+        read_b(I0{}, I1{});
+        read_b(I0{}, I2{});
+        read_a(I0{}, I0{});
+        read_a(I0{}, I1{});
+
+        int  left = n_stage;
+        auto stage = [&](auto s4_c) __attribute__((always_inline)) {
+            constexpr int S4 = decltype(s4_c)::value;
+            if (left <= S4) return;
+            using SN = integral_constant<int, (S4 + 1) % LPB_PERIOD>;
+            using S3 = integral_constant<int, (S4 + 3) % LPB_PERIOD>;
+            if (wh == 0) dma_stage(S3{});
+            auto tile = [&](auto mt_c) __attribute__((always_inline)) {
+                constexpr int MTI = decltype(mt_c)::value;
+                if constexpr (MTI + 2 < LRP_B_MT)
+                    read_a(s4_c, integral_constant<int, MTI + 2>{});
+                else
+                    read_a(SN{}, integral_constant<int, MTI + 2 - LRP_B_MT>{});
+                auto comp = [&](auto c_c) __attribute__((always_inline)) {
+                    constexpr int CC = decltype(c_c)::value;
+                    acc[MTI][CC] = PR::mma(a[(LRP_B_MT * S4 + MTI) & 3], bf[CC], acc[MTI][CC]);
+                    if constexpr (MTI == LRP_B_MT - 1) read_b(SN{}, c_c);
+                };
+                comp(I0{});
+                comp(I1{});
+                comp(I2{});
+                __builtin_amdgcn_sched_barrier(0);
+            };
+            [&]<int... Ms>(std::integer_sequence<int, Ms...>) __attribute__((always_inline)) { (tile(integral_constant<int, Ms>{}), ...); }(
+                std::make_integer_sequence<int, LRP_B_MT>{});
+            asm volatile("s_waitcnt vmcnt(10)\n\ts_barrier" ::: "memory");
+        };
+        for (; left > 0; left -= LPB_PERIOD)
+            [&]<int... Ss>(std::integer_sequence<int, Ss...>) __attribute__((always_inline)) { (stage(integral_constant<int, Ss>{}), ...); }(
+                std::make_integer_sequence<int, LPB_PERIOD>{});
+        asm volatile("s_waitcnt vmcnt(0)" ::: "memory");
+
+        const int lane_e = __builtin_amdgcn_mbcnt_hi(~0u, __builtin_amdgcn_mbcnt_lo(~0u, 0u));
+        const int r16_e = lane_e & 15, q_e = lane_e >> 4;
+        k1_store_q(Q, acc, wh * (16 * LRP_B_MT) + LRP_A_ROWS, q_e, (int64_t)tb * LP_T_BLK + wf * 16 + r16_e, T, K, q_stride, qscale_d);
+    }
+}
+
+int launch_k1_lowrank_pair(psa_ctx* c, const void* d_planes, const void* d_nodes, const void* d_diff, float2* d_qn, float2* d_q,
+                           const ProjGeom& g, int64_t n_fg, float dscale) {
+    PSA_REQUIRE(g.M_pad_d == LRP_ROWS && 2 * g.K <= LRP_ROWS && g.K > 0, "pair launch: one 512-row D block only");
+    PSA_REQUIRE(g.A_pad % (2 * K1_BA) == 0 && g.A_pad > 0, "pair launch needs the atom axis padded to %d", 2 * K1_BA);
+    PSA_REQUIRE(g.vscale > 0.f && dscale > 0.f && n_fg * 16 >= g.T, "planes do not cover the launch");
+    ProjGeom g2 = g;
+    g2.M_pad = 2 * LRP_ROWS;
+    K1Grid gr;
+    PSA_TRY(k1_grid(g2, LRP_ROWS, LP_T_BLK, gr));
+    PSA_REQUIRE(gr.n_mblk == 2 && gr.n_tblk < (1 << 29) && n_fg < (1ll << 31), "projection grid too large");
+    const float qscale_n = 1.f / (g.vscale * F16x2::P_SCALE) * g.wscale;
+    const float qscale_d = 1.f / (g.vscale * dscale) * g.wscale;
+    hipLaunchKernelGGL(k1_lowrank_pair_kernel, dim3(gr.blocks), dim3(512), 0, c->stream, (const _Float16*)d_planes,
+                       (const _Float16*)d_nodes, (const _Float16*)d_diff, d_qn, d_q, g.T, g.q_stride, (int)n_fg, g.A_pad / K1_BA, g.K,
+                       gr.n_tblk, qscale_n, qscale_d);
+    PSA_HIP_CHECK(hipGetLastError());
+    return PSA_OK;
+}
+
+}
diff --git a/psa_amd/csrc/k1_planes_diff.hip b/psa_amd/csrc/k1_planes_diff.hip
--- a/psa_amd/csrc/k1_planes_diff.hip
+++ b/psa_amd/csrc/k1_planes_diff.hip
@@ -1,6 +1,7 @@
 #include <utility>
 
 #include "k1_f16.h"
+#include "k1_lowrank_pair.h"
 
 namespace psa {
 
@@ -155,6 +156,7 @@
                                 d_planes, d_diff, d_q, g, n_fg);
 }
 
+template <bool PAIR>
 __global__ void __launch_bounds__(256)
 diff_table_kernel(const float* __restrict__ kvec, const double* __restrict__ kline, const float* __restrict__ mean_all,
                   const int* __restrict__ idx, const float* __restrict__ w, float wnorm, _Float16* __restrict__ Db, int K,
@@ -178,8 +180,8 @@
         d[1] = (float)(((double)cs[1] - se) * (double)dscale * wa);
     }
     const int n_stage = A_pad / K1_BA;
-    Db[pd16_index(2 * k, a, n_stage)] = (_Float16)d[0];
-    Db[pd16_index(2 * k + 1, a, n_stage)] = (_Float16)d[1];
+    Db[PAIR ? pd16_pair_index(2 * k, a, n_stage) : pd16_index(2 * k, a, n_stage)] = (_Float16)d[0];
+    Db[PAIR ? pd16_pair_index(2 * k + 1, a, n_stage) : pd16_index(2 * k + 1, a, n_stage)] = (_Float16)d[1];
 }
 
 __global__ void __launch_bounds__(256)
@@ -213,13 +215,22 @@
 
 int launch_lowrank_tables(psa_ctx* c, const float* d_kvec, const double* d_kline, const double* d_geo, const double* d_kappa,
                           const float* d_mean_all, const int* d_idx, void* d_diff, void* d_nodes, const ProjGeom& g, int M_pad_d,
-                          float dscale) {
+                          float dscale, bool pair) {
     PSA_REQUIRE(M_pad_d % D_M_BLK == 0 && M_pad_d >= 2 * g.K && g.A_pad % K1_BA == 0, "bad low-rank table geometry");
-    hipLaunchKernelGGL(diff_table_kernel, dim3(M_pad_d / 2, (g.A_pad + 255) / 256), dim3(256), 0, c->stream, d_kvec, d_kline, d_mean_all,
-                       d_idx, g.weights, 1.f / g.wscale, (_Float16*)d_diff, g.K, g.n_g, g.A_pad, dscale);
+    PSA_REQUIRE(!pair || M_pad_d == LRP_ROWS, "the pair launch's image is one 512-row block");
+    hipLaunchKernelGGL(pair ? diff_table_kernel<true> : diff_table_kernel<false>, dim3(M_pad_d / 2, (g.A_pad + 255) / 256), dim3(256), 0,
+                       c->stream, d_kvec, d_kline, d_mean_all, d_idx, g.weights, 1.f / g.wscale, (_Float16*)d_diff, g.K, g.n_g, g.A_pad,
+                       dscale);
     PSA_HIP_CHECK(hipGetLastError());
-    PSA_HIP_CHECK(hipMemsetAsync((char*)d_diff + (size_t)M_pad_d * g.A_pad * 2, 0, pd16_table_bytes(M_pad_d, g.A_pad) - (size_t)M_pad_d * g.A_pad * 2,
-                                 c->stream));
+    if (pair) {
+        const size_t n_stage = (size_t)g.A_pad / K1_BA, a_pad = LRP_PAD_STAGES * LRP_A_UNITS * 1024, b_pad = LRP_PAD_STAGES * LRP_B_UNITS * 1024;
+        static_assert(LRP_ROWS == D_M_BLK, "the pair image has the size of one D block");
+        PSA_HIP_CHECK(hipMemsetAsync((char*)d_diff + n_stage * LRP_A_UNITS * 1024, 0, a_pad, c->stream));
+        PSA_HIP_CHECK(hipMemsetAsync((char*)d_diff + pd16_pair_table_bytes((int)n_stage) - b_pad, 0, b_pad, c->stream));
+    } else {
+        PSA_HIP_CHECK(hipMemsetAsync((char*)d_diff + (size_t)M_pad_d * g.A_pad * 2, 0,
+                                     pd16_table_bytes(M_pad_d, g.A_pad) - (size_t)M_pad_d * g.A_pad * 2, c->stream));
+    }
     hipLaunchKernelGGL(node_table_kernel, dim3(LOWRANK_NODES, (g.A_pad + 255) / 256), dim3(256), 0, c->stream, d_geo, d_kappa, d_mean_all,
                        d_idx, g.weights, 1.f / g.wscale, (_Float16*)d_nodes, g.n_g, g.A_pad);
     PSA_HIP_CHECK(hipGetLastError());
diff --git a/psa_amd/csrc/psa_ctx.h b/psa_amd/csrc/psa_ctx.h
--- a/psa_amd/csrc/psa_ctx.h
+++ b/psa_amd/csrc/psa_ctx.h
@@ -133,6 +133,7 @@
     bool    lowrank = false;
     int     M_pad_d = 0;
     float   dscale = 0.f;
+    bool    lr_pair = false;
     const float* weights = nullptr;
     float        wscale = 1.f;
 };
@@ -219,6 +220,8 @@
     int64_t      opt_k1_lowrank_min_k = 256;
     int64_t      opt_k1_lowrank_min_local = 128;
     int64_t      lowrank_launches = 0;
+    int64_t      opt_k1_lowrank_pair = 1;
+    int64_t      lowrank_pair_launches = 0;
     psa::DevBuf  d_lr_diff, d_lr_qn, d_lr_L, d_lr_phi, d_lr_f64;
 
     psa::DevBuf  d_weights;
@@ -319,9 +322,12 @@
 size_t pd16_table_bytes(int M_pad, int A_pad);
 int    launch_lowrank_tables(psa_ctx* c, const float* d_kvec, const double* d_kline, const double* d_geo, const double* d_kappa,
                              const float* d_mean_all, const int* d_idx, void* d_diff, void* d_nodes, const ProjGeom& g, int M_pad_d,
-                             float dscale);
+                             float dscale, bool pair);
 int    launch_k1_planes_diff(psa_ctx* c, const void* d_planes, const void* d_diff, float2* d_q, const ProjGeom& g, int64_t n_fg,
                              float dscale);
+
+int    launch_k1_lowrank_pair(psa_ctx* c, const void* d_planes, const void* d_nodes, const void* d_diff, float2* d_qn, float2* d_q,
+                              const ProjGeom& g, int64_t n_fg, float dscale);
 
 int    launch_lowrank_combine_r(psa_ctx* c, const float2* d_qn, const float* d_L, const float2* d_phi, float2* d_q, const ProjGeom& g,
                                 int64_t qn_stride);
```

New measurement: 55150 billion (median of 6 runs). 2.3% higher.
